# autonomousvision/unimatch

Hardware: NVIDIA H100
Metric: image-pairs/sec @480x832 gmflow-scale2-refine6; EPE vs reference (higher is better)
Workload: dtype fp32

## Files before the change

### include/unimatch_sm100.h

```cpp
#ifndef UNIMATCH_SM100_H_
#define UNIMATCH_SM100_H_

#include <stdint.h>

#ifdef __cplusplus
extern "C" {
#endif

#define UM_OK 0
#define UM_EINVAL (-22)
#define UM_ECUDA (-5)

#define UM_FEATURE_DIM 128

#define UM_ABI_VERSION 4
int um_abi_version(void);
const char* um_build_info(void);
const char* um_last_error(void);
int64_t um_launch_count(void);

#define UM_MASK_NONE 0
#define UM_MASK_SWIN 1
#define UM_MASK_CAUSAL 2

typedef struct um_attn_geom {
  int32_t h, w;
  int32_t kh, kw;
  int32_t sh, sw;
  int32_t mask_mode;
} um_attn_geom;

int um_window_attention(const float* q, const float* k, const float* v, float* out,
                        int32_t n_streams, int32_t kv_shift,
                        int64_t ldq, int64_t ldk, int64_t ldv, int64_t ldo,
                        const um_attn_geom* geom, void* workspace, int64_t workspace_bytes, int32_t flags,
                        void* stream);
#define UM_ATTN_FORCE_CUDA_CORES 1
int64_t um_window_attention_workspace(const um_attn_geom* geom, int32_t n_streams);

int32_t um_attention_planes_lp(const um_attn_geom* geom);
int um_window_attention_planes(const void* q_planes, const void* k_planes, const void* v_planes, float* out, int64_t ldo,
                               void* out_split, int64_t split_plane_stride, int32_t n_streams, int32_t kv_shift,
                               const um_attn_geom* geom, void* stream);

#define UM_VALUE_TENSOR 0
#define UM_VALUE_COORDS 1
#define UM_VALUE_XCOORD 2
#define UM_POST_NONE 0
#define UM_POST_MINUS_OWN 1
#define UM_POST_OWN_MINUS 2

int um_softmax_expectation(const float* q, const float* k, const float* values, float* out,
                           int32_t n_streams, int32_t n_total, int32_t kv_shift,
                           int64_t ldq, int64_t ldk, int32_t vdim, int32_t value_mode, int32_t post_op,
                           const um_attn_geom* geom, void* workspace, int64_t workspace_bytes, int32_t flags,
                           void* stream);
int64_t um_softmax_expectation_workspace(const um_attn_geom* geom, int32_t n_total, int32_t value_mode);

int um_local_corr_softmax(const float* f0, const float* f1, float* flow,
                          int32_t batch, int32_t h, int32_t w, int32_t ry, int32_t rx, int32_t stereo,
                          void* stream);

int um_local_corr_volume(const float* f0, const float* f1, const float* flow, float* corr,
                         int32_t batch, int32_t h, int32_t w, int32_t radius, int32_t flow_dim, void* stream);

int um_flow_warp(const float* f, const float* flow, float* out,
                 int32_t batch, int32_t h, int32_t w, int32_t flow_dim, void* stream);

int um_fb_consistency(const float* fwd_flow, const float* bwd_flow, float alpha, float beta, float* fwd_occ,
                      float* bwd_occ, int32_t batch, int32_t h, int32_t w, void* stream);

int um_fb_consistency_error(const float* fwd_flow, const float* bwd_flow, float alpha, float beta, float* fwd_occ,
                            float* bwd_occ, float* fwd_err, int32_t batch, int32_t h, int32_t w, void* stream);

int um_propagate_local(const float* q, const float* k, const float* flow, float* out,
                       int32_t batch, int32_t h, int32_t w, int32_t radius, int32_t flow_dim,
                       int64_t ldq, int64_t ldk, void* stream);

int um_depth_corr_softmax(const float* f0, const float* f1, const float* Kmat, const float* Kinv,
                          const float* pose, const float* cand, float* out,
                          int32_t batch, int32_t h, int32_t w, int32_t num_cand, int32_t from_argmax,
                          void* stream);

int um_add_position(const float* x, const float* table, float* out,
                    int32_t n_streams, int32_t h, int32_t w, int32_t wh, int32_t ww, void* stream);

int um_convex_upsample(const float* flow, const float* mask, float* up,
                       int32_t batch, int32_t h, int32_t w, int32_t flow_dim, int32_t factor, float mult,
                       void* stream);

int um_upsample2x(const float* flow, float* out, int32_t batch, int32_t h, int32_t w, int32_t flow_dim,
                  float mult, void* stream);

int um_resize_bilinear(const float* in, float* out, int32_t batch, int32_t channels, int32_t h_in, int32_t w_in,
                       int32_t h_out, int32_t w_out, const float* scale, int32_t flip_x, void* stream);

int um_frames_to_planar(const uint8_t* frames, float* out, int32_t n, int32_t h, int32_t w, int32_t transpose,
                        int32_t h_out, int32_t w_out, void* stream);

int um_frames_to_planar_normalized(const uint8_t* frames, float* out, int32_t n, int32_t h, int32_t w, int32_t h_out,
                                   int32_t w_out, const float* mean, const float* std, void* stream);

typedef struct um_ragged_item {
  int64_t offset;
  int32_t h, w;
  float scale;
  int32_t flags;
} um_ragged_item;
#define UM_RAGGED_FLIP_X 1
#define UM_RAGGED_TRANSPOSE 2

int um_frames_to_planar_normalized_ragged(const uint8_t* frames, int64_t frames_bytes, const um_ragged_item* items, float* out,
                                          int32_t n, int32_t h_max, int32_t w_max, int32_t h_out, int32_t w_out,
                                          const float* mean, const float* std, void* stream);

int um_frames_to_planar_ragged(const uint8_t* frames, int64_t frames_bytes, const um_ragged_item* items, float* out, int32_t n,
                               int32_t h_max, int32_t w_max, int32_t h_out, int32_t w_out, void* stream);

int um_resize_bilinear_ragged(const float* in, float* out, int64_t out_numel, const um_ragged_item* items, int32_t n,
                              int32_t h_in, int32_t w_in, int32_t h_max, int32_t w_max, void* stream);

int um_disparity_to_image_ragged(const float* disp, int64_t numel, const um_ragged_item* items, uint8_t* out,
                                 float* minmax_scratch, int32_t n, int32_t h_max, int32_t w_max, void* stream);

int um_flow_to_image_ragged(const float* flow, int64_t flow_numel, const um_ragged_item* flow_items, uint8_t* out,
                            int64_t out_bytes, const um_ragged_item* picture_items, float* max_scratch, int32_t n,
                            int32_t h_max, int32_t w_max, void* stream);

int um_fb_consistency_ragged(const float* flow, int64_t flow_numel, const um_ragged_item* flow_items, float alpha, float beta,
                             float* occ, int64_t occ_numel, const um_ragged_item* occ_items, int32_t n, int32_t h_max,
                             int32_t w_max, void* stream);

int um_chain_tracks(const float* flow, const float* occ, int32_t n, int32_t h, int32_t w, float* pos, uint8_t* vis,
                    float* pos_out, uint8_t* vis_out, void* stream);

int um_track_points_forward(const float* flow, const float* occ, int32_t n, int32_t h, int32_t w, int32_t t0,
                            const float* queries, int32_t nq, int32_t nt, float* pos, uint8_t* vis, float* tracks,
                            uint8_t* visible, void* stream);
int um_track_points_backward(const float* flow, const float* occ, int32_t n, int32_t h, int32_t w, const float* queries,
                             int32_t nq, int32_t nt, float* tracks, uint8_t* visible, void* stream);

int um_multi_flow_tracks(const float* flow, const float* occ, const float* err, const int32_t* src, const int32_t* dst,
                         int32_t n, int32_t k, int32_t h, int32_t w, int32_t r, float* pos, float* sig, uint8_t* vis,
                         float* tracks, uint8_t* visible, float* sigma, void* stream);

int um_flow_to_image(const float* flow, uint8_t* out, int64_t row_stride, int64_t image_stride, float* max_scratch,
                     int32_t n, int32_t h, int32_t w, void* stream);

int um_disparity_to_image(const float* disp, uint8_t* out, int64_t row_stride, int64_t image_stride, float* minmax_scratch,
                          int32_t n, int32_t h, int32_t w, void* stream);

int um_depth_to_image(const float* depth, uint8_t* out, int64_t row_stride, int64_t image_stride, void* scratch, int32_t n,
                      int32_t h, int32_t w, void* stream);

int um_depth_to_image_ragged(const float* depth, int64_t numel, const um_ragged_item* items, uint8_t* out, void* scratch,
                             int32_t n, int32_t h_max, int32_t w_max, void* stream);

#define UM_SUBMIT_CROP 0
#define UM_SUBMIT_RESIZE 1
#define UM_SUBMIT_FLO 0
#define UM_SUBMIT_KITTI_FLOW_PNG 1
#define UM_SUBMIT_KITTI_DISP_PNG 2
#define UM_SUBMIT_PFM 3
int um_encode_submission(const float* pred, int32_t batch, int32_t channels, int32_t h, int32_t w, int32_t geometry,
                         int32_t top, int32_t left, int32_t out_h, int32_t out_w, int32_t format, uint8_t* out,
                         int64_t sample_stride, void* stream);

#define UM_EVAL_FLOW 0
#define UM_EVAL_STEREO 1
#define UM_EVAL_DEPTH 2
#define UM_EVAL_PARTS 128
#define UM_EVAL_MASK_ALL 0
#define UM_EVAL_MASK_VALID 1
#define UM_EVAL_MASK_VALID_MAX 2
enum um_eval_flow_cols {
  UM_EVF_N = 0,
  UM_EVF_EPE,
  UM_EVF_1PX, UM_EVF_3PX, UM_EVF_5PX,
  UM_EVF_OUTLIER,
  UM_EVF_S0_10_N, UM_EVF_S0_10_EPE,
  UM_EVF_S10_40_N, UM_EVF_S10_40_EPE,
  UM_EVF_S40_N, UM_EVF_S40_EPE,
  UM_EVF_MATCHED_N, UM_EVF_MATCHED_EPE,
  UM_EVF_UNMATCHED_N, UM_EVF_UNMATCHED_EPE,
  UM_EVAL_FLOW_COLS
};
enum um_eval_stereo_cols {
  UM_EVS_N = 0, UM_EVS_ABS,
  UM_EVS_D1,
  UM_EVS_1PX, UM_EVS_2PX, UM_EVS_3PX,
  UM_EVAL_STEREO_COLS
};
enum um_eval_depth_cols {
  UM_EVD_N = 0,
  UM_EVD_ABS_REL,
  UM_EVD_SQ_REL,
  UM_EVD_SQ,
  UM_EVD_LOG_SQ,
  UM_EVD_A1, UM_EVD_A2, UM_EVD_A3,
  UM_EVAL_DEPTH_COLS
};
int um_eval_stats(const float* pred, int64_t pred_sb, int64_t pred_sc, int64_t pred_sy, int64_t pred_sx, const float* gt,
                  const float* valid, const float* noc_valid, int32_t task, int32_t mask_mode, float max_val, float eval_min,
                  float eval_max, int32_t batch, int32_t h, int32_t w, double* scratch, double* out, void* stream);

#define UM_ACT_NONE 0
#define UM_ACT_RELU 1
#define UM_ACT_TANH 2
#define UM_ACT_SIGMOID 3
#define UM_ACT_GELU 4
#define UM_CONV_LINEAR 0
#define UM_CONV_GRU_ZR 1
#define UM_CONV_GRU_Q 2
#define UM_CONV_LN 3
typedef struct um_conv_desc {
  const void* src[2];
  int32_t cin_p[2];
  int32_t nsrc;
  int32_t batch, h, w;
  const void* weights;
  const float* bias;
  int32_t kh, kw, pad_h, pad_w;
  int32_t cout, cout_p, bn;
  int32_t mode, act;
  float* out_f32;
  int64_t ld_f32;
  int32_t off_f32;
  int32_t cp_split;
  void* out_split;
  int32_t off_split;
  int32_t stride;
  const float* aux0;
  int64_t ld_aux0;
  const float* aux1;
  int64_t ld_aux1;
  const float* gamma;
  const float* beta;
  int64_t src_plane_stride, split_plane_stride;
  void* win_dst;
  int32_t win_c0, win_c1, win_lp, win_streams;
  um_attn_geom win_geom;
  const float* pre;
  int64_t ld_pre;
} um_conv_desc;
int um_conv2d_tc(const um_conv_desc* desc, void* stream);

typedef struct um_ffn_desc {
  const void* src[2];
  int64_t src_plane_stride;
  int64_t rows;
  const void* w1;
  const void* w2;
  int32_t hidden;
  const float* residual;
  int64_t ld_res;
  const float* gamma;
  const float* beta;
  float* out_f32;
  int64_t ld_f32;
  void* out_split;
  int64_t split_plane_stride;
} um_ffn_desc;
int um_ffn_tc(const um_ffn_desc* desc, void* stream);

int um_conv7x7_small(const float* in0, const float* in1, int32_t nchw, int32_t n_half, int32_t n, int32_t h, int32_t w,
                     int32_t cin, int32_t stride, const float* weight, const float* bias, int32_t cout, int32_t relu,
                     const float* scale, const float* shift, float* out_f32, int64_t ld_out, void* out_split, int32_t cp,
                     void* stream);

int64_t um_instance_norm_scratch_floats(int32_t n, int32_t c);
int um_instance_norm_stats(const float* x, int64_t ld, int32_t n, int32_t hw, int32_t c, float* scratch, float* stats,
                           void* stream);
int um_instance_norm_apply(const float* a, int64_t ld_a, const float* stats_a, int32_t relu_a, const float* res,
                           int64_t ld_res, const float* stats_res, int32_t relu_out, float* out_f32, int64_t ld_o,
                           void* out_split, int32_t cp, int32_t off, int32_t n, int32_t hw, int32_t c, void* stream);

int um_split_planes(const float* src, int64_t rows, int32_t channels, int64_t ld, void* dst, int32_t cp, int32_t off,
                    int64_t dst_plane_stride, void* stream);

#ifdef __cplusplus
}
#endif
#endif
```

### unimatch_b200/csrc/um_conv_tc.cu

```cuda
#include <stdlib.h>

#include "um_common.cuh"
#include "um_tc.cuh"

namespace um {

using namespace tc;

namespace {

constexpr int TW = 16, TH = 8;
__host__ __device__ constexpr int stages_for(int bn) { return bn >= 96 ? 2 : 3; }
constexpr int NTHREADS = 512;
constexpr int EPILOGUE = 8;
constexpr int PRODUCER = 12;
constexpr int REGS_PRODUCER = 32, REGS_MMA = 168, REGS_EPI = 144;
constexpr uint32_t A_BYTES = 2 * 16384;
constexpr uint32_t STAGING_UNIT = 16384;
constexpr uint32_t STAGING_BYTES = 2 * STAGING_UNIT;
constexpr uint32_t TAIL_BYTES = 256 + 2048;
__host__ __device__ constexpr uint32_t acc_bytes(int bn) { return (bn < 32 ? 32 : bn) * 128 * 4; }
__host__ __device__ constexpr uint32_t conv_smem_bytes(int bn) {
  return stages_for(bn) * (A_BYTES + 2 * bn * 128) + acc_bytes(bn) + STAGING_BYTES + TAIL_BYTES;
}

struct ConvParams {
  int B, H, W, tiles_x, tiles_y;
  int nsrc, cin_p[2];
  int KH, KW, PH, PW, stride;
  int cout, cout_p;
  const float* bias;
  int mode, act;
  float* out_f32; long long ld_f32; int off_f32;
  __half* out_split; int cp_split, off_split; long long plane_split;
  const float* aux0; long long ld_aux0;
  const float* aux1; long long ld_aux1;
  const float* gamma; const float* beta;
  const float* pre; long long ld_pre;
  int ntiles, tiles_n;
  __half* win_dst; long long win_plane;
  int win_c0, win_c1, win_lp;
  long long win_tokens, win_L;
  Geom win_g;
};

__device__ __forceinline__ float sigmoid_fast(float y) { return __fdividef(1.0f, 1.0f + __expf(-y)); }
__device__ __forceinline__ float tanh_fast(float y) { return 1.0f - __fdividef(2.0f, 1.0f + __expf(2.0f * y)); }
__device__ __forceinline__ uint32_t pack_h2(__half a, __half b) {
  return (uint32_t)__half_as_ushort(a) | ((uint32_t)__half_as_ushort(b) << 16);
}

__device__ __forceinline__ void load_acc32(const float* accs, int r, int c0, float* v) {
  const float* row = accs + (c0 >> 5) * 4096 + r * 32;
#pragma unroll
  for (int i = 0; i < 8; ++i) {
    const float4 x = *reinterpret_cast<const float4*>(row + ((i ^ (r & 7)) << 2));
    v[4 * i] = x.x; v[4 * i + 1] = x.y; v[4 * i + 2] = x.z; v[4 * i + 3] = x.w;
  }
}

template <int BN, int G, int MODE, int ACT, bool WIN = false>
__global__ void __launch_bounds__(NTHREADS, 1)
conv_tc_kernel(const __grid_constant__ CUtensorMap map_a0, const __grid_constant__ CUtensorMap map_a1,
               const __grid_constant__ CUtensorMap map_w, const __grid_constant__ CUtensorMap map_of,
               const __grid_constant__ CUtensorMap map_os, ConvParams p) {
  static_assert(BN == 16 || BN == 64 || BN == 96 || BN == 128, "tile widths 16, 64, 96, 128");
  constexpr int NSB = 2;
  constexpr uint32_t B_BYTES = 2 * BN * 128;
  constexpr uint32_t STAGE_BYTES = A_BYTES + B_BYTES;
  constexpr int STAGES = stages_for(BN);
  constexpr uint32_t ACC_BYTES = acc_bytes(BN);
  extern __shared__ __align__(1024) uint8_t smem[];
  float* accs = reinterpret_cast<float*>(smem + STAGES * STAGE_BYTES);
  float* stage_buf = reinterpret_cast<float*>(smem + STAGES * STAGE_BYTES + ACC_BYTES);
  uint64_t* bars = reinterpret_cast<uint64_t*>(smem + STAGES * STAGE_BYTES + ACC_BYTES + STAGING_BYTES);
  uint64_t* full = bars;
  uint64_t* empty = bars + STAGES;
  uint64_t* acc_full = bars + 2 * STAGES;
  uint64_t* acc_empty = acc_full + 1;
  float* coef = reinterpret_cast<float*>(reinterpret_cast<uint8_t*>(bars) + 256);
  const int mode = MODE >= 0 ? MODE : p.mode;
  const int act = ACT >= 0 ? ACT : p.act;

  const int warp = threadIdx.x >> 5, lane = threadIdx.x & 31;
  auto k_stages = [&]() {
    int n = 0;
    for (int s = 0; s < p.nsrc; ++s) n += p.KH * p.KW * (p.cin_p[s] >> 6);
    return n;
  };

  if (threadIdx.x == 0) {
    for (int i = 0; i < STAGES; ++i) { mbar_init(full + i, 1); mbar_init(empty + i, 8); }
    mbar_init(acc_full, 256);
    mbar_init(acc_empty, 128);
    fence_barrier_init();
  }
  if (warp == PRODUCER && lane == 0) {
    tma_prefetch_desc(&map_a0); tma_prefetch_desc(&map_w);
    if (p.nsrc > 1) tma_prefetch_desc(&map_a1);
  }
  __syncthreads();

  if (warp >= PRODUCER) {
    setmaxnreg_dec<REGS_PRODUCER>();
    if (warp != PRODUCER) return;
    const int cid = (int)blockIdx.x, ncid = (int)gridDim.x;
    const int taps = p.KH * p.KW;
    const int nk = k_stages();
    int it = 0;
    for (int t = cid; t < p.ntiles; t += ncid) {
      const int n0 = (t % p.tiles_n) * BN;
      int tile = t / p.tiles_n;
      const int x0 = (tile % p.tiles_x) * TW; tile /= p.tiles_x;
      const int y0 = (tile % p.tiles_y) * TH;
      const int b = tile / p.tiles_y;
      const int chunks0 = p.cin_p[0] >> 6;
      const int nk0 = taps * chunks0;
      const int rot = (int)((unsigned)cid % (unsigned)nk);
      for (int kk = 0; kk < nk; ++kk, ++it) {
        int k = kk + rot; if (k >= nk) k -= nk;
        const int sidx = (k >= nk0) ? 1 : 0;
        const int kl = sidx ? k - nk0 : k;
        const int chunks = sidx ? (p.cin_p[1] >> 6) : chunks0;
        const int tap = kl / chunks, kc = kl - tap * chunks;
        const int ky = tap / p.KW, kx = tap - ky * p.KW;
        const CUtensorMap* ma = sidx ? &map_a1 : &map_a0;
        const int st = it % STAGES;
        mbar_wait_inline(empty + st, ((it / STAGES) & 1) ^ 1);
        uint8_t* sa = smem + st * STAGE_BYTES;
        uint8_t* sb = sa + A_BYTES;
        const int kcol = (sidx ? taps * p.cin_p[0] : 0) + tap * p.cin_p[sidx] + kc * 64;
        if (elect_one()) {
          mbar_arrive_expect_tx(full + st, STAGE_BYTES);
#pragma unroll
          for (int part = 0; part < 2; ++part) {
            tma_load_4d(sa + part * 16384, ma, full + st, kc * 64, x0 * p.stride + kx - p.PW, y0 * p.stride + ky - p.PH, part * p.B + b);
            tma_load_2d(sb + part * (BN * 128), &map_w, full + st, kcol, part * p.cout_p + n0);
          }
        }
        __syncwarp();
      }
    }
  } else if (warp < EPILOGUE) {
    setmaxnreg_inc<REGS_MMA>();
    const int cid = (int)blockIdx.x, ncid = (int)gridDim.x;
    const int nk = k_stages();
    const int quarter = warp & 3;
    const int grp = warp >> 2;
    const int frow = grp * 64 + quarter * 16 + (lane >> 2);
    const int fcol = 2 * (lane & 3);
    int lt = 0, it = 0;
    for (int t = cid; t < p.ntiles; t += ncid, ++lt) {
      float acc[BN / 2], part[BN / 2];
      for (int k = 0; k < nk; ++k, ++it) {
        const int st = it % STAGES;
        mbar_wait_inline(full + st, (it / STAGES) & 1);
        const uint32_t a_base = smem_u32(smem + st * STAGE_BYTES) + grp * 8192;
        const uint32_t b_base = smem_u32(smem + st * STAGE_BYTES) + A_BYTES;
        const int pa[3] = {1, 0, 0}, pb[3] = {0, 1, 0};
        if (G > 1) fence_acc(part); else fence_acc(acc);
        wgmma_fence();
#pragma unroll
        for (int c = 0; c < 3; ++c)
#pragma unroll
          for (int ks = 0; ks < 4; ++ks) {
            const uint64_t da = desc_kmajor(a_base + pa[c] * 16384 + ks * 32);
            const uint64_t db = desc_kmajor(b_base + pb[c] * (BN * 128) + ks * 32);
            if (G > 1) wgmma_ss<BN>(part, da, db, (c | ks) != 0);
            else wgmma_ss<BN>(acc, da, db, k > 0 || (c | ks) != 0);
          }
        wgmma_commit();
        wgmma_wait<0>();
        if (G > 1) fence_acc(part); else fence_acc(acc);
        __syncwarp();
        if (lane == 0) mbar_arrive(empty + st);
        if (G > 1) {
#pragma unroll
          for (int i = 0; i < BN / 2; ++i) acc[i] = k ? acc[i] + part[i] : part[i];
        }
      }
      mbar_wait_inline(acc_empty, (lt & 1) ^ 1);
#pragma unroll
      for (int j = 0; j < BN / 8; ++j) {
        const int col = 8 * j + fcol;
        float* chunk = accs + (col >> 5) * 4096;
#pragma unroll
        for (int h = 0; h < 2; ++h) {
          const int row = frow + 8 * h;
          *reinterpret_cast<float2*>(chunk + row * 32 + ((((col & 31) >> 2) ^ (row & 7)) << 2) + (col & 3)) =
              make_float2(acc[4 * j + 2 * h], acc[4 * j + 2 * h + 1]);
        }
      }
      mbar_arrive(acc_full);
    }
  } else {
    setmaxnreg_inc<REGS_EPI>();
    const int cid = (int)blockIdx.x, ncid = (int)gridDim.x;
    const int r = threadIdx.x - EPILOGUE * 32;
    const bool leader = r == 0;
    int sctr = 0;
    auto epi_sync = [&]() { asm volatile("bar.sync 1, 128;" ::: "memory"); };
    if (mode == UM_CONV_LN) { coef[256 + r] = __ldg(p.gamma + r); coef[384 + r] = __ldg(p.beta + r); }
    epi_sync();
    int lt = 0;
    for (int t = cid; t < p.ntiles; t += ncid, ++lt) {
      const int n0 = (t % p.tiles_n) * BN;
      int tile = t / p.tiles_n;
      const int x0 = (tile % p.tiles_x) * TW; tile /= p.tiles_x;
      const int y0 = (tile % p.tiles_y) * TH;
      const int b = tile / p.tiles_y;
      const long long pix_r = ((long long)b * p.H + (y0 + (r >> 4))) * p.W + x0 + (r & 15);
      const bool valid_r = (y0 + (r >> 4) < p.H) && (x0 + (r & 15) < p.W);

      auto emit = [&](const float (&v)[32], int co_out, bool to_f32, bool to_split, bool to_win = false) {
        if (WIN && to_win) {
          uint8_t* sbs = reinterpret_cast<uint8_t*>(stage_buf + (sctr % NSB) * 4096);
          ++sctr;
          if (leader) bulk_wait_read<0>();
          epi_sync();
#pragma unroll
          for (int i = 0; i < 4; ++i) {
            uint32_t hw[4], lw[4];
#pragma unroll
            for (int e = 0; e < 4; ++e) split_f16x2(v[8 * i + 2 * e], v[8 * i + 2 * e + 1], &hw[e], &lw[e]);
            const int off = r * 64 + ((i ^ ((r >> 1) & 3)) << 4);
            *reinterpret_cast<uint4*>(sbs + off) = make_uint4(hw[0], hw[1], hw[2], hw[3]);
            *reinterpret_cast<uint4*>(sbs + 8192 + off) = make_uint4(lw[0], lw[1], lw[2], lw[3]);
          }
          epi_sync();
          const int wc = co_out - p.win_c0;
          __half* obase = p.win_dst + (long long)(wc >> 7) * 2 * p.win_plane + (wc & 127);
          const int* rowdst = reinterpret_cast<const int*>(coef + 256) + (lt & 1) * 128;
          const int piece = r & 3;
#pragma unroll
          for (int itr = 0; itr < 4; ++itr) {
            const int row = itr * 32 + (r >> 2);
            const int drow = rowdst[row];
            if (drow < 0) continue;
            const int soff = row * 64 + ((piece ^ ((row >> 1) & 3)) << 4);
            const uint4 hv = *reinterpret_cast<const uint4*>(sbs + soff);
            const uint4 lv = *reinterpret_cast<const uint4*>(sbs + 8192 + soff);
            __half* d = obase + (long long)drow * 128 + piece * 8;
            *reinterpret_cast<uint4*>(d) = hv;
            *reinterpret_cast<uint4*>(d + p.win_plane) = lv;
          }
          return;
        }
        if (to_f32) {
          float* my_stage = stage_buf + (sctr % NSB) * 4096;
          ++sctr;
          if (leader) bulk_wait_read<NSB - 1>();
          epi_sync();
#pragma unroll
          for (int i = 0; i < 8; ++i)
            *reinterpret_cast<float4*>(my_stage + r * 32 + ((i ^ (r & 7)) << 2)) = make_float4(v[4 * i], v[4 * i + 1], v[4 * i + 2], v[4 * i + 3]);
          fence_proxy_async();
          epi_sync();
          if (leader) { tma_store_4d(&map_of, my_stage, co_out, x0, y0, b); bulk_commit(); }
        }
        if (to_split) {
          uint8_t* sbs = reinterpret_cast<uint8_t*>(stage_buf + (sctr % NSB) * 4096);
          ++sctr;
          if (leader) bulk_wait_read<NSB - 1>();
          epi_sync();
#pragma unroll
          for (int i = 0; i < 4; ++i) {
            uint32_t hw[4], lw[4];
#pragma unroll
            for (int e = 0; e < 4; ++e) split_f16x2(v[8 * i + 2 * e], v[8 * i + 2 * e + 1], &hw[e], &lw[e]);
            const int off = r * 64 + ((i ^ ((r >> 1) & 3)) << 4);
            *reinterpret_cast<uint4*>(sbs + off) = make_uint4(hw[0], hw[1], hw[2], hw[3]);
            *reinterpret_cast<uint4*>(sbs + 8192 + off) = make_uint4(lw[0], lw[1], lw[2], lw[3]);
          }
          fence_proxy_async();
          epi_sync();
          if (leader) {
            tma_store_4d(&map_os, sbs, co_out, x0, y0, b);
            tma_store_4d(&map_os, sbs + 8192, co_out, x0, y0, p.B + b);
            bulk_commit();
          }
        }
      };

      if constexpr (BN == 128) {
        if (mode == UM_CONV_LN) {
          mbar_wait_inline(acc_full, lt & 1);
          float sum0 = 0.f, sum1 = 0.f, sq0 = 0.f, sq1 = 0.f;
#pragma unroll 1
          for (int h = 0; h < 2; ++h) {
            float v0[32], v1[32];
            load_acc32(accs, r, 32 * h, v0);
            load_acc32(accs, r, 64 + 32 * h, v1);
            float sum = 0.f;
#pragma unroll
            for (int i = 0; i < 32; ++i) sum += v0[i];
#pragma unroll
            for (int i = 0; i < 32; ++i) sum += v1[i];
            if (h == 0) sum0 = sum; else sum1 = sum;
          }
          const float mean = (sum0 + sum1) * (1.0f / 128.0f);
#pragma unroll 1
          for (int h = 0; h < 2; ++h) {
            float v0[32], v1[32];
            load_acc32(accs, r, 32 * h, v0);
            load_acc32(accs, r, 64 + 32 * h, v1);
            float sq = 0.f;
#pragma unroll
            for (int i = 0; i < 32; ++i) { const float dd = v0[i] - mean; sq = fmaf(dd, dd, sq); }
#pragma unroll
            for (int i = 0; i < 32; ++i) { const float dd = v1[i] - mean; sq = fmaf(dd, dd, sq); }
            if (h == 0) sq0 = sq; else sq1 = sq;
          }
          const float rstd = rsqrtf((sq0 + sq1) * (1.0f / 128.0f) + 1e-5f);
          const bool need_a = valid_r && p.aux0;
#pragma unroll 1
          for (int c0 = 0; c0 < 128; c0 += 32) {
            float a[32];
            if (need_a) {
              const float4* pa = reinterpret_cast<const float4*>(p.aux0 + pix_r * p.ld_aux0 + c0);
#pragma unroll
              for (int i = 0; i < 8; ++i) { const float4 t4 = __ldg(pa + i); a[4 * i] = t4.x; a[4 * i + 1] = t4.y; a[4 * i + 2] = t4.z; a[4 * i + 3] = t4.w; }
            }
            float v[32];
            load_acc32(accs, r, c0, v);
            if (c0 == 96) mbar_arrive(acc_empty);
            const float4* g4 = reinterpret_cast<const float4*>(coef + 256 + c0);
            const float4* b4 = reinterpret_cast<const float4*>(coef + 384 + c0);
#pragma unroll
            for (int i = 0; i < 8; ++i) {
              const float4 g = g4[i], bb = b4[i];
              v[4 * i] = (v[4 * i] - mean) * rstd * g.x + bb.x;
              v[4 * i + 1] = (v[4 * i + 1] - mean) * rstd * g.y + bb.y;
              v[4 * i + 2] = (v[4 * i + 2] - mean) * rstd * g.z + bb.z;
              v[4 * i + 3] = (v[4 * i + 3] - mean) * rstd * g.w + bb.w;
            }
            if (need_a) {
#pragma unroll
              for (int i = 0; i < 32; ++i) v[i] += a[i];
            }
            emit(v, c0, p.out_f32 != nullptr, p.out_split != nullptr);
          }
          continue;
        }
      }

      float* sbias = coef + (lt & 1) * 128;
      if (r < BN) sbias[r] = (p.bias && n0 + r < p.cout) ? __ldg(p.bias + n0 + r) : 0.f;
      if (WIN) {
        const int yy = y0 + (r >> 4), xx = x0 + (r & 15);
        const long long token = ((long long)b * p.H + yy) * p.W + xx;
        int drow = -1;
        if (yy < p.H && xx < p.W && token < p.win_tokens) {
          const Geom& g = p.win_g;
          const int n = (int)(token / p.win_L);
          const int t = (int)(token - (long long)n * p.win_L);
          const int ty = t / g.w, tx = t - ty * g.w;
          int yr = ty - g.sh; if (yr < 0) yr += g.h;
          int xr = tx - g.sw; if (xr < 0) xr += g.w;
          const int wy = yr / g.wh, wx = xr / g.ww;
          drow = (n * g.nwin + wy * g.kw + wx) * p.win_lp + (yr - wy * g.wh) * g.ww + (xr - wx * g.ww);
        }
        reinterpret_cast<int*>(coef + 256)[(lt & 1) * 128 + r] = drow;
      }
      epi_sync();

      constexpr int CH = BN < 32 ? BN : 32;
#pragma unroll 1
      for (int c0 = 0; c0 < BN; c0 += 32) {
        const int co0 = n0 + c0;
        const bool live = co0 < p.cout;
        bool to_f32 = p.out_f32 != nullptr, to_split = p.out_split != nullptr;
        int co_out = co0;
        if (mode == UM_CONV_GRU_ZR) {
          to_f32 = co0 < 128; to_split = co0 >= 128;
          if (co0 >= 128) co_out = co0 - 128;
        }
        bool to_win = false;
        if (WIN && co0 >= p.win_c0 && co0 < p.win_c1) { to_win = true; to_f32 = to_split = false; }
        float px[32];
        const bool need_p = live && valid_r && p.pre;
        if (need_p) {
          const float4* pp = reinterpret_cast<const float4*>(p.pre + pix_r * p.ld_pre + co0);
#pragma unroll
          for (int i = 0; i < 8; ++i) { const float4 t4 = __ldg(pp + i); px[4 * i] = t4.x; px[4 * i + 1] = t4.y; px[4 * i + 2] = t4.z; px[4 * i + 3] = t4.w; }
        }
        float v[32];
        mbar_wait_inline(acc_full, lt & 1);
        load_acc32(accs, r, c0, v);
        if (c0 + 32 >= BN) mbar_arrive(acc_empty);
        if (!live) continue;
        if (p.bias) {
          const float4* s4 = reinterpret_cast<const float4*>(sbias + c0);
#pragma unroll
          for (int i = 0; i < CH / 4; ++i) {
            const float4 bb = s4[i];
            v[4 * i] += bb.x; v[4 * i + 1] += bb.y; v[4 * i + 2] += bb.z; v[4 * i + 3] += bb.w;
          }
        }
        if (need_p) {
#pragma unroll
          for (int i = 0; i < CH; ++i) v[i] += px[i];
        }
        float ax[32], bx[32];
        const bool need_a = valid_r && p.aux0 && (mode == UM_CONV_GRU_Q || (mode == UM_CONV_GRU_ZR && co0 >= 128));
        const bool need_b = valid_r && mode == UM_CONV_GRU_Q;
        if (need_a) {
          const float4* ap = reinterpret_cast<const float4*>(p.aux0 + pix_r * p.ld_aux0 + (mode == UM_CONV_GRU_ZR ? co0 - 128 : co0));
#pragma unroll
          for (int i = 0; i < 8; ++i) { const float4 t4 = __ldg(ap + i); ax[4 * i] = t4.x; ax[4 * i + 1] = t4.y; ax[4 * i + 2] = t4.z; ax[4 * i + 3] = t4.w; }
        }
        if (need_b) {
          const float4* bp = reinterpret_cast<const float4*>(p.aux1 + pix_r * p.ld_aux1 + co0);
#pragma unroll
          for (int i = 0; i < 8; ++i) { const float4 t4 = __ldg(bp + i); bx[4 * i] = t4.x; bx[4 * i + 1] = t4.y; bx[4 * i + 2] = t4.z; bx[4 * i + 3] = t4.w; }
        }
        if (mode == UM_CONV_GRU_ZR) {
#pragma unroll
          for (int i = 0; i < CH; ++i) v[i] = sigmoid_fast(v[i]);
          if (need_a) {
#pragma unroll
            for (int i = 0; i < CH; ++i) v[i] *= ax[i];
          }
        } else if (mode == UM_CONV_GRU_Q) {
          if (need_b) {
#pragma unroll
            for (int i = 0; i < CH; ++i) v[i] = (1.0f - bx[i]) * ax[i] + bx[i] * tanh_fast(v[i]);
          }
        } else if (act == UM_ACT_RELU) {
#pragma unroll
          for (int i = 0; i < CH; ++i) v[i] = fmaxf(v[i], 0.f);
        } else if (act == UM_ACT_TANH) {
#pragma unroll
          for (int i = 0; i < CH; ++i) v[i] = tanh_fast(v[i]);
        } else if (act == UM_ACT_SIGMOID) {
#pragma unroll
          for (int i = 0; i < CH; ++i) v[i] = sigmoid_fast(v[i]);
        } else if (act == UM_ACT_GELU) {
#pragma unroll
          for (int i = 0; i < CH; ++i) v[i] = act_gelu(v[i]);
        }
        if constexpr (BN >= 32) {
          emit(v, co_out, to_f32, to_split, to_win);
        } else {
          const int nvalid = min(CH, p.cout - co0);
          float* sb = stage_buf;
          epi_sync();
#pragma unroll
          for (int i = 0; i < CH / 4; ++i)
            *reinterpret_cast<float4*>(sb + r * 32 + ((i ^ (r & 7)) << 2)) = make_float4(v[4 * i], v[4 * i + 1], v[4 * i + 2], v[4 * i + 3]);
          epi_sync();
          if (to_f32) {
#pragma unroll 1
            for (int itr = 0; itr < 8; ++itr) {
              const int row = itr * 16 + (r >> 3), piece = r & 7;
              const int yy = y0 + (row >> 4), xx = x0 + (row & 15);
              if (yy >= p.H || xx >= p.W || piece * 4 >= nvalid) continue;
              const float4 val = *reinterpret_cast<const float4*>(sb + row * 32 + ((piece ^ (row & 7)) << 2));
              float* dst = p.out_f32 + (((long long)b * p.H + yy) * p.W + xx) * p.ld_f32 + p.off_f32 + co_out + piece * 4;
              const float e[4] = {val.x, val.y, val.z, val.w};
              for (int k = 0; k < 4; ++k) if (piece * 4 + k < nvalid) dst[k] = e[k];
            }
          }
          if (to_split) {
#pragma unroll 1
            for (int itr = 0; itr < 4; ++itr) {
              const int row = itr * 32 + (r >> 2), piece = r & 3;
              const int yy = y0 + (row >> 4), xx = x0 + (row & 15);
              if (yy >= p.H || xx >= p.W || piece * 8 >= nvalid) continue;
              const float4 a4 = *reinterpret_cast<const float4*>(sb + row * 32 + (((2 * piece) ^ (row & 7)) << 2));
              const float4 c4 = *reinterpret_cast<const float4*>(sb + row * 32 + (((2 * piece + 1) ^ (row & 7)) << 2));
              const float e[8] = {a4.x, a4.y, a4.z, a4.w, c4.x, c4.y, c4.z, c4.w};
              __half* dh = p.out_split + (((long long)b * p.H + yy) * p.W + xx) * p.cp_split + p.off_split + co_out + piece * 8;
              __half* dl = dh + p.plane_split;
              for (int k = 0; k < 8; ++k)
                if (piece * 8 + k < nvalid) { __half h0, l0; split_f16(e[k], &h0, &l0); dh[k] = h0; dl[k] = l0; }
            }
          }
        }
      }
    }
    if (leader) bulk_wait_all();
  }
}

template <int VEC>
__global__ void __launch_bounds__(256) split_planes_kernel(const float* __restrict__ src, long long ld, int C,
                                                           __half* __restrict__ dst, int cp, int off, long long plane,
                                                           long long rows) {
  const int per_row = C / VEC;
  const long long i = (long long)blockIdx.x * blockDim.x + threadIdx.x;
  if (i >= rows * per_row) return;
  const long long row = i / per_row;
  const int c = (int)(i - row * per_row) * VEC;
  if (VEC == 4) {
    const float4 x = __ldg(reinterpret_cast<const float4*>(src + row * ld + c));
    __half h[4], l[4];
    split_f16(x.x, &h[0], &l[0]); split_f16(x.y, &h[1], &l[1]); split_f16(x.z, &h[2], &l[2]); split_f16(x.w, &h[3], &l[3]);
    *reinterpret_cast<uint2*>(dst + row * cp + off + c) = make_uint2(pack_h2(h[0], h[1]), pack_h2(h[2], h[3]));
    *reinterpret_cast<uint2*>(dst + plane + row * cp + off + c) = make_uint2(pack_h2(l[0], l[1]), pack_h2(l[2], l[3]));
  } else {
    __half h, l;
    split_f16(__ldg(src + row * ld + c), &h, &l);
    dst[row * cp + off + c] = h;
    dst[plane + row * cp + off + c] = l;
  }
}

}

int make_map_4d_f16(CUtensorMap* map, const void* base, uint64_t cp, uint64_t W, uint64_t H, uint64_t NB, uint32_t stride,
                    uint64_t plane_elems) {
  PFN_encodeTiled enc = get_encode_tiled();
  if (!enc) { set_error("cuTensorMapEncodeTiled unavailable"); return UM_ECUDA; }
  cuuint64_t dims[4] = {cp, W, H, NB};
  cuuint64_t strides[3] = {cp * 2, cp * W * 2, (plane_elems ? plane_elems : cp * W * H) * 2};
  cuuint32_t box[4] = {64, 16 * stride, 8 * stride, 1};
  cuuint32_t estr[4] = {1, stride, stride, 1};
  CUresult r = enc(map, CU_TENSOR_MAP_DATA_TYPE_FLOAT16, 4, const_cast<void*>(base), dims, strides, box, estr,
                   CU_TENSOR_MAP_INTERLEAVE_NONE, CU_TENSOR_MAP_SWIZZLE_128B, CU_TENSOR_MAP_L2_PROMOTION_L2_128B,
                   CU_TENSOR_MAP_FLOAT_OOB_FILL_NONE);
  if (r != CUDA_SUCCESS) { set_error("cuTensorMapEncodeTiled(4d) failed (%d)", (int)r); return UM_ECUDA; }
  return UM_OK;
}

int make_map_out(CUtensorMap* map, void* base, int elem_bytes, uint64_t cout, uint64_t ld, uint64_t W, uint64_t H, uint64_t N,
                 uint64_t plane_elems) {
  PFN_encodeTiled enc = get_encode_tiled();
  if (!enc) { set_error("cuTensorMapEncodeTiled unavailable"); return UM_ECUDA; }
  cuuint64_t dims[4] = {cout, W, H, N};
  cuuint64_t strides[3] = {ld * elem_bytes, ld * W * elem_bytes, (plane_elems ? plane_elems : ld * W * H) * elem_bytes};
  cuuint32_t box[4] = {32, 16, 8, 1};
  cuuint32_t estr[4] = {1, 1, 1, 1};
  CUresult r = enc(map, elem_bytes == 4 ? CU_TENSOR_MAP_DATA_TYPE_FLOAT32 : CU_TENSOR_MAP_DATA_TYPE_FLOAT16, 4, base, dims,
                   strides, box, estr, CU_TENSOR_MAP_INTERLEAVE_NONE,
                   elem_bytes == 4 ? CU_TENSOR_MAP_SWIZZLE_128B : CU_TENSOR_MAP_SWIZZLE_64B,
                   CU_TENSOR_MAP_L2_PROMOTION_NONE, CU_TENSOR_MAP_FLOAT_OOB_FILL_NONE);
  if (r != CUDA_SUCCESS) { set_error("cuTensorMapEncodeTiled(out) failed (%d)", (int)r); return UM_ECUDA; }
  return UM_OK;
}

namespace {

template <int BN, int G, int MODE, int ACT, bool WIN = false>
int launch_conv(const CUtensorMap& m0, const CUtensorMap& m1, const CUtensorMap& mw, const CUtensorMap& mof,
                const CUtensorMap& mos, const ConvParams& p, cudaStream_t st) {
  constexpr uint32_t smem = conv_smem_bytes(BN);
  static_assert(smem <= 232448, "shared memory budget");
  static PerDeviceBytes configured;
  if (int rc = ensure_smem(configured, conv_tc_kernel<BN, G, MODE, ACT, WIN>, smem, "conv_tc")) return rc;
  const int num_sms = device_sm_count();
  const int grid = p.ntiles < num_sms ? p.ntiles : num_sms;
  conv_tc_kernel<BN, G, MODE, ACT, WIN><<<grid, NTHREADS, smem, st>>>(m0, m1, mw, mof, mos, p);
  return check_launch("um_conv2d_tc");
}

}
}

extern "C" {

int um_conv2d_tc(const um_conv_desc* d, void* stream) {
  using namespace um;
  UM_REQUIRE(d && d->src[0] && d->weights, "um_conv2d_tc: null descriptor / source / weights");
  UM_REQUIRE(d->batch > 0 && d->h > 0 && d->w > 0, "um_conv2d_tc: bad shape");
  UM_REQUIRE(d->nsrc == 1 || (d->nsrc == 2 && d->src[1]), "um_conv2d_tc: nsrc must be 1 or 2");
  for (int s = 0; s < d->nsrc; ++s)
    UM_REQUIRE(d->cin_p[s] > 0 && d->cin_p[s] % 64 == 0, "um_conv2d_tc: padded input channels must be multiples of 64");
  UM_REQUIRE(d->bn == 16 || d->bn == 64 || d->bn == 96 || d->bn == 128 || d->bn == 192 || d->bn == 256,
             "um_conv2d_tc: bn must be 16, 64, 96, 128, 192 or 256");
  UM_REQUIRE(d->cout > 0 && d->cout_p >= d->cout && d->cout_p % d->bn == 0, "um_conv2d_tc: bad output channel padding");
  UM_REQUIRE(d->kh > 0 && d->kw > 0 && d->kh * d->kw <= 49, "um_conv2d_tc: bad filter size");
  UM_REQUIRE(d->mode >= UM_CONV_LINEAR && d->mode <= UM_CONV_LN, "um_conv2d_tc: bad mode");
  if (d->mode == UM_CONV_LN)
    UM_REQUIRE(d->cout == 128 && d->cout_p == 128 && d->bn == 128 && d->gamma && d->beta && d->ld_f32 % 4 == 0 &&
                   d->off_f32 % 4 == 0 && d->cp_split % 8 == 0 && d->off_split % 8 == 0 && d->ld_aux0 % 4 == 0,
               "um_conv2d_tc: LN needs cout = cout_p = bn = 128, gamma/beta and 16-byte aligned rows");
  const bool win = d->win_dst != nullptr;
  UM_REQUIRE(d->out_f32 || d->out_split || win, "um_conv2d_tc: no output");
  Geom wg{};
  if (win) {
    UM_REQUIRE(d->mode == UM_CONV_LINEAR && d->act == UM_ACT_NONE && d->bn == 128 && d->batch == 1 && d->stride == 1 &&
                   d->kh == 1 && d->kw == 1 && d->nsrc == 1 && d->cin_p[0] == 128,
               "um_conv2d_tc: window-plane output needs a plain 128 -> cout Linear layer (bn 128, batch 1)");
    UM_REQUIRE(make_geom(&d->win_geom, &wg), "um_conv2d_tc: bad window geometry");
    UM_REQUIRE(d->win_c0 >= 0 && d->win_c0 % 128 == 0 && d->win_c1 % 128 == 0 && d->win_c1 > d->win_c0 && d->win_c1 <= d->cout_p,
               "um_conv2d_tc: window-plane channel range must be 128-aligned and inside cout_p");
    UM_REQUIRE(d->win_streams > 0 && d->win_lp >= wg.lw && d->win_lp % 128 == 0 &&
                   (long long)d->win_streams * wg.h * wg.w <= (long long)d->h * d->w,
               "um_conv2d_tc: window-plane rows (streams * h * w) exceed the GEMM rows / bad lp");
    UM_REQUIRE((reinterpret_cast<uintptr_t>(d->win_dst) & 15) == 0, "um_conv2d_tc: window planes must be 16-byte aligned");
    UM_REQUIRE(d->out_f32 || d->out_split || (d->win_c0 == 0 && d->win_c1 >= d->cout),
               "um_conv2d_tc: channels outside the window-plane range have no destination");
  }
  if (d->src_plane_stride || d->split_plane_stride)
    UM_REQUIRE(d->batch == 1 && d->src_plane_stride >= 0 && d->split_plane_stride >= 0 && d->src_plane_stride % 8 == 0 &&
                   d->split_plane_stride % 8 == 0,
               "um_conv2d_tc: explicit (hi, lo) plane strides need batch 1 and multiples of 8 halves");
  if (d->mode == UM_CONV_GRU_ZR)
    UM_REQUIRE(d->cout == 256 && (d->bn == 128 || d->bn == 256) && d->aux0 && d->out_f32 && d->out_split,
               "um_conv2d_tc: GRU_ZR needs cout 256, bn 128 or 256, h, z-out and rh-out");
  if (d->mode == UM_CONV_GRU_Q)
    UM_REQUIRE(d->cout == 128 && d->aux0 && d->aux1, "um_conv2d_tc: GRU_Q needs cout 128, h and z");

  if (d->pre)
    UM_REQUIRE(d->mode != UM_CONV_LN && d->bn >= 32 && d->ld_pre % 4 == 0 && d->ld_pre >= d->cout && d->cout % 32 == 0 &&
                   (reinterpret_cast<uintptr_t>(d->pre) & 15) == 0,
               "um_conv2d_tc: pre-accumulated input needs a non-LN mode, bn >= 32, cout %% 32 == 0 and 16-byte aligned rows");
  UM_REQUIRE(d->stride == 1 || d->stride == 2 || d->stride == 4 || d->stride == 8, "um_conv2d_tc: stride must be 1, 2, 4 or 8");
  const int ho = (d->h + 2 * d->pad_h - d->kh) / d->stride + 1, wo = (d->w + 2 * d->pad_w - d->kw) / d->stride + 1;
  UM_REQUIRE(ho > 0 && wo > 0, "um_conv2d_tc: empty output");
  ConvParams p{};
  p.B = d->batch; p.H = ho; p.W = wo; p.stride = d->stride;
  p.tiles_x = (wo + TW - 1) / TW; p.tiles_y = (ho + TH - 1) / TH;
  p.nsrc = d->nsrc; p.cin_p[0] = d->cin_p[0]; p.cin_p[1] = d->nsrc > 1 ? d->cin_p[1] : 0;
  p.KH = d->kh; p.KW = d->kw; p.PH = d->pad_h; p.PW = d->pad_w;
  p.cout = d->cout; p.cout_p = d->cout_p; p.bias = d->bias; p.mode = d->mode; p.act = d->act;
  p.out_f32 = d->out_f32; p.ld_f32 = d->ld_f32; p.off_f32 = d->off_f32;
  p.out_split = reinterpret_cast<__half*>(d->out_split); p.cp_split = d->cp_split; p.off_split = d->off_split;
  p.plane_split = (long long)d->batch * ho * wo * d->cp_split;
  p.aux0 = d->aux0; p.ld_aux0 = d->ld_aux0; p.aux1 = d->aux1; p.ld_aux1 = d->ld_aux1;
  p.gamma = d->gamma; p.beta = d->beta;
  p.pre = d->pre; p.ld_pre = d->ld_pre;
  if (d->split_plane_stride) p.plane_split = d->split_plane_stride;
  if (win) {
    p.win_dst = reinterpret_cast<__half*>(d->win_dst);
    p.win_g = wg; p.win_lp = d->win_lp; p.win_c0 = d->win_c0; p.win_c1 = d->win_c1;
    p.win_L = (long long)wg.h * wg.w;
    p.win_tokens = (long long)d->win_streams * p.win_L;
    p.win_plane = (long long)d->win_streams * wg.nwin * d->win_lp * 128;
  }

  long long ktot = 0;
  for (int s = 0; s < d->nsrc; ++s) ktot += (long long)d->kh * d->kw * d->cin_p[s];
  const long long nk = ktot / 64;
  const bool multi = nk >= 8;
  const int bn = d->bn == 256 ? 128 : d->bn == 192 ? 96 : d->bn;
  p.tiles_n = d->cout_p / bn;
  p.ntiles = p.tiles_x * p.tiles_y * p.B * p.tiles_n;
  CUtensorMap m0, m1, mw;
  int rc;
  const uint64_t sps = (uint64_t)d->src_plane_stride;
  if ((rc = make_map_4d_f16(&m0, d->src[0], d->cin_p[0], d->w, d->h, 2ull * d->batch, d->stride, sps))) return rc;
  if (d->nsrc > 1) { if ((rc = make_map_4d_f16(&m1, d->src[1], d->cin_p[1], d->w, d->h, 2ull * d->batch, d->stride, sps))) return rc; }
  else m1 = m0;
  if ((rc = make_map_2d_f16(&mw, d->weights, 2ull * d->cout_p, (uint64_t)ktot, (uint32_t)bn))) return rc;
  cudaStream_t st = (cudaStream_t)stream;
  CUtensorMap mof = m0, mos = m0;
  if (d->bn >= 32) {
    const int c_f32 = (d->mode == UM_CONV_GRU_ZR) ? 128 : d->cout, c_split = (d->mode == UM_CONV_GRU_ZR) ? 128 : d->cout;
    if (d->out_f32) {
      UM_REQUIRE(d->ld_f32 % 4 == 0 && d->off_f32 % 4 == 0 && (reinterpret_cast<uintptr_t>(d->out_f32) & 15) == 0,
                 "um_conv2d_tc: fp32 output must be 16-byte aligned (ld, channel offset multiples of 4)");
      if ((rc = make_map_out(&mof, d->out_f32 + d->off_f32, 4, c_f32, d->ld_f32, wo, ho, d->batch))) return rc;
    }
    if (d->out_split) {
      UM_REQUIRE(d->cp_split % 8 == 0 && d->off_split % 8 == 0 && (reinterpret_cast<uintptr_t>(d->out_split) & 15) == 0,
                 "um_conv2d_tc: split output must be 16-byte aligned (cp, channel offset multiples of 8)");
      if ((rc = make_map_out(&mos, reinterpret_cast<__half*>(d->out_split) + d->off_split, 2, c_split, d->cp_split, wo, ho,
                             2ull * d->batch, (uint64_t)d->split_plane_stride))) return rc;
    }
  }
#define UM_CONV_CASE(BN_, G_, MODE_, ACT_)                                                   \
  if (bn == BN_ && multi == (G_ > 1) && d->mode == MODE_ && ((MODE_) != UM_CONV_LINEAR || d->act == (ACT_))) \
    return launch_conv<BN_, G_, MODE_, (MODE_) == UM_CONV_LINEAR ? (ACT_) : 0>(m0, m1, mw, mof, mos, p, st);
  if (win) {
    UM_REQUIRE(nk <= 2, "um_conv2d_tc: window-plane output is built for K <= 128");
    return launch_conv<128, 1, UM_CONV_LINEAR, UM_ACT_NONE, true>(m0, m1, mw, mof, mos, p, st);
  }
  UM_CONV_CASE(128, 1, UM_CONV_LINEAR, UM_ACT_NONE)
  UM_CONV_CASE(128, 1, UM_CONV_LINEAR, UM_ACT_RELU)
  UM_CONV_CASE(128, 1, UM_CONV_LINEAR, UM_ACT_GELU)
  UM_CONV_CASE(128, 1, UM_CONV_LN, 0)
  UM_CONV_CASE(128, 2, UM_CONV_LN, 0)
  UM_CONV_CASE(128, 2, UM_CONV_LINEAR, UM_ACT_NONE)
  UM_CONV_CASE(128, 2, UM_CONV_LINEAR, UM_ACT_RELU)
  UM_CONV_CASE(128, 2, UM_CONV_GRU_ZR, 0)
  UM_CONV_CASE(128, 2, UM_CONV_GRU_Q, 0)
  UM_CONV_CASE(96, 2, UM_CONV_LINEAR, UM_ACT_RELU)
  UM_CONV_CASE(64, 4, UM_CONV_LINEAR, UM_ACT_NONE)
  UM_CONV_CASE(64, 4, UM_CONV_LINEAR, UM_ACT_RELU)
#undef UM_CONV_CASE
  if (bn == 128) return multi ? launch_conv<128, 2, -1, -1>(m0, m1, mw, mof, mos, p, st) : launch_conv<128, 1, -1, -1>(m0, m1, mw, mof, mos, p, st);
  if (bn == 96) return multi ? launch_conv<96, 2, -1, -1>(m0, m1, mw, mof, mos, p, st) : launch_conv<96, 1, -1, -1>(m0, m1, mw, mof, mos, p, st);
  if (bn == 64) return multi ? launch_conv<64, 4, -1, -1>(m0, m1, mw, mof, mos, p, st) : launch_conv<64, 1, -1, -1>(m0, m1, mw, mof, mos, p, st);
  return multi ? launch_conv<16, 4, -1, -1>(m0, m1, mw, mof, mos, p, st) : launch_conv<16, 1, -1, -1>(m0, m1, mw, mof, mos, p, st);
}

int um_split_planes(const float* src, int64_t rows, int32_t channels, int64_t ld, void* dst, int32_t cp, int32_t off,
                    int64_t dst_plane_stride, void* stream) {
  UM_REQUIRE(src && dst && rows > 0 && channels > 0 && off >= 0 && off + channels <= cp && ld >= channels,
             "um_split_planes: bad arguments");
  UM_REQUIRE(dst_plane_stride == 0 || (dst_plane_stride >= rows * cp && dst_plane_stride % 4 == 0),
             "um_split_planes: dst_plane_stride must cover rows * cp halves (multiple of 4)");
  const long long plane = dst_plane_stride ? (long long)dst_plane_stride : (long long)rows * cp;
  const bool vec = (channels % 4 == 0) && (ld % 4 == 0) && (off % 4 == 0) && (cp % 4 == 0) &&
                   ((reinterpret_cast<uintptr_t>(src) & 15) == 0);
  if (vec) {
    const long long total = (long long)rows * (channels / 4);
    um::split_planes_kernel<4><<<(unsigned)((total + 255) / 256), 256, 0, (cudaStream_t)stream>>>(
        src, ld, channels, reinterpret_cast<__half*>(dst), cp, off, plane, rows);
  } else {
    const long long total = (long long)rows * channels;
    um::split_planes_kernel<1><<<(unsigned)((total + 255) / 256), 256, 0, (cudaStream_t)stream>>>(
        src, ld, channels, reinterpret_cast<__half*>(dst), cp, off, plane, rows);
  }
  return um::check_launch("um_split_planes");
}

}
```

### unimatch_b200/csrc/um_norm.cu

```cuda
#include "um_common.cuh"
#include "um_tc.cuh"

namespace {

constexpr int CHUNKS = 64;

__device__ __forceinline__ float4 in_pivot(const float* __restrict__ x, long long ld, int hw, int n, int c4) {
  const int np = hw < 16 ? hw : 16;
  float4 p = make_float4(0.f, 0.f, 0.f, 0.f);
  for (int r = 0; r < np; ++r) {
    const float4 v = __ldg(reinterpret_cast<const float4*>(x + ((long long)n * hw + r) * ld) + c4);
    p.x += v.x; p.y += v.y; p.z += v.z; p.w += v.w;
  }
  const float inv = 1.0f / (float)np;
  return make_float4(p.x * inv, p.y * inv, p.z * inv, p.w * inv);
}

__global__ void __launch_bounds__(256) in_partial_kernel(const float* __restrict__ x, long long ld, int hw, int C,
                                                         float* __restrict__ partial) {
  extern __shared__ float sm[];
  const int n = blockIdx.y, chunk = blockIdx.x;
  const int c4n = C >> 2;
  const int rlanes = 256 / c4n;
  const int c4 = threadIdx.x % c4n, rl = threadIdx.x / c4n;
  const int rows_per_chunk = (hw + CHUNKS - 1) / CHUNKS;
  const int r0 = chunk * rows_per_chunk, r1 = min(hw, r0 + rows_per_chunk);
  float4 s = make_float4(0.f, 0.f, 0.f, 0.f), q = make_float4(0.f, 0.f, 0.f, 0.f);
  if (rl < rlanes) {
    const float4 pv = in_pivot(x, ld, hw, n, c4);
    for (int r = r0 + rl; r < r1; r += rlanes) {
      float4 v = __ldg(reinterpret_cast<const float4*>(x + ((long long)n * hw + r) * ld) + c4);
      v.x -= pv.x; v.y -= pv.y; v.z -= pv.z; v.w -= pv.w;
      s.x += v.x; s.y += v.y; s.z += v.z; s.w += v.w;
      q.x = fmaf(v.x, v.x, q.x); q.y = fmaf(v.y, v.y, q.y); q.z = fmaf(v.z, v.z, q.z); q.w = fmaf(v.w, v.w, q.w);
    }
  }
  float* ss = sm;
  float* qs = sm + rlanes * C;
  if (rl < rlanes) {
    reinterpret_cast<float4*>(ss + rl * C)[c4] = s;
    reinterpret_cast<float4*>(qs + rl * C)[c4] = q;
  }
  __syncthreads();
  if (threadIdx.x < C) {
    float a = 0.f, b = 0.f;
    for (int i = 0; i < rlanes; ++i) { a += ss[i * C + threadIdx.x]; b += qs[i * C + threadIdx.x]; }
    float* dst = partial + (((long long)n * CHUNKS + chunk) * 2) * C;
    dst[threadIdx.x] = a;
    dst[C + threadIdx.x] = b;
  }
}

__global__ void in_finalize_kernel(const float* __restrict__ x, long long ld, const float* __restrict__ partial,
                                   float* __restrict__ stats, int hw, int C, int total) {
  const int i = blockIdx.x * blockDim.x + threadIdx.x;
  if (i >= total) return;
  const int n = i / C, c = i - n * C;
  const float4 pv = in_pivot(x, ld, hw, n, c >> 2);
  const float piv = (c & 3) == 0 ? pv.x : (c & 3) == 1 ? pv.y : (c & 3) == 2 ? pv.z : pv.w;
  double s = 0.0, q = 0.0;
  for (int k = 0; k < CHUNKS; ++k) {
    const float* p = partial + (((long long)n * CHUNKS + k) * 2) * C;
    s += (double)p[c]; q += (double)p[C + c];
  }
  const double dm = s / hw;
  double var = q / hw - dm * dm;
  if (var < 0.0) var = 0.0;
  stats[((long long)n * 2) * C + c] = (float)((double)piv + dm);
  stats[((long long)n * 2 + 1) * C + c] = (float)(1.0 / sqrt(var + 1e-5));
}

struct ApplyParams {
  const float* a; long long ld_a; const float* st_a; int relu_a;
  const float* res; long long ld_res; const float* st_res; int relu_out;
  float* out; long long ld_o;
  __half* split; int cp, off; long long plane;
  int hw, C; long long total4;
};

__device__ __forceinline__ uint32_t pk(__half a, __half b) {
  return (uint32_t)__half_as_ushort(a) | ((uint32_t)__half_as_ushort(b) << 16);
}

__global__ void __launch_bounds__(256) in_apply_kernel(ApplyParams p) {
  long long i = (long long)blockIdx.x * blockDim.x + threadIdx.x;
  const long long stride = (long long)gridDim.x * blockDim.x;
  const int c4n = p.C >> 2;
  for (; i < p.total4; i += stride) {
    const int c4 = (int)(i % c4n);
    const long long row = i / c4n;
    const int n = (int)(row / p.hw);
    float4 v = __ldg(reinterpret_cast<const float4*>(p.a + row * p.ld_a) + c4);
    if (p.st_a) {
      const float4 m = __ldg(reinterpret_cast<const float4*>(p.st_a + ((long long)n * 2) * p.C) + c4);
      const float4 r = __ldg(reinterpret_cast<const float4*>(p.st_a + ((long long)n * 2 + 1) * p.C) + c4);
      v.x = (v.x - m.x) * r.x; v.y = (v.y - m.y) * r.y; v.z = (v.z - m.z) * r.z; v.w = (v.w - m.w) * r.w;
    }
    if (p.relu_a) { v.x = fmaxf(v.x, 0.f); v.y = fmaxf(v.y, 0.f); v.z = fmaxf(v.z, 0.f); v.w = fmaxf(v.w, 0.f); }
    if (p.res) {
      float4 u = __ldg(reinterpret_cast<const float4*>(p.res + row * p.ld_res) + c4);
      if (p.st_res) {
        const float4 m = __ldg(reinterpret_cast<const float4*>(p.st_res + ((long long)n * 2) * p.C) + c4);
        const float4 r = __ldg(reinterpret_cast<const float4*>(p.st_res + ((long long)n * 2 + 1) * p.C) + c4);
        u.x = (u.x - m.x) * r.x; u.y = (u.y - m.y) * r.y; u.z = (u.z - m.z) * r.z; u.w = (u.w - m.w) * r.w;
      }
      v.x += u.x; v.y += u.y; v.z += u.z; v.w += u.w;
    }
    if (p.relu_out) { v.x = fmaxf(v.x, 0.f); v.y = fmaxf(v.y, 0.f); v.z = fmaxf(v.z, 0.f); v.w = fmaxf(v.w, 0.f); }
    if (p.out) reinterpret_cast<float4*>(p.out + row * p.ld_o)[c4] = v;
    if (p.split) {
      __half h[4], l[4];
      um::tc::split_f16(v.x, &h[0], &l[0]); um::tc::split_f16(v.y, &h[1], &l[1]);
      um::tc::split_f16(v.z, &h[2], &l[2]); um::tc::split_f16(v.w, &h[3], &l[3]);
      __half* d = p.split + row * p.cp + p.off + c4 * 4;
      *reinterpret_cast<uint2*>(d) = make_uint2(pk(h[0], h[1]), pk(h[2], h[3]));
      *reinterpret_cast<uint2*>(d + p.plane) = make_uint2(pk(l[0], l[1]), pk(l[2], l[3]));
    }
  }
}

}

extern "C" {

int64_t um_instance_norm_scratch_floats(int32_t n, int32_t c) { return (int64_t)n * CHUNKS * 2 * c; }

int um_instance_norm_stats(const float* x, int64_t ld, int32_t n, int32_t hw, int32_t c, float* scratch, float* stats,
                           void* stream) {
  UM_REQUIRE(x && scratch && stats && n > 0 && hw > 0 && c > 0 && c % 4 == 0 && c <= 256 && ld % 4 == 0 && ld >= c,
             "um_instance_norm_stats: bad arguments (channels must be a multiple of 4, <= 256)");
  const int rlanes = 256 / (c / 4);
  UM_REQUIRE(rlanes >= 1, "um_instance_norm_stats: too many channels");
  cudaStream_t st = (cudaStream_t)stream;
  in_partial_kernel<<<dim3(CHUNKS, n), 256, 2 * rlanes * c * sizeof(float), st>>>(x, ld, hw, c, scratch);
  int rc = um::check_launch("um_instance_norm_stats(partial)");
  if (rc) return rc;
  const int total = n * c;
  in_finalize_kernel<<<(total + 127) / 128, 128, 0, st>>>(x, ld, scratch, stats, hw, c, total);
  return um::check_launch("um_instance_norm_stats(finalize)");
}

int um_instance_norm_apply(const float* a, int64_t ld_a, const float* stats_a, int32_t relu_a, const float* res,
                           int64_t ld_res, const float* stats_res, int32_t relu_out, float* out_f32, int64_t ld_o,
                           void* out_split, int32_t cp, int32_t off, int32_t n, int32_t hw, int32_t c, void* stream) {
  UM_REQUIRE(a && n > 0 && hw > 0 && c > 0 && c % 4 == 0 && ld_a % 4 == 0, "um_instance_norm_apply: bad arguments");
  UM_REQUIRE(out_f32 || out_split, "um_instance_norm_apply: no output");
  UM_REQUIRE(!res || ld_res % 4 == 0, "um_instance_norm_apply: bad residual stride");
  UM_REQUIRE(!out_f32 || ld_o % 4 == 0, "um_instance_norm_apply: bad output stride");
  UM_REQUIRE(!out_split || (cp % 4 == 0 && off % 4 == 0 && off + c <= cp), "um_instance_norm_apply: bad split layout");
  ApplyParams p{};
  p.a = a; p.ld_a = ld_a; p.st_a = stats_a; p.relu_a = relu_a;
  p.res = res; p.ld_res = ld_res; p.st_res = stats_res; p.relu_out = relu_out;
  p.out = out_f32; p.ld_o = ld_o;
  p.split = reinterpret_cast<__half*>(out_split); p.cp = cp; p.off = off; p.plane = (long long)n * hw * cp;
  p.hw = hw; p.C = c; p.total4 = (long long)n * hw * (c / 4);
  long long blocks = (p.total4 + 255) / 256;
  if (blocks > 132LL * 32) blocks = 132LL * 32;
  in_apply_kernel<<<(unsigned)blocks, 256, 0, (cudaStream_t)stream>>>(p);
  return um::check_launch("um_instance_norm_apply");
}

}
```

### unimatch_b200/csrc/um_stem.cu

```cuda
#include "um_common.cuh"
#include "um_tc.cuh"

namespace {

constexpr int TX = 32, TY = 8;
constexpr int PX = 4;
constexpr int CB = 16;
constexpr int NT = 256;

struct StemParams {
  const float* in0; const float* in1;
  int nchw, n_half;
  int N, H, W, cin, stride;
  int HO, WO, cout;
  const float* weight;
  const float* bias;
  int relu;
  float scale[3], shift[3];
  float* out; long long ld_out;
  __half* split; int cp; long long plane;
  int tiles_x, tiles_y, ntiles;
};

template <int CIN, int S>
__global__ void __launch_bounds__(NT) stem7x7_kernel(StemParams p) {
  extern __shared__ __align__(16) float sm[];
  constexpr int IWR = (TX - 1) * S + 7, IW = (IWR + 3) & ~3, IH = (TY - 1) * S + 7;
  constexpr int NIN = (PX - 1) * S + 7;
  float* s_w = sm;
  float* s_in = sm + p.cout * CIN * 49;
  const int tid = threadIdx.x;
  for (int i = tid; i < p.cout * CIN * 49; i += NT) {
    const int co = i / (CIN * 49), k = i - co * (CIN * 49);
    s_w[k * p.cout + co] = __ldg(p.weight + i);
  }
  const int pg = tid & 63, cg = tid >> 6;
  const int lx = (pg & 7) * PX, ly = pg >> 3;

  for (int t = blockIdx.x; t < p.ntiles; t += gridDim.x) {
    int tt = t;
    const int tx0 = (tt % p.tiles_x) * TX; tt /= p.tiles_x;
    const int ty0 = (tt % p.tiles_y) * TY;
    const int n = tt / p.tiles_y;
    const int x_in0 = tx0 * S - 3, y_in0 = ty0 * S - 3;
    __syncthreads();
    for (int i = tid; i < CIN * IH * IW; i += NT) {
      const int c = i / (IH * IW), r = i - c * IH * IW;
      const int yy = y_in0 + r / IW, xx = x_in0 + r % IW;
      float v = 0.f;
      if (yy >= 0 && yy < p.H && xx >= 0 && xx < p.W) {
        if (p.nchw) {
          const float* src = (n < p.n_half) ? p.in0 + (long long)n * CIN * p.H * p.W : p.in1 + (long long)(n - p.n_half) * CIN * p.H * p.W;
          v = __ldg(src + ((long long)c * p.H + yy) * p.W + xx) * p.scale[c] + p.shift[c];
        } else {
          v = __ldg(p.in0 + (((long long)n * p.H + yy) * p.W + xx) * CIN + c);
        }
      }
      s_in[i] = v;
    }
    __syncthreads();
    const int oy = ty0 + ly;
    for (int cbase = cg * CB; cbase < p.cout; cbase += 4 * CB) {
      float acc[PX][CB];
#pragma unroll
      for (int c = 0; c < CB; ++c) {
        const float bv = p.bias ? __ldg(p.bias + cbase + c) : 0.f;
#pragma unroll
        for (int j = 0; j < PX; ++j) acc[j][c] = bv;
      }
#pragma unroll 1
      for (int c = 0; c < CIN; ++c) {
#pragma unroll 1
        for (int ky = 0; ky < 7; ++ky) {
          const float* row = s_in + (c * IH + ly * S + ky) * IW + lx * S;
          float in[16];
#pragma unroll
          for (int q = 0; q < (NIN + 3) / 4; ++q) {
            const float4 v4 = *reinterpret_cast<const float4*>(row + 4 * q);
            in[4 * q] = v4.x; in[4 * q + 1] = v4.y; in[4 * q + 2] = v4.z; in[4 * q + 3] = v4.w;
          }
          const float* wrow = s_w + ((c * 7 + ky) * 7) * p.cout + cbase;
#pragma unroll
          for (int kx = 0; kx < 7; ++kx) {
            float w[CB];
#pragma unroll
            for (int q = 0; q < CB / 4; ++q) {
              const float4 w4 = *reinterpret_cast<const float4*>(wrow + kx * p.cout + 4 * q);
              w[4 * q] = w4.x; w[4 * q + 1] = w4.y; w[4 * q + 2] = w4.z; w[4 * q + 3] = w4.w;
            }
#pragma unroll
            for (int j = 0; j < PX; ++j) {
              const float xv = in[j * S + kx];
#pragma unroll
              for (int cc = 0; cc < CB; ++cc) acc[j][cc] = fmaf(xv, w[cc], acc[j][cc]);
            }
          }
        }
      }
      if (oy < p.HO) {
#pragma unroll
        for (int j = 0; j < PX; ++j) {
          const int ox = tx0 + lx + j;
          if (ox >= p.WO) continue;
          const long long pix = ((long long)n * p.HO + oy) * p.WO + ox;
          if (p.relu) {
#pragma unroll
            for (int cc = 0; cc < CB; ++cc) acc[j][cc] = fmaxf(acc[j][cc], 0.f);
          }
          if (p.out) {
#pragma unroll
            for (int q = 0; q < CB / 4; ++q)
              *reinterpret_cast<float4*>(p.out + pix * p.ld_out + cbase + 4 * q) =
                  make_float4(acc[j][4 * q], acc[j][4 * q + 1], acc[j][4 * q + 2], acc[j][4 * q + 3]);
          }
          if (p.split) {
            __half* d = p.split + pix * p.cp + cbase;
#pragma unroll
            for (int q = 0; q < CB / 8; ++q) {
              uint32_t hw[4], lw[4];
#pragma unroll
              for (int e = 0; e < 4; ++e) um::tc::split_f16x2(acc[j][8 * q + 2 * e], acc[j][8 * q + 2 * e + 1], &hw[e], &lw[e]);
              *reinterpret_cast<uint4*>(d + 8 * q) = make_uint4(hw[0], hw[1], hw[2], hw[3]);
              *reinterpret_cast<uint4*>(d + p.plane + 8 * q) = make_uint4(lw[0], lw[1], lw[2], lw[3]);
            }
          }
        }
      }
    }
  }
}

template <int CIN, int S>
int launch(StemParams p, cudaStream_t st) {
  constexpr int IWR = (TX - 1) * S + 7, IW = (IWR + 3) & ~3, IH = (TY - 1) * S + 7;
  const size_t smem = (size_t)(p.cout * CIN * 49 + CIN * IH * IW + 8) * sizeof(float);
  static um::PerDeviceBytes configured;
  if (int rc = um::ensure_smem(configured, stem7x7_kernel<CIN, S>, smem, "stem7x7")) return rc;
  const int num_sms = um::device_sm_count();
  p.tiles_x = (p.WO + TX - 1) / TX; p.tiles_y = (p.HO + TY - 1) / TY;
  p.ntiles = p.tiles_x * p.tiles_y * p.N;
  const int grid = p.ntiles < 2 * num_sms ? p.ntiles : 2 * num_sms;
  stem7x7_kernel<CIN, S><<<grid, NT, smem, st>>>(p);
  return um::check_launch("um_conv7x7_small");
}

}

extern "C" int um_conv7x7_small(const float* in0, const float* in1, int32_t nchw, int32_t n_half, int32_t n, int32_t h,
                                int32_t w, int32_t cin, int32_t stride, const float* weight, const float* bias, int32_t cout,
                                int32_t relu, const float* scale, const float* shift, float* out_f32, int64_t ld_out,
                                void* out_split, int32_t cp, void* stream) {
  UM_REQUIRE(in0 && weight && n > 0 && h > 0 && w > 0 && cin >= 1 && cin <= 3 && (stride == 1 || stride == 2),
             "um_conv7x7_small: bad arguments (1 <= cin <= 3, stride 1 or 2)");
  UM_REQUIRE(cout > 0 && cout % 16 == 0 && cout <= 128 && (out_f32 || out_split),
             "um_conv7x7_small: cout must be a multiple of 16 (<= 128) and an output given");
  UM_REQUIRE(!out_f32 || ld_out % 4 == 0, "um_conv7x7_small: bad output stride");
  UM_REQUIRE(!out_split || cp % 8 == 0, "um_conv7x7_small: bad plane width");
  UM_REQUIRE(!nchw || in1 || n_half >= n, "um_conv7x7_small: second source missing");
  StemParams p{};
  p.in0 = in0; p.in1 = in1; p.nchw = nchw; p.n_half = n_half;
  p.N = n; p.H = h; p.W = w; p.cin = cin; p.stride = stride;
  p.HO = (h + 6 - 7) / stride + 1; p.WO = (w + 6 - 7) / stride + 1; p.cout = cout;
  p.weight = weight; p.bias = bias; p.relu = relu;
  for (int c = 0; c < 3; ++c) { p.scale[c] = scale ? scale[c] : 1.f; p.shift[c] = shift ? shift[c] : 0.f; }
  p.out = out_f32; p.ld_out = ld_out;
  p.split = reinterpret_cast<__half*>(out_split); p.cp = cp; p.plane = (long long)n * p.HO * p.WO * cp;
  cudaStream_t st = (cudaStream_t)stream;
  if (stride == 1) {
    if (cin == 1) return launch<1, 1>(p, st);
    if (cin == 2) return launch<2, 1>(p, st);
    return launch<3, 1>(p, st);
  }
  if (cin == 1) return launch<1, 2>(p, st);
  if (cin == 2) return launch<2, 2>(p, st);
  return launch<3, 2>(p, st);
}
```

### unimatch_b200/ops.py

```python
import ctypes
import os

import torch

_HERE = os.path.dirname(os.path.abspath(__file__))
LIB_PATH = os.path.join(_HERE, "libunimatch_sm100.so")

MASK_NONE, MASK_SWIN, MASK_CAUSAL = 0, 1, 2
VALUE_TENSOR, VALUE_COORDS, VALUE_XCOORD = 0, 1, 2
POST_NONE, POST_MINUS_OWN, POST_OWN_MINUS = 0, 1, 2


FORCE_CUDA_CORES = 1
_force_cuda_cores = False


def set_force_cuda_cores(flag):
    global _force_cuda_cores
    _force_cuda_cores = bool(flag)


EVAL_FLOW, EVAL_STEREO, EVAL_DEPTH = 0, 1, 2
EVAL_MASK_ALL, EVAL_MASK_VALID, EVAL_MASK_VALID_MAX = 0, 1, 2
EVAL_PARTS = 128
EVAL_FLOW_COLS = ("n", "epe", "1px", "3px", "5px", "outlier", "s0_10_n", "s0_10_epe", "s10_40_n", "s10_40_epe", "s40_n",
                  "s40_epe", "matched_n", "matched_epe", "unmatched_n", "unmatched_epe")
EVAL_STEREO_COLS = ("n", "abs", "d1", "1px", "2px", "3px")
EVAL_DEPTH_COLS = ("n", "abs_rel", "sq_rel", "sq", "log_sq", "a1", "a2", "a3")
EVAL_COLS = {EVAL_FLOW: EVAL_FLOW_COLS, EVAL_STEREO: EVAL_STEREO_COLS, EVAL_DEPTH: EVAL_DEPTH_COLS}


ACT_NONE, ACT_RELU, ACT_TANH, ACT_SIGMOID, ACT_GELU = 0, 1, 2, 3, 4
CONV_LINEAR, CONV_GRU_ZR, CONV_GRU_Q, CONV_LN = 0, 1, 2, 3


class AttnGeom(ctypes.Structure):
    _fields_ = [(n, ctypes.c_int32) for n in ("h", "w", "kh", "kw", "sh", "sw", "mask_mode")]


class ConvDesc(ctypes.Structure):
    _fields_ = [("src", ctypes.c_void_p * 2), ("cin_p", ctypes.c_int32 * 2), ("nsrc", ctypes.c_int32),
                ("batch", ctypes.c_int32), ("h", ctypes.c_int32), ("w", ctypes.c_int32),
                ("weights", ctypes.c_void_p), ("bias", ctypes.c_void_p),
                ("kh", ctypes.c_int32), ("kw", ctypes.c_int32), ("pad_h", ctypes.c_int32), ("pad_w", ctypes.c_int32),
                ("cout", ctypes.c_int32), ("cout_p", ctypes.c_int32), ("bn", ctypes.c_int32),
                ("mode", ctypes.c_int32), ("act", ctypes.c_int32),
                ("out_f32", ctypes.c_void_p), ("ld_f32", ctypes.c_int64), ("off_f32", ctypes.c_int32),
                ("cp_split", ctypes.c_int32), ("out_split", ctypes.c_void_p), ("off_split", ctypes.c_int32),
                ("stride", ctypes.c_int32),
                ("aux0", ctypes.c_void_p), ("ld_aux0", ctypes.c_int64), ("aux1", ctypes.c_void_p), ("ld_aux1", ctypes.c_int64),
                ("gamma", ctypes.c_void_p), ("beta", ctypes.c_void_p),
                ("src_plane_stride", ctypes.c_int64), ("split_plane_stride", ctypes.c_int64),
                ("win_dst", ctypes.c_void_p), ("win_c0", ctypes.c_int32), ("win_c1", ctypes.c_int32),
                ("win_lp", ctypes.c_int32), ("win_streams", ctypes.c_int32), ("win_geom", AttnGeom),
                ("pre", ctypes.c_void_p), ("ld_pre", ctypes.c_int64)]


class RaggedItem(ctypes.Structure):
    _fields_ = [("offset", ctypes.c_int64), ("h", ctypes.c_int32), ("w", ctypes.c_int32), ("scale", ctypes.c_float),
                ("flags", ctypes.c_int32)]


RAGGED_FLIP_X, RAGGED_TRANSPOSE = 1, 2
RAGGED_ITEM_BYTES = ctypes.sizeof(RaggedItem)


class FfnDesc(ctypes.Structure):
    _fields_ = [("src", ctypes.c_void_p * 2), ("src_plane_stride", ctypes.c_int64), ("rows", ctypes.c_int64),
                ("w1", ctypes.c_void_p), ("w2", ctypes.c_void_p), ("hidden", ctypes.c_int32),
                ("residual", ctypes.c_void_p), ("ld_res", ctypes.c_int64), ("gamma", ctypes.c_void_p), ("beta", ctypes.c_void_p),
                ("out_f32", ctypes.c_void_p), ("ld_f32", ctypes.c_int64), ("out_split", ctypes.c_void_p),
                ("split_plane_stride", ctypes.c_int64)]


_P, _I, _L, _F = ctypes.c_void_p, ctypes.c_int32, ctypes.c_int64, ctypes.c_float
_G, _FP, _RC = ctypes.POINTER(AttnGeom), ctypes.POINTER(ctypes.c_float), ctypes.c_int

_SIGNATURES = {
    "um_abi_version": (_RC, []),
    "um_build_info": (ctypes.c_char_p, []),
    "um_last_error": (ctypes.c_char_p, []),
    "um_launch_count": (_L, []),
    "um_window_attention": (_RC, [_P, _P, _P, _P, _I, _I, _L, _L, _L, _L, _G, _P, _L, _I, _P]),
    "um_window_attention_workspace": (_L, [_G, _I]),
    "um_attention_planes_lp": (_I, [_G]),
    "um_window_attention_planes": (_RC, [_P, _P, _P, _P, _L, _P, _L, _I, _I, _G, _P]),
    "um_softmax_expectation": (_RC, [_P, _P, _P, _P, _I, _I, _I, _L, _L, _I, _I, _I, _G, _P, _L, _I, _P]),
    "um_softmax_expectation_workspace": (_L, [_G, _I, _I]),
    "um_local_corr_softmax": (_RC, [_P, _P, _P, _I, _I, _I, _I, _I, _I, _P]),
    "um_local_corr_volume": (_RC, [_P, _P, _P, _P, _I, _I, _I, _I, _I, _P]),
    "um_flow_warp": (_RC, [_P, _P, _P, _I, _I, _I, _I, _P]),
    "um_fb_consistency": (_RC, [_P, _P, _F, _F, _P, _P, _I, _I, _I, _P]),
    "um_fb_consistency_ragged": (_RC, [_P, _L, _P, _F, _F, _P, _L, _P, _I, _I, _I, _P]),
    "um_fb_consistency_error": (_RC, [_P, _P, _F, _F, _P, _P, _P, _I, _I, _I, _P]),
    "um_chain_tracks": (_RC, [_P, _P, _I, _I, _I, _P, _P, _P, _P, _P]),
    "um_track_points_forward": (_RC, [_P, _P, _I, _I, _I, _I, _P, _I, _I, _P, _P, _P, _P, _P]),
    "um_track_points_backward": (_RC, [_P, _P, _I, _I, _I, _P, _I, _I, _P, _P, _P]),
    "um_multi_flow_tracks": (_RC, [_P, _P, _P, _P, _P, _I, _I, _I, _I, _I, _P, _P, _P, _P, _P, _P, _P]),
    "um_propagate_local": (_RC, [_P, _P, _P, _P, _I, _I, _I, _I, _I, _L, _L, _P]),
    "um_depth_corr_softmax": (_RC, [_P, _P, _P, _P, _P, _P, _P, _I, _I, _I, _I, _I, _P]),
    "um_add_position": (_RC, [_P, _P, _P, _I, _I, _I, _I, _I, _P]),
    "um_convex_upsample": (_RC, [_P, _P, _P, _I, _I, _I, _I, _I, _F, _P]),
    "um_upsample2x": (_RC, [_P, _P, _I, _I, _I, _I, _F, _P]),
    "um_resize_bilinear": (_RC, [_P, _P, _I, _I, _I, _I, _I, _I, _FP, _I, _P]),
    "um_frames_to_planar": (_RC, [_P, _P, _I, _I, _I, _I, _I, _I, _P]),
    "um_frames_to_planar_ragged": (_RC, [_P, _L, _P, _P, _I, _I, _I, _I, _I, _P]),
    "um_frames_to_planar_normalized": (_RC, [_P, _P, _I, _I, _I, _I, _I, _FP, _FP, _P]),
    "um_frames_to_planar_normalized_ragged": (_RC, [_P, _L, _P, _P, _I, _I, _I, _I, _I, _FP, _FP, _P]),
    "um_resize_bilinear_ragged": (_RC, [_P, _P, _L, _P, _I, _I, _I, _I, _I, _P]),
    "um_disparity_to_image_ragged": (_RC, [_P, _L, _P, _P, _P, _I, _I, _I, _P]),
    "um_flow_to_image": (_RC, [_P, _P, _L, _L, _P, _I, _I, _I, _P]),
    "um_flow_to_image_ragged": (_RC, [_P, _L, _P, _P, _L, _P, _P, _I, _I, _I, _P]),
    "um_disparity_to_image": (_RC, [_P, _P, _L, _L, _P, _I, _I, _I, _P]),
    "um_depth_to_image": (_RC, [_P, _P, _L, _L, _P, _I, _I, _I, _P]),
    "um_depth_to_image_ragged": (_RC, [_P, _L, _P, _P, _P, _I, _I, _I, _P]),
    "um_encode_submission": (_RC, [_P, _I, _I, _I, _I, _I, _I, _I, _I, _I, _I, _P, _L, _P]),
    "um_eval_stats": (_RC, [_P, _L, _L, _L, _L, _P, _P, _P, _I, _I, _F, _F, _F, _I, _I, _I, _P, _P, _P]),
    "um_conv2d_tc": (_RC, [ctypes.POINTER(ConvDesc), _P]),
    "um_ffn_tc": (_RC, [ctypes.POINTER(FfnDesc), _P]),
    "um_conv7x7_small": (_RC, [_P, _P, _I, _I, _I, _I, _I, _I, _I, _P, _P, _I, _I, _FP, _FP, _P, _L, _P, _I, _P]),
    "um_instance_norm_scratch_floats": (_L, [_I, _I]),
    "um_instance_norm_stats": (_RC, [_P, _L, _I, _I, _I, _P, _P, _P]),
    "um_instance_norm_apply": (_RC, [_P, _L, _P, _I, _P, _L, _P, _I, _P, _L, _P, _I, _I, _I, _I, _I, _P]),
    "um_split_planes": (_RC, [_P, _L, _I, _L, _P, _I, _I, _L, _P]),
}
SYMBOLS = list(_SIGNATURES)


def _load():
    from .csrc.build import build, have_nvcc
    if have_nvcc():
        build()
    elif not os.path.exists(LIB_PATH):
        raise ImportError("libunimatch_sm100.so is missing and nvcc is not available to build it")
    lib = ctypes.CDLL(LIB_PATH)
    missing = [s for s in SYMBOLS if not hasattr(lib, s)]
    if missing:
        raise ImportError("libunimatch_sm100.so lacks symbols %s (stale build? run python unimatch_b200/csrc/build.py --force)" % missing)
    for name, (restype, argtypes) in _SIGNATURES.items():
        fn = getattr(lib, name)
        fn.restype, fn.argtypes = restype, argtypes
    return lib


LIB = _load()


def build_info():
    return LIB.um_build_info().decode()


def launch_count():
    return int(LIB.um_launch_count())


def _check(rc, name):
    if rc != 0:
        raise RuntimeError("%s failed (%d): %s" % (name, rc, LIB.um_last_error().decode()))


def _p(t):
    return ctypes.c_void_p(t.data_ptr()) if t is not None else None


def _stream():
    return ctypes.c_void_p(torch.cuda.current_stream().cuda_stream)


def _f32c(t, name, rows_ok=False):
    if not t.is_cuda:
        raise RuntimeError("%s: expected a CUDA tensor (libunimatch_sm100 has no CPU path)" % name)
    if t.dtype != torch.float32:
        raise RuntimeError("%s: expected float32" % name)
    if rows_ok:
        if t.stride(-1) != 1:
            raise RuntimeError("%s: last dim must be contiguous" % name)
    elif not t.is_contiguous():
        raise RuntimeError("%s: expected a contiguous tensor" % name)
    return t


def _rows(t, name):
    _f32c(t, name, rows_ok=True)
    if t.dim() != 3 or t.shape[-1] != 128:
        raise RuntimeError("%s: expected [N, L, 128]" % name)
    ld = t.stride(1)
    if t.shape[0] > 1 and t.stride(0) != ld * t.shape[1]:
        raise RuntimeError("%s: batch stride must equal L * row stride" % name)
    return ld


_lib = torch.library.Library("unimatch_sm100", "DEF")


def _define(schema, impl):
    _lib.define(schema)
    name = schema.split("(")[0]
    _lib.impl(name, impl, "CUDA")
    return getattr(torch.ops.unimatch_sm100, name)


def _window_attention(q, k, v, kv_shift, h, w, kh, kw, sh, sw, mask_mode):
    ldq, ldk, ldv = _rows(q, "q"), _rows(k, "k"), _rows(v, "v")
    n, l, _ = q.shape
    out = torch.empty((n, l, 128), device=q.device, dtype=torch.float32)
    g = AttnGeom(h, w, kh, kw, sh, sw, mask_mode)
    flags = FORCE_CUDA_CORES if _force_cuda_cores else 0
    ws_bytes = 0 if flags else int(LIB.um_window_attention_workspace(ctypes.byref(g), n))
    ws = torch.empty((ws_bytes,), device=q.device, dtype=torch.uint8) if ws_bytes else None
    _check(LIB.um_window_attention(_p(q), _p(k), _p(v), _p(out), n, kv_shift, ldq, ldk, ldv, 128, ctypes.byref(g),
                                   _p(ws), ws_bytes, flags, _stream()), "um_window_attention")
    return out


window_attention = _define(
    "window_attention(Tensor q, Tensor k, Tensor v, int kv_shift, int h, int w, int kh, int kw, int sh, int sw, "
    "int mask_mode) -> Tensor", _window_attention)


def attention_planes_lp(h, w, kh, kw, sh, sw, mask_mode):
    g = AttnGeom(h, w, kh, kw, sh, sw, mask_mode)
    return int(LIB.um_attention_planes_lp(ctypes.byref(g)))


def _planes_ok(t, name, n, nwin, lp):
    if t.dtype != torch.float16 or not t.is_contiguous() or t.numel() != 2 * n * nwin * lp * 128:
        raise RuntimeError("%s: expected contiguous fp16 planes [2, %d, %d, %d, 128]" % (name, n, nwin, lp))


def _window_attention_planes(qp, kp, vp, n, kv_shift, h, w, kh, kw, sh, sw, mask_mode, out_f32, out_split):
    g = AttnGeom(h, w, kh, kw, sh, sw, mask_mode)
    lp = int(LIB.um_attention_planes_lp(ctypes.byref(g)))
    if lp == 0:
        raise RuntimeError("window_attention_planes: geometry is not built for the tensor-core kernel")
    for t, nm in ((qp, "q_planes"), (kp, "k_planes"), (vp, "v_planes")):
        _planes_ok(t, nm, n, kh * kw, lp)
    ldo, plane = 0, 0
    if out_f32 is not None:
        ldo = _rows(out_f32, "out_f32")
    if out_split is not None:
        if out_split.dtype != torch.float16 or not out_split.is_contiguous() or out_split.shape[0] != 2 or out_split.shape[-1] != 128:
            raise RuntimeError("window_attention_planes: out_split must be contiguous fp16 planes [2, rows, 128]")
        plane = out_split[0].numel()
    _check(LIB.um_window_attention_planes(_p(qp), _p(kp), _p(vp), _p(out_f32), ldo, _p(out_split), plane, n, kv_shift,
                                          ctypes.byref(g), _stream()), "um_window_attention_planes")


window_attention_planes = _define(
    "window_attention_planes(Tensor q_planes, Tensor k_planes, Tensor v_planes, int n_streams, int kv_shift, int h, int w, "
    "int kh, int kw, int sh, int sw, int mask_mode, Tensor(a!)? out_f32, Tensor(b!)? out_split) -> ()",
    _window_attention_planes)


def _softmax_expectation(q, k, values, n_streams, kv_shift, vdim, value_mode, post_op, h, w, kh, kw, mask_mode):
    ldq, ldk = _rows(q, "q"), _rows(k, "k")
    n_total, l, _ = q.shape
    if values is not None:
        _f32c(values, "values")
    out = torch.empty((n_streams, l, vdim), device=q.device, dtype=torch.float32)
    g = AttnGeom(h, w, kh, kw, 0, 0, mask_mode)
    flags = FORCE_CUDA_CORES if _force_cuda_cores else 0
    ws_bytes = 0 if flags else int(LIB.um_softmax_expectation_workspace(ctypes.byref(g), n_total, value_mode))
    ws = torch.empty((ws_bytes,), device=q.device, dtype=torch.uint8) if ws_bytes else None
    _check(LIB.um_softmax_expectation(_p(q), _p(k), _p(values), _p(out), n_streams, n_total, kv_shift, ldq, ldk, vdim,
                                      value_mode, post_op, ctypes.byref(g), _p(ws), ws_bytes, flags, _stream()),
           "um_softmax_expectation")
    return out


softmax_expectation = _define(
    "softmax_expectation(Tensor q, Tensor k, Tensor? values, int n_streams, int kv_shift, int vdim, int value_mode, "
    "int post_op, int h, int w, int kh, int kw, int mask_mode) -> Tensor", _softmax_expectation)


def _local_corr_softmax(f0, f1, h, w, ry, rx, stereo):
    _f32c(f0, "f0"), _f32c(f1, "f1")
    b = f0.shape[0]
    out = torch.empty((b, h, w, 1 if stereo else 2), device=f0.device, dtype=torch.float32)
    _check(LIB.um_local_corr_softmax(_p(f0), _p(f1), _p(out), b, h, w, ry, rx, int(stereo), _stream()),
           "um_local_corr_softmax")
    return out


local_corr_softmax = _define("local_corr_softmax(Tensor f0, Tensor f1, int h, int w, int ry, int rx, bool stereo) -> Tensor",
                             _local_corr_softmax)


def _local_corr_volume(f0, f1, flow, h, w, radius):
    _f32c(f0, "f0"), _f32c(f1, "f1"), _f32c(flow, "flow")
    b = f0.shape[0]
    k = (2 * radius + 1) ** 2
    out = torch.empty((b, h, w, k), device=f0.device, dtype=torch.float32)
    _check(LIB.um_local_corr_volume(_p(f0), _p(f1), _p(flow), _p(out), b, h, w, radius, flow.shape[-1], _stream()),
           "um_local_corr_volume")
    return out


local_corr_volume = _define("local_corr_volume(Tensor f0, Tensor f1, Tensor flow, int h, int w, int radius) -> Tensor",
                            _local_corr_volume)


def _flow_warp(f, flow, h, w):
    _f32c(f, "f"), _f32c(flow, "flow")
    out = torch.empty_like(f)
    _check(LIB.um_flow_warp(_p(f), _p(flow), _p(out), f.shape[0], h, w, flow.shape[-1], _stream()), "um_flow_warp")
    return out


flow_warp = _define("flow_warp(Tensor f, Tensor flow, int h, int w) -> Tensor", _flow_warp)


def _fb_consistency(fwd_flow, bwd_flow, alpha, beta):
    _f32c(fwd_flow, "fwd_flow"), _f32c(bwd_flow, "bwd_flow")
    if fwd_flow.dim() != 4 or fwd_flow.shape[1] != 2 or fwd_flow.shape != bwd_flow.shape:
        raise ValueError("fb_consistency: flows must be planar [B,2,H,W] of equal shape")
    b, _, h, w = fwd_flow.shape
    fwd_occ = torch.empty((b, h, w), device=fwd_flow.device, dtype=torch.float32)
    bwd_occ = torch.empty_like(fwd_occ)
    _check(LIB.um_fb_consistency(_p(fwd_flow), _p(bwd_flow), float(alpha), float(beta), _p(fwd_occ), _p(bwd_occ), b, h, w,
                                 _stream()), "um_fb_consistency")
    return fwd_occ, bwd_occ


fb_consistency = _define("fb_consistency(Tensor fwd_flow, Tensor bwd_flow, float alpha, float beta) -> (Tensor, Tensor)",
                         _fb_consistency)


def _fb_consistency_error(fwd_flow, bwd_flow, alpha, beta):
    _f32c(fwd_flow, "fwd_flow"), _f32c(bwd_flow, "bwd_flow")
    if fwd_flow.dim() != 4 or fwd_flow.shape[1] != 2 or fwd_flow.shape != bwd_flow.shape:
        raise ValueError("fb_consistency_error: flows must be planar [B,2,H,W] of equal shape")
    b, _, h, w = fwd_flow.shape
    fwd_occ = torch.empty((b, h, w), device=fwd_flow.device, dtype=torch.float32)
    bwd_occ, fwd_err = torch.empty_like(fwd_occ), torch.empty_like(fwd_occ)
    _check(LIB.um_fb_consistency_error(_p(fwd_flow), _p(bwd_flow), float(alpha), float(beta), _p(fwd_occ), _p(bwd_occ),
                                       _p(fwd_err), b, h, w, _stream()), "um_fb_consistency_error")
    return fwd_occ, bwd_occ, fwd_err


fb_consistency_error = _define("fb_consistency_error(Tensor fwd_flow, Tensor bwd_flow, float alpha, float beta) -> "
                               "(Tensor, Tensor, Tensor)", _fb_consistency_error)


def _chain_tracks(flow, occ, pos, vis):
    _f32c(flow, "flow"), _f32c(pos, "pos")
    if flow.dim() != 4 or flow.shape[1] != 2:
        raise RuntimeError("chain_tracks: expected planar flows [n, 2, h, w]")
    n, _, h, w = flow.shape
    if occ is not None:
        _f32c(occ, "occ")
        if tuple(occ.shape) != (n, h, w) or occ.device != flow.device:
            raise RuntimeError("chain_tracks: occ must be [n, h, w] on the flows' device")
    if tuple(pos.shape) != (h, w, 2) or pos.device != flow.device:
        raise RuntimeError("chain_tracks: pos must be [h, w, 2] on the flows' device")
    if vis.dtype != torch.uint8 or tuple(vis.shape) != (h, w) or not vis.is_contiguous() or vis.device != flow.device:
        raise RuntimeError("chain_tracks: vis must be contiguous uint8 [h, w] on the flows' device")
    pos_out = torch.empty((n, h, w, 2), device=flow.device, dtype=torch.float32)
    vis_out = torch.empty((n, h, w), device=flow.device, dtype=torch.uint8)
    _check(LIB.um_chain_tracks(_p(flow), _p(occ), n, h, w, _p(pos), _p(vis), _p(pos_out), _p(vis_out), _stream()),
           "um_chain_tracks")
    return pos_out, vis_out


chain_tracks = _define("chain_tracks(Tensor flow, Tensor? occ, Tensor(a!) pos, Tensor(b!) vis) -> (Tensor, Tensor)",
                       _chain_tracks)


def _point_tables(queries, tracks, visible, device):
    _f32c(queries, "queries"), _f32c(tracks, "tracks")
    if queries.dim() != 2 or queries.shape[1] != 3 or queries.device != device:
        raise RuntimeError("track_points: queries must be [nq, 3] on the flows' device")
    nq = queries.shape[0]
    if tracks.dim() != 3 or tracks.shape[0] != nq or tracks.shape[2] != 2 or tracks.device != device:
        raise RuntimeError("track_points: tracks must be [nq, nt, 2] on the flows' device")
    if (visible.dtype != torch.uint8 or tuple(visible.shape) != tuple(tracks.shape[:2]) or not visible.is_contiguous()
            or visible.device != device):
        raise RuntimeError("track_points: visible must be contiguous uint8 [nq, nt] on the flows' device")
    return nq, tracks.shape[1]


def _flows_and_masks(flow, occ, name):
    _f32c(flow, name)
    if flow.dim() != 4 or flow.shape[1] != 2:
        raise RuntimeError("%s: expected planar flows [n, 2, h, w]" % name)
    if occ is not None:
        _f32c(occ, "occ")
        if tuple(occ.shape) != (flow.shape[0],) + tuple(flow.shape[2:]) or occ.device != flow.device:
            raise RuntimeError("%s: occ must be [n, h, w] on the flows' device" % name)
    return flow.shape[0], flow.shape[2], flow.shape[3]


def _track_points_forward(flow, occ, t0, queries, pos, vis, tracks, visible):
    n, h, w = _flows_and_masks(flow, occ, "track_points_forward")
    nq, nt = _point_tables(queries, tracks, visible, flow.device)
    _f32c(pos, "pos")
    if tuple(pos.shape) != (nq, 2) or pos.device != flow.device:
        raise RuntimeError("track_points_forward: pos must be [nq, 2] on the flows' device")
    if vis.dtype != torch.uint8 or tuple(vis.shape) != (nq,) or vis.device != flow.device:
        raise RuntimeError("track_points_forward: vis must be uint8 [nq] on the flows' device")
    _check(LIB.um_track_points_forward(_p(flow), _p(occ), n, h, w, int(t0), _p(queries), nq, nt, _p(pos), _p(vis),
                                       _p(tracks), _p(visible), _stream()), "um_track_points_forward")


track_points_forward = _define("track_points_forward(Tensor flow, Tensor? occ, int t0, Tensor queries, Tensor(a!) pos, "
                               "Tensor(b!) vis, Tensor(c!) tracks, Tensor(d!) visible) -> ()", _track_points_forward)


def _track_points_backward(flow, occ, queries, tracks, visible):
    n, h, w = _flows_and_masks(flow, occ, "track_points_backward")
    nq, nt = _point_tables(queries, tracks, visible, flow.device)
    _check(LIB.um_track_points_backward(_p(flow) if n else None, _p(occ) if n else None, n, h, w, _p(queries), nq, nt,
                                        _p(tracks), _p(visible), _stream()), "um_track_points_backward")


track_points_backward = _define("track_points_backward(Tensor flow, Tensor? occ, Tensor queries, Tensor(a!) tracks, "
                                "Tensor(b!) visible) -> ()", _track_points_backward)


def _multi_flow_tracks(flow, occ, err, src, dst, pos, sig, vis):
    _f32c(flow, "flow"), _f32c(occ, "occ"), _f32c(err, "err"), _f32c(pos, "pos"), _f32c(sig, "sig")
    if flow.dim() != 5 or flow.shape[2] != 2:
        raise RuntimeError("multi_flow_tracks: expected planar flows [n, k, 2, h, w]")
    n, k, _, h, w = flow.shape
    dev = flow.device
    for name, t in (("occ", occ), ("err", err)):
        if tuple(t.shape) != (n, k, h, w) or t.device != dev:
            raise RuntimeError("multi_flow_tracks: %s must be [n, k, h, w] on the flows' device" % name)
    for name, t, shape in (("src", src, (n, k)), ("dst", dst, (n,))):
        if t.dtype != torch.int32 or tuple(t.shape) != shape or not t.is_contiguous() or t.device != dev:
            raise RuntimeError("multi_flow_tracks: %s must be contiguous int32 %s on the flows' device" % (name, list(shape)))
    r = pos.shape[0] if pos.dim() == 4 else -1
    if tuple(pos.shape) != (r, h, w, 2) or pos.device != dev:
        raise RuntimeError("multi_flow_tracks: pos must be [r, h, w, 2] on the flows' device")
    if tuple(sig.shape) != (r, h, w) or sig.device != dev:
        raise RuntimeError("multi_flow_tracks: sig must be [r, h, w] like pos")
    if vis.dtype != torch.uint8 or tuple(vis.shape) != (r, h, w) or not vis.is_contiguous() or vis.device != dev:
        raise RuntimeError("multi_flow_tracks: vis must be contiguous uint8 [r, h, w] like pos")
    tracks = torch.empty((n, h, w, 2), device=dev, dtype=torch.float32)
    visible = torch.empty((n, h, w), device=dev, dtype=torch.uint8)
    sigma = torch.empty((n, h, w), device=dev, dtype=torch.float32)
    _check(LIB.um_multi_flow_tracks(_p(flow), _p(occ), _p(err), _p(src), _p(dst), n, k, h, w, r, _p(pos), _p(sig), _p(vis),
                                    _p(tracks), _p(visible), _p(sigma), _stream()), "um_multi_flow_tracks")
    return tracks, visible, sigma


multi_flow_tracks = _define("multi_flow_tracks(Tensor flow, Tensor occ, Tensor err, Tensor src, Tensor dst, Tensor(a!) pos, "
                            "Tensor(b!) sig, Tensor(c!) vis) -> (Tensor, Tensor, Tensor)", _multi_flow_tracks)


def _propagate_local(q, k, flow, h, w, radius):
    ldq, ldk = _rows(q, "q"), _rows(k, "k")
    _f32c(flow, "flow")
    b = q.shape[0]
    out = torch.empty_like(flow)
    _check(LIB.um_propagate_local(_p(q), _p(k), _p(flow), _p(out), b, h, w, radius, flow.shape[-1], ldq, ldk, _stream()),
           "um_propagate_local")
    return out


propagate_local = _define("propagate_local(Tensor q, Tensor k, Tensor flow, int h, int w, int radius) -> Tensor",
                          _propagate_local)


def _depth_corr_softmax(f0, f1, K, Kinv, pose, cand, h, w, from_argmax):
    for t, n in ((f0, "f0"), (f1, "f1"), (K, "K"), (Kinv, "Kinv"), (pose, "pose"), (cand, "cand")):
        _f32c(t, n)
    b = f0.shape[0]
    out = torch.empty((b, h, w, 1), device=f0.device, dtype=torch.float32)
    _check(LIB.um_depth_corr_softmax(_p(f0), _p(f1), _p(K), _p(Kinv), _p(pose), _p(cand), _p(out), b, h, w,
                                     cand.numel(), int(from_argmax), _stream()), "um_depth_corr_softmax")
    return out


depth_corr_softmax = _define(
    "depth_corr_softmax(Tensor f0, Tensor f1, Tensor K, Tensor Kinv, Tensor pose, Tensor cand, int h, int w, "
    "bool from_argmax) -> Tensor", _depth_corr_softmax)


def _add_position(x, table, h, w):
    _f32c(x, "x"), _f32c(table, "table")
    out = torch.empty_like(x)
    _check(LIB.um_add_position(_p(x), _p(table), _p(out), x.shape[0], h, w, table.shape[0], table.shape[1], _stream()),
           "um_add_position")
    return out


add_position = _define("add_position(Tensor x, Tensor table, int h, int w) -> Tensor", _add_position)


def _convex_upsample(flow, mask, factor, mult):
    _f32c(flow, "flow"), _f32c(mask, "mask")
    b, h, w, fd = flow.shape
    out = torch.empty((b, fd, h * factor, w * factor), device=flow.device, dtype=torch.float32)
    _check(LIB.um_convex_upsample(_p(flow), _p(mask), _p(out), b, h, w, fd, factor, float(mult), _stream()),
           "um_convex_upsample")
    return out


convex_upsample = _define("convex_upsample(Tensor flow, Tensor mask, int factor, float mult) -> Tensor", _convex_upsample)


def _upsample2x(flow, mult):
    _f32c(flow, "flow")
    b, h, w, fd = flow.shape
    out = torch.empty((b, 2 * h, 2 * w, fd), device=flow.device, dtype=torch.float32)
    _check(LIB.um_upsample2x(_p(flow), _p(out), b, h, w, fd, float(mult), _stream()), "um_upsample2x")
    return out


upsample2x = _define("upsample2x(Tensor flow, float mult) -> Tensor", _upsample2x)


def _resize_bilinear(x, h_out, w_out, scale, flip_x):
    _f32c(x, "x")
    if x.dim() != 4 or x.shape[1] > 3:
        raise RuntimeError("resize_bilinear: expected planar [B, C <= 3, H, W]")
    b, c, h, w = x.shape
    out = torch.empty((b, c, h_out, w_out), device=x.device, dtype=torch.float32)
    sc = (ctypes.c_float * c)(*scale) if scale is not None else None
    _check(LIB.um_resize_bilinear(_p(x), _p(out), b, c, h, w, h_out, w_out, sc, int(flip_x), _stream()), "um_resize_bilinear")
    return out


resize_bilinear = _define("resize_bilinear(Tensor x, int h_out, int w_out, float[]? scale, bool flip_x) -> Tensor", _resize_bilinear)


def _frames_to_planar(frames, h_out, w_out, transpose):
    if not frames.is_cuda or frames.dtype != torch.uint8 or frames.dim() != 4 or frames.shape[-1] != 3 or not frames.is_contiguous():
        raise RuntimeError("frames_to_planar: expected contiguous CUDA uint8 frames [T, H, W, 3]")
    t, h, w, _ = frames.shape
    out = torch.empty((t, 3, h_out, w_out), device=frames.device, dtype=torch.float32)
    _check(LIB.um_frames_to_planar(_p(frames), _p(out), t, h, w, int(transpose), h_out, w_out, _stream()), "um_frames_to_planar")
    return out


frames_to_planar = _define("frames_to_planar(Tensor frames, int h_out, int w_out, bool transpose) -> Tensor", _frames_to_planar)


def _frames_to_planar_normalized(frames, h_out, w_out, mean, std):
    if not frames.is_cuda or frames.dtype != torch.uint8 or frames.dim() != 4 or frames.shape[-1] != 3 or not frames.is_contiguous():
        raise RuntimeError("frames_to_planar_normalized: expected contiguous CUDA uint8 frames [T, H, W, 3]")
    if len(mean) != 3 or len(std) != 3:
        raise RuntimeError("frames_to_planar_normalized: expected 3 means and 3 stds")
    t, h, w, _ = frames.shape
    out = torch.empty((t, 3, h_out, w_out), device=frames.device, dtype=torch.float32)
    m, s = (ctypes.c_float * 3)(*mean), (ctypes.c_float * 3)(*std)
    _check(LIB.um_frames_to_planar_normalized(_p(frames), _p(out), t, h, w, h_out, w_out, m, s, _stream()),
           "um_frames_to_planar_normalized")
    return out


frames_to_planar_normalized = _define(
    "frames_to_planar_normalized(Tensor frames, int h_out, int w_out, float[] mean, float[] std) -> Tensor",
    _frames_to_planar_normalized)


def _flow_to_image(flow, out):
    _f32c(flow, "flow")
    if flow.dim() != 4 or flow.shape[1] != 2:
        raise RuntimeError("flow_to_image: expected planar flow [N, 2, H, W]")
    n, _, h, w = flow.shape
    if out.dtype != torch.uint8 or tuple(out.shape) != (n, h, w, 3) or out.stride(-1) != 1 or (w > 1 and out.stride(2) != 3) \
            or out.device != flow.device:
        raise RuntimeError("flow_to_image: out must be uint8 [N, H, W, 3] on the flow's device with 3-byte pixels")
    scratch = torch.empty((n,), device=flow.device, dtype=torch.float32)
    _check(LIB.um_flow_to_image(_p(flow), _p(out), out.stride(1), out.stride(0), _p(scratch), n, h, w, _stream()),
           "um_flow_to_image")


flow_to_image = _define("flow_to_image(Tensor flow, Tensor(a!) out) -> ()", _flow_to_image)


def _disparity_to_image(disp, out):
    _f32c(disp, "disp")
    if disp.dim() != 3:
        raise RuntimeError("disparity_to_image: expected disparities [N, H, W]")
    n, h, w = disp.shape
    if out.dtype != torch.uint8 or tuple(out.shape) != (n, h, w, 3) or out.stride(-1) != 1 or (w > 1 and out.stride(2) != 3) \
            or out.device != disp.device:
        raise RuntimeError("disparity_to_image: out must be uint8 [N, H, W, 3] on the disparity's device with 3-byte pixels")
    scratch = torch.empty((2 * n,), device=disp.device, dtype=torch.float32)
    _check(LIB.um_disparity_to_image(_p(disp), _p(out), out.stride(1), out.stride(0), _p(scratch), n, h, w, _stream()),
           "um_disparity_to_image")


disparity_to_image = _define("disparity_to_image(Tensor disp, Tensor(a!) out) -> ()", _disparity_to_image)


def _ragged_items(items, name):
    if not items.is_cuda or items.dtype != torch.uint8 or items.dim() != 2 or items.shape[1] != RAGGED_ITEM_BYTES \
            or not items.is_contiguous() or not 1 <= items.shape[0] <= 65535:
        raise RuntimeError("%s: items must be a contiguous CUDA uint8 table [1..65535, %d]" % (name, RAGGED_ITEM_BYTES))
    return items.shape[0]


def _frames_to_planar_normalized_ragged(frames, items, h_max, w_max, h_out, w_out, mean, std):
    if not frames.is_cuda or frames.dtype != torch.uint8 or not frames.is_contiguous() or frames.numel() == 0:
        raise RuntimeError("frames_to_planar_normalized_ragged: expected contiguous CUDA uint8 packed frames")
    if len(mean) != 3 or len(std) != 3:
        raise RuntimeError("frames_to_planar_normalized_ragged: expected 3 means and 3 stds")
    n = _ragged_items(items, "frames_to_planar_normalized_ragged")
    out = torch.empty((n, 3, h_out, w_out), device=frames.device, dtype=torch.float32)
    m, s = (ctypes.c_float * 3)(*mean), (ctypes.c_float * 3)(*std)
    _check(LIB.um_frames_to_planar_normalized_ragged(_p(frames), frames.numel(), _p(items), _p(out), n, h_max, w_max, h_out,
                                                     w_out, m, s, _stream()), "um_frames_to_planar_normalized_ragged")
    return out


frames_to_planar_normalized_ragged = _define(
    "frames_to_planar_normalized_ragged(Tensor frames, Tensor items, int h_max, int w_max, int h_out, int w_out, float[] mean, "
    "float[] std) -> Tensor", _frames_to_planar_normalized_ragged)


def _resize_bilinear_ragged(x, items, h_max, w_max, out_numel):
    _f32c(x, "x")
    if x.dim() != 4 or x.shape[1] != 1:
        raise RuntimeError("resize_bilinear_ragged: expected planar [n, 1, H, W]")
    n = _ragged_items(items, "resize_bilinear_ragged")
    if x.shape[0] != n or out_numel < 1:
        raise RuntimeError("resize_bilinear_ragged: one item per image and a positive output size")
    out = torch.empty((out_numel,), device=x.device, dtype=torch.float32)
    _check(LIB.um_resize_bilinear_ragged(_p(x), _p(out), out_numel, _p(items), n, x.shape[2], x.shape[3], h_max, w_max,
                                         _stream()), "um_resize_bilinear_ragged")
    return out


resize_bilinear_ragged = _define("resize_bilinear_ragged(Tensor x, Tensor items, int h_max, int w_max, int out_numel) -> Tensor",
                                 _resize_bilinear_ragged)


def _disparity_to_image_ragged(disp, items, out, h_max, w_max):
    _f32c(disp, "disp")
    if out.dtype != torch.uint8 or not out.is_contiguous() or out.device != disp.device or out.numel() < 3 * disp.numel():
        raise RuntimeError("disparity_to_image_ragged: out must be contiguous uint8 of 3 bytes per disparity on its device")
    n = _ragged_items(items, "disparity_to_image_ragged")
    scratch = torch.empty((2 * n,), device=disp.device, dtype=torch.float32)
    _check(LIB.um_disparity_to_image_ragged(_p(disp), disp.numel(), _p(items), _p(out), _p(scratch), n, h_max, w_max, _stream()),
           "um_disparity_to_image_ragged")


disparity_to_image_ragged = _define("disparity_to_image_ragged(Tensor disp, Tensor items, Tensor(a!) out, int h_max, int w_max) -> ()",
                                    _disparity_to_image_ragged)


def _frames_to_planar_ragged(frames, items, h_max, w_max, h_out, w_out):
    if not frames.is_cuda or frames.dtype != torch.uint8 or not frames.is_contiguous() or frames.numel() == 0:
        raise RuntimeError("frames_to_planar_ragged: expected contiguous CUDA uint8 packed frames")
    n = _ragged_items(items, "frames_to_planar_ragged")
    out = torch.empty((n, 3, h_out, w_out), device=frames.device, dtype=torch.float32)
    _check(LIB.um_frames_to_planar_ragged(_p(frames), frames.numel(), _p(items), _p(out), n, h_max, w_max, h_out, w_out,
                                          _stream()), "um_frames_to_planar_ragged")
    return out


frames_to_planar_ragged = _define(
    "frames_to_planar_ragged(Tensor frames, Tensor items, int h_max, int w_max, int h_out, int w_out) -> Tensor",
    _frames_to_planar_ragged)


def _flow_to_image_ragged(flow, flow_items, out, picture_items, h_max, w_max):
    _f32c(flow, "flow")
    if out.dtype != torch.uint8 or not out.is_contiguous() or out.device != flow.device or out.numel() == 0:
        raise RuntimeError("flow_to_image_ragged: out must be contiguous uint8 on the flow's device")
    n = _ragged_items(flow_items, "flow_to_image_ragged")
    if _ragged_items(picture_items, "flow_to_image_ragged") != n:
        raise RuntimeError("flow_to_image_ragged: one picture item per flow item")
    scratch = torch.empty((n,), device=flow.device, dtype=torch.float32)
    _check(LIB.um_flow_to_image_ragged(_p(flow), flow.numel(), _p(flow_items), _p(out), out.numel(), _p(picture_items),
                                       _p(scratch), n, h_max, w_max, _stream()), "um_flow_to_image_ragged")


flow_to_image_ragged = _define(
    "flow_to_image_ragged(Tensor flow, Tensor flow_items, Tensor(a!) out, Tensor picture_items, int h_max, int w_max) -> ()",
    _flow_to_image_ragged)


def _fb_consistency_ragged(flow, flow_items, occ, occ_items, h_max, w_max, alpha, beta):
    _f32c(flow, "flow"), _f32c(occ, "occ")
    n2 = _ragged_items(flow_items, "fb_consistency_ragged")
    if _ragged_items(occ_items, "fb_consistency_ragged") != n2 or n2 % 2 or occ.device != flow.device:
        raise RuntimeError("fb_consistency_ragged: two flow items and two mask items per pair, on one device")
    _check(LIB.um_fb_consistency_ragged(_p(flow), flow.numel(), _p(flow_items), float(alpha), float(beta), _p(occ), occ.numel(),
                                        _p(occ_items), n2 // 2, h_max, w_max, _stream()), "um_fb_consistency_ragged")


fb_consistency_ragged = _define(
    "fb_consistency_ragged(Tensor flow, Tensor flow_items, Tensor(a!) occ, Tensor occ_items, int h_max, int w_max, float alpha, "
    "float beta) -> ()", _fb_consistency_ragged)

DEPTH_TO_IMAGE_SCRATCH_WORDS = 2056


def _depth_to_image(depth, out):
    _f32c(depth, "depth")
    if depth.dim() != 3:
        raise RuntimeError("depth_to_image: expected depths [N, H, W]")
    n, h, w = depth.shape
    if out.dtype != torch.uint8 or tuple(out.shape) != (n, h, w, 3) or out.stride(-1) != 1 or (w > 1 and out.stride(2) != 3) \
            or out.device != depth.device:
        raise RuntimeError("depth_to_image: out must be uint8 [N, H, W, 3] on the depth's device with 3-byte pixels")
    scratch = torch.empty((DEPTH_TO_IMAGE_SCRATCH_WORDS * n,), device=depth.device, dtype=torch.int32)
    _check(LIB.um_depth_to_image(_p(depth), _p(out), out.stride(1), out.stride(0), _p(scratch), n, h, w, _stream()),
           "um_depth_to_image")


depth_to_image = _define("depth_to_image(Tensor depth, Tensor(a!) out) -> ()", _depth_to_image)


def _depth_to_image_ragged(depth, items, out, h_max, w_max):
    _f32c(depth, "depth")
    if out.dtype != torch.uint8 or not out.is_contiguous() or out.device != depth.device or out.numel() < 3 * depth.numel():
        raise RuntimeError("depth_to_image_ragged: out must be contiguous uint8 of 3 bytes per depth on its device")
    n = _ragged_items(items, "depth_to_image_ragged")
    scratch = torch.empty((DEPTH_TO_IMAGE_SCRATCH_WORDS * n,), device=depth.device, dtype=torch.int32)
    _check(LIB.um_depth_to_image_ragged(_p(depth), depth.numel(), _p(items), _p(out), _p(scratch), n, h_max, w_max, _stream()),
           "um_depth_to_image_ragged")


depth_to_image_ragged = _define("depth_to_image_ragged(Tensor depth, Tensor items, Tensor(a!) out, int h_max, int w_max) -> ()",
                                _depth_to_image_ragged)

SUBMIT_CROP, SUBMIT_RESIZE = 0, 1
SUBMIT_FLO, SUBMIT_KITTI_FLOW_PNG, SUBMIT_KITTI_DISP_PNG, SUBMIT_PFM = 0, 1, 2, 3
SUBMIT_CHANNELS = {SUBMIT_FLO: 2, SUBMIT_KITTI_FLOW_PNG: 2, SUBMIT_KITTI_DISP_PNG: 1, SUBMIT_PFM: 1}


def submission_payload_bytes(fmt, h, w):
    if fmt == SUBMIT_FLO:
        return 8 * h * w
    if fmt == SUBMIT_PFM:
        return 4 * h * w
    if fmt == SUBMIT_KITTI_FLOW_PNG:
        return h * (1 + 6 * w)
    if fmt == SUBMIT_KITTI_DISP_PNG:
        return h * (1 + 2 * w)
    raise RuntimeError("encode_submission: unknown format %r" % (fmt,))


def _encode_submission(pred, fmt, out_h, out_w, resize, top, left):
    _f32c(pred, "pred")
    if pred.dim() != 4:
        raise RuntimeError("encode_submission: expected planar predictions [B, C, h, w]")
    if fmt not in SUBMIT_CHANNELS or pred.shape[1] != SUBMIT_CHANNELS[fmt]:
        raise RuntimeError("encode_submission: format %r needs [B, %s, h, w]" % (fmt, SUBMIT_CHANNELS.get(fmt, "?")))
    b, c, h, w = pred.shape
    nbytes = submission_payload_bytes(fmt, out_h, out_w)
    out = torch.empty((b, nbytes), device=pred.device, dtype=torch.uint8)
    _check(LIB.um_encode_submission(_p(pred), b, c, h, w, SUBMIT_RESIZE if resize else SUBMIT_CROP, top, left, out_h, out_w,
                                    fmt, _p(out), nbytes, _stream()), "um_encode_submission")
    return out


encode_submission = _define(
    "encode_submission(Tensor pred, int fmt, int out_h, int out_w, bool resize, int top, int left) -> Tensor",
    _encode_submission)


def _eval_stats(pred, gt, valid, noc_valid, task, mask_mode, max_val, eval_min, eval_max):
    if task not in EVAL_COLS:
        raise RuntimeError("eval_stats: unknown task %d" % task)
    nd = 4 if task == EVAL_FLOW else 3
    if pred.dim() != nd or (nd == 4 and pred.shape[1] != 2):
        raise RuntimeError("eval_stats: expected pred [B, 2, h, w] for flow and [B, h, w] otherwise")
    if not pred.is_cuda or pred.dtype != torch.float32:
        raise RuntimeError("eval_stats: pred must be a float32 CUDA tensor")
    _f32c(gt, "gt")
    if gt.shape != pred.shape or gt.device != pred.device:
        raise RuntimeError("eval_stats: gt must have the prediction's shape and device")
    b, h, w = pred.shape[0], pred.shape[-2], pred.shape[-1]
    for t, name in ((valid, "valid"), (noc_valid, "noc_valid")):
        if t is not None:
            _f32c(t, name)
            if tuple(t.shape) != (b, h, w) or t.device != pred.device:
                raise RuntimeError("eval_stats: %s must be [B, h, w] on the prediction's device" % name)
    sb, sy, sx = pred.stride(0), pred.stride(-2), pred.stride(-1)
    sc = pred.stride(1) if nd == 4 else 0
    cols = len(EVAL_COLS[task])
    scratch = torch.empty((b * EVAL_PARTS * cols,), device=pred.device, dtype=torch.float64)
    out = torch.empty((b, cols), device=pred.device, dtype=torch.float64)
    _check(LIB.um_eval_stats(_p(pred), sb, sc, sy, sx, _p(gt), _p(valid), _p(noc_valid), task, mask_mode, float(max_val),
                             float(eval_min), float(eval_max), b, h, w, _p(scratch), _p(out), _stream()), "um_eval_stats")
    return out


eval_stats = _define(
    "eval_stats(Tensor pred, Tensor gt, Tensor? valid, Tensor? noc_valid, int task, int mask_mode, float max_val, "
    "float eval_min, float eval_max) -> Tensor", _eval_stats)


def prep_conv_weight(w, cin_splits, cout_p):
    cout, _, kh, kw = w.shape
    cols, off = [], 0
    for c in cin_splits:
        cp = (c + 63) // 64 * 64
        ws = w[:, off:off + c].permute(0, 2, 3, 1)
        ws = torch.nn.functional.pad(ws, (0, cp - c)).reshape(cout, kh * kw * cp)
        cols.append(ws)
        off += c
    m = torch.cat(cols, dim=1)
    m = torch.nn.functional.pad(m, (0, 0, 0, cout_p - cout)).float()
    hi = m.half()
    lo = (m - hi.float()).half()
    return torch.stack((hi, lo), dim=0).contiguous()


def split_buffer(batch, h, w, cp, device):
    return torch.zeros((2, batch, h, w, cp), device=device, dtype=torch.float16)


def _split_planes(src, dst, off):
    _f32c(src, "src", rows_ok=True)
    s2 = src.flatten(0, -2)
    rows, c = s2.shape
    cp = dst.shape[-1]
    if dst.dtype != torch.float16 or not dst.is_contiguous() or dst.shape[0] != 2 or dst[0].numel() < rows * cp:
        raise RuntimeError("split_planes: dst must be contiguous fp16 planes [2, >= rows, cp]")
    _check(LIB.um_split_planes(_p(s2), rows, c, s2.stride(0), _p(dst), cp, off, dst[0].numel(), _stream()), "um_split_planes")


split_planes = _define("split_planes(Tensor src, Tensor(a!) dst, int off) -> ()", _split_planes)


def _conv2d_tc(src0, src1, weights, bias, kh, kw, pad_h, pad_w, cout, bn, mode, act, out_f32, off_f32, out_split,
               off_split, aux0, aux1, gamma=None, beta=None, stride=1, rows=0, win_dst=None, win_geom=None, win_c0=0,
               win_c1=0, win_streams=0, pre=None):
    d = ConvDesc()
    if rows:
        if rows % 16 or src0.dim() != 3 or rows > src0.shape[1]:
            raise RuntimeError("conv2d_tc: rows must be a multiple of 16 within the [2, R, cp] source planes")
        b, h, w, cp0 = 1, rows // 16, 16, src0.shape[-1]
        d.src_plane_stride = src0.stride(0)
        if src1 is not None and (src1.shape[1] != src0.shape[1] or src1.stride(0) != src0.stride(0)):
            raise RuntimeError("conv2d_tc: both sources must have the same number of rows and the same plane stride")
        if out_split is not None:
            d.split_plane_stride = out_split.stride(0)
    else:
        _, b, h, w, cp0 = src0.shape
    d.src[0] = src0.data_ptr(); d.cin_p[0] = cp0
    d.nsrc = 1
    if src1 is not None:
        d.src[1] = src1.data_ptr(); d.cin_p[1] = src1.shape[-1]; d.nsrc = 2
    d.batch, d.h, d.w = b, h, w
    d.weights = weights.data_ptr()
    d.bias = bias.data_ptr() if bias is not None else None
    d.kh, d.kw, d.pad_h, d.pad_w = kh, kw, pad_h, pad_w
    d.stride = stride
    d.cout, d.cout_p, d.bn = cout, weights.shape[1], bn
    d.mode, d.act = mode, act
    if out_f32 is not None:
        _f32c(out_f32, "out_f32", rows_ok=True)
        d.out_f32 = out_f32.data_ptr(); d.ld_f32 = out_f32.stride(-2); d.off_f32 = off_f32
    if out_split is not None:
        d.out_split = out_split.data_ptr(); d.cp_split = out_split.shape[-1]; d.off_split = off_split
    if aux0 is not None:
        d.aux0 = aux0.data_ptr(); d.ld_aux0 = aux0.stride(-2)
    if aux1 is not None:
        d.aux1 = aux1.data_ptr(); d.ld_aux1 = aux1.stride(-2)
    if gamma is not None:
        d.gamma = gamma.data_ptr(); d.beta = beta.data_ptr()
    if pre is not None:
        _f32c(pre, "pre", rows_ok=True)
        d.pre = pre.data_ptr(); d.ld_pre = pre.stride(-2)
    if win_dst is not None:
        g = AttnGeom(*win_geom)
        lp = int(LIB.um_attention_planes_lp(ctypes.byref(g)))
        nops = (win_c1 - win_c0) // 128
        if win_dst.dtype != torch.float16 or not win_dst.is_contiguous() or lp == 0 or \
                win_dst.numel() != nops * 2 * win_streams * g.kh * g.kw * lp * 128:
            raise RuntimeError("conv2d_tc: win_dst must be contiguous fp16 planes [ops, 2, streams, windows, lp, 128]")
        d.win_dst = win_dst.data_ptr(); d.win_geom = g; d.win_lp = lp
        d.win_c0, d.win_c1, d.win_streams = win_c0, win_c1, win_streams
    _check(LIB.um_conv2d_tc(ctypes.byref(d), _stream()), "um_conv2d_tc")


conv2d_tc = _define(
    "conv2d_tc(Tensor src0, Tensor? src1, Tensor weights, Tensor? bias, int kh, int kw, int pad_h, int pad_w, int cout, "
    "int bn, int mode, int act, Tensor(a!)? out_f32, int off_f32, Tensor(b!)? out_split, int off_split, Tensor? aux0, "
    "Tensor? aux1, Tensor? gamma=None, Tensor? beta=None, int stride=1, int rows=0, Tensor(c!)? win_dst=None, "
    "int[]? win_geom=None, int win_c0=0, int win_c1=0, int win_streams=0, Tensor? pre=None) -> ()", _conv2d_tc)


def ffn_tc_supported(rows):
    return rows > 0 and rows % 256 == 0


def _ffn_tc(src0, src1, w1, w2, residual, gamma, beta, out_f32, out_split, rows):
    for t, name in ((src0, "src0"), (src1, "src1")):
        if t.dtype != torch.float16 or t.dim() != 3 or t.shape[0] != 2 or t.shape[-1] != 128 or t.stride(-1) != 1 or \
                t.stride(1) != 128 or rows > t.shape[1]:
            raise RuntimeError("ffn_tc: %s must be fp16 planes [2, R >= rows, 128]" % name)
    if src1.stride(0) != src0.stride(0):
        raise RuntimeError("ffn_tc: both sources must have the same plane stride")
    hidden = w1.shape[1]
    if w1.shape[0] != 2 or w1.shape[2] != 256 or tuple(w2.shape) != (2, 128, hidden) or not w1.is_contiguous() or not w2.is_contiguous():
        raise RuntimeError("ffn_tc: w1 must be [2, hidden, 256] and w2 [2, 128, hidden] prepared planes")
    d = FfnDesc()
    d.src[0] = src0.data_ptr(); d.src[1] = src1.data_ptr(); d.src_plane_stride = src0.stride(0)
    d.rows = rows; d.w1 = w1.data_ptr(); d.w2 = w2.data_ptr(); d.hidden = hidden
    if residual is not None:
        _f32c(residual, "residual", rows_ok=True)
        d.residual = residual.data_ptr(); d.ld_res = residual.stride(-2)
    d.gamma = gamma.data_ptr(); d.beta = beta.data_ptr()
    if out_f32 is not None:
        _f32c(out_f32, "out_f32", rows_ok=True)
        d.out_f32 = out_f32.data_ptr(); d.ld_f32 = out_f32.stride(-2)
    if out_split is not None:
        if out_split.dtype != torch.float16 or out_split.shape[0] != 2 or out_split.shape[-1] != 128 or out_split.stride(1) != 128:
            raise RuntimeError("ffn_tc: out_split must be fp16 planes [2, R, 128]")
        d.out_split = out_split.data_ptr(); d.split_plane_stride = out_split.stride(0)
    _check(LIB.um_ffn_tc(ctypes.byref(d), _stream()), "um_ffn_tc")


ffn_tc = _define(
    "ffn_tc(Tensor src0, Tensor src1, Tensor w1, Tensor w2, Tensor? residual, Tensor gamma, Tensor beta, "
    "Tensor(a!)? out_f32, Tensor(b!)? out_split, int rows) -> ()", _ffn_tc)


def _instance_norm_stats(x):
    _f32c(x, "x", rows_ok=True)
    n, c = x.shape[0], x.shape[-1]
    hw = x[0].numel() // c
    scratch = torch.empty((int(LIB.um_instance_norm_scratch_floats(n, c)),), device=x.device, dtype=torch.float32)
    stats = torch.empty((n, 2, c), device=x.device, dtype=torch.float32)
    _check(LIB.um_instance_norm_stats(_p(x), x.stride(-2), n, hw, c, _p(scratch), _p(stats), _stream()),
           "um_instance_norm_stats")
    return stats


instance_norm_stats = _define("instance_norm_stats(Tensor x) -> Tensor", _instance_norm_stats)


def _instance_norm_apply(a, stats_a, relu_a, res, stats_res, relu_out, out_f32, out_split, off):
    _f32c(a, "a", rows_ok=True)
    n, c = a.shape[0], a.shape[-1]
    hw = a[0].numel() // c
    _check(LIB.um_instance_norm_apply(_p(a), a.stride(-2), _p(stats_a), int(relu_a), _p(res),
                                      res.stride(-2) if res is not None else 0, _p(stats_res), int(relu_out), _p(out_f32),
                                      out_f32.stride(-2) if out_f32 is not None else 0, _p(out_split),
                                      out_split.shape[-1] if out_split is not None else 0, off, n, hw, c, _stream()),
           "um_instance_norm_apply")


instance_norm_apply = _define(
    "instance_norm_apply(Tensor a, Tensor? stats_a, bool relu_a, Tensor? res, Tensor? stats_res, bool relu_out, "
    "Tensor(a!)? out_f32, Tensor(b!)? out_split, int off) -> ()", _instance_norm_apply)


def _conv7x7_small(in0, in1, nchw, weight, bias, stride, relu, scale, shift, out_f32, out_split):
    _f32c(in0, "in0"), _f32c(weight, "weight")
    if nchw:
        n0, cin, h, w = in0.shape
        n = n0 + (in1.shape[0] if in1 is not None else 0)
    else:
        n, h, w, cin = in0.shape
        n0 = n
    cout = weight.shape[0]
    sc = (ctypes.c_float * 3)(*scale) if scale is not None else None
    sh = (ctypes.c_float * 3)(*shift) if shift is not None else None
    _check(LIB.um_conv7x7_small(_p(in0), _p(in1), int(nchw), n0, n, h, w, cin, stride, _p(weight), _p(bias), cout, int(relu),
                                sc, sh, _p(out_f32), out_f32.stride(-2) if out_f32 is not None else 0, _p(out_split),
                                out_split.shape[-1] if out_split is not None else 0, _stream()), "um_conv7x7_small")


conv7x7_small = _define(
    "conv7x7_small(Tensor in0, Tensor? in1, bool nchw, Tensor weight, Tensor? bias, int stride, bool relu, float[]? scale, "
    "float[]? shift, Tensor(a!)? out_f32, Tensor(b!)? out_split) -> ()", _conv7x7_small)
```

### unimatch_b200/unimatch.py

```python
import math
from collections import namedtuple
from contextlib import contextmanager

import torch
import torch.nn as nn

from . import ops
from .spec import param_spec

_OPS = torch.ops.unimatch_sm100


class _Layer(namedtuple("_Layer", "weights bias kh kw pad_h pad_w stride cout bn mode act gamma beta k")):
    __slots__ = ()

    def out_hw(self, h, w, stride):
        return (h + 2 * self.pad_h - self.kh) // stride + 1, (w + 2 * self.pad_w - self.kw) // stride + 1


def _layer(w, cin_splits, bn, bias=None, act=ops.ACT_NONE, mode=ops.CONV_LINEAR, gamma=None, beta=None, stride=1):
    if w.dim() == 2:
        w = w[:, :, None, None]
    cout, cin, kh, kw = w.shape
    return _Layer(ops.prep_conv_weight(w, cin_splits, (cout + bn - 1) // bn * bn), bias, kh, kw, kh // 2, kw // 2, stride,
                  cout, bn, mode, act, gamma, beta, cin * kh * kw)


class _Node(nn.Module):
    """Parameter container; gives the flat spec table the reference's dotted state_dict names."""


def _attach(root, key, param):
    parts = key.split(".")
    node = root
    for name in parts[:-1]:
        if name not in node._modules:
            node.add_module(name, _Node())
        node = node._modules[name]
    node.register_parameter(parts[-1], param)


def _sine_table(wh, ww):
    y = torch.arange(1, wh + 1, dtype=torch.float32)
    x = torch.arange(1, ww + 1, dtype=torch.float32)
    y = y / (float(wh) + 1e-6) * (2 * math.pi)
    x = x / (float(ww) + 1e-6) * (2 * math.pi)
    n = torch.arange(64, dtype=torch.float32)
    dim_t = 10000 ** (2 * torch.div(n, 2, rounding_mode="floor") / 64)
    even = (torch.arange(64) % 2 == 0)

    def enc(v):
        a = v[:, None] / dim_t
        return torch.where(even, a.sin(), a.cos())

    ey, ex = enc(y), enc(x)
    return torch.cat((ey[:, None, :].expand(wh, ww, 64), ex[None, :, :].expand(wh, ww, 64)), dim=2).contiguous()


def _ceil16(n):
    return (n + 15) // 16 * 16


class UniMatch(nn.Module):
    def __init__(self, num_scales=1, feature_channels=128, upsample_factor=8, num_head=1, ffn_dim_expansion=4,
                 num_transformer_layers=6, reg_refine=False, task="flow"):
        super().__init__()
        if feature_channels != 128:
            raise ValueError("libunimatch_sm100 is built for feature_channels=128 (main_flow.py:73)")
        if num_head != 1:
            raise NotImplementedError("multi-head attention is not implemented (as in transformer.py:63-66)")
        self.feature_channels = feature_channels
        self.num_scales = num_scales
        self.upsample_factor = upsample_factor
        self.reg_refine = reg_refine
        self.num_transformer_layers = num_transformer_layers
        self.task_built = task
        self._spec = param_spec(num_scales, feature_channels, upsample_factor, num_head, ffn_dim_expansion,
                                num_transformer_layers, reg_refine, task)
        for key, shape in self._spec.items():
            _attach(self, key, nn.Parameter(self._init_tensor(key, shape)))
        self._prep_key = None
        self._prep = None
        self._tables = {}
        self._cands = {}
        self._attn_ws = {}
        self._pad_ws = {}
        self.training = False
        self.kernel_timer = None

    @staticmethod
    def _init_tensor(key, shape):
        t = torch.empty(shape)
        if len(shape) == 4:
            nn.init.kaiming_normal_(t, mode="fan_out", nonlinearity="relu")
        elif len(shape) == 2:
            nn.init.xavier_uniform_(t)
        elif ".norm" in key:
            t.fill_(1.0 if key.endswith("weight") else 0.0)
        else:
            t.uniform_(-0.05, 0.05)
        return t

    def train(self, mode=True):
        if mode:
            raise NotImplementedError("unimatch_b200.UniMatch is inference-only (use .eval(); training stays on the reference)")
        return super().train(False)

    def _prepared(self):
        params = dict(self.named_parameters())
        key = (tuple((p._version, p.data_ptr()) for p in params.values()),)
        if self._prep_key == key:
            return self._prep
        w = {k: v.detach() for k, v in params.items()}
        LN = ops.CONV_LN
        P = {"raw": w, "blocks": []}
        for i in range(self.num_transformer_layers):
            sk, ck = "transformer.layers.%d.self_attn." % i, "transformer.layers.%d.cross_attn_ffn." % i
            w_in = torch.cat([w[sk + "q_proj.weight"], w[sk + "k_proj.weight"], w[sk + "v_proj.weight"],
                              w[ck + "k_proj.weight"], w[ck + "v_proj.weight"]], dim=0)
            hid = w[ck + "mlp.0.weight"].shape[0]
            P["blocks"].append(dict(
                tc_in=_layer(w_in, [128], 128),
                tc_m_s=_layer(w[sk + "merge.weight"], [128], 128, mode=LN, gamma=w[sk + "norm1.weight"], beta=w[sk + "norm1.bias"]),
                tc_q_c=_layer(w[ck + "q_proj.weight"], [128], 128),
                tc_m_c=_layer(w[ck + "merge.weight"], [128], 128, mode=LN, gamma=w[ck + "norm1.weight"], beta=w[ck + "norm1.bias"]),
                tc_w1=_layer(w[ck + "mlp.0.weight"], [128, 128], 256, act=ops.ACT_GELU),
                tc_w2=_layer(w[ck + "mlp.2.weight"], [hid], 128, mode=LN, gamma=w[ck + "norm2.weight"], beta=w[ck + "norm2.bias"])))
        P["tcb"] = self._prepare_backbone(w, self.num_scales)
        qw, qb = w["feature_flow_attn.q_proj.weight"], w["feature_flow_attn.q_proj.bias"]
        kw, kb = w["feature_flow_attn.k_proj.weight"], w["feature_flow_attn.k_proj.bias"]
        P["prop_q"] = _layer(qw, [128], 128, qb.contiguous())
        P["prop_k"] = _layer(kw, [128], 128, kb.contiguous())
        P["prop_qk"] = _layer(torch.cat([qw, kw], 0), [128], 128, torch.cat([qb, kb]).contiguous())
        if self.reg_refine:
            P["tc"] = self._prepare_refine(w)
        if "upsampler.0.weight" in w:
            w0 = w["upsampler.0.weight"]
            w0 = torch.cat([w0[:, 2:], w0[:, :2]], dim=1)
            w2 = w["upsampler.2.weight"]
            P["up"] = dict(c0=_layer(w0, [130], 128, w["upsampler.0.bias"], act=ops.ACT_RELU),
                           c2=_layer(w2, [256], 192 if w2.shape[0] % 192 == 0 else 64, w["upsampler.2.bias"]))
        self._prep_key, self._prep = key, P
        return P

    @staticmethod
    def _prepare_backbone(w, num_scales):
        first_stride = {"layer2": 2, "layer3": 2 if num_scales == 1 else 1}
        T = {}
        for key, wt in w.items():
            if not key.startswith("backbone.") or not key.endswith(".weight") or key == "backbone.conv1.weight":
                continue
            name = key[:-7]
            part = name.split(".")
            stride = first_stride.get(part[1], 1) if part[2:3] == ["0"] and part[3] in ("conv1", "downsample") else 1
            bn = 128 if wt.shape[0] > 64 else 64
            T[name] = _layer(wt, [wt.shape[1]], bn, w.get(name + ".bias"), stride=stride)
        return T

    @staticmethod
    def _prepare_refine(w):
        R = ops.ACT_RELU
        T = {}
        pw, pb = w["refine_proj.weight"], w["refine_proj.bias"]
        T["proj_net"] = _layer(pw[:128], [128], 128, pb[:128].contiguous(), act=ops.ACT_TANH)
        T["proj_inp"] = _layer(pw[128:], [128], 128, pb[128:].contiguous(), act=R)
        e = "refine.encoder."
        T["convc1"] = _layer(w[e + "convc1.weight"], [81], 256, w[e + "convc1.bias"], act=R)
        T["convc2"] = _layer(w[e + "convc2.weight"], [256], 96, w[e + "convc2.bias"], act=R)
        T["convf2"] = _layer(w[e + "convf2.weight"], [128], 64, w[e + "convf2.bias"], act=R)
        T["conv"] = _layer(w[e + "conv.weight"], [256], 128, w[e + "conv.bias"], act=R)
        g = "refine.gru.conv"
        Z, Q = ops.CONV_GRU_ZR, ops.CONV_GRU_Q
        for sfx in ("1", "2"):
            wzr = torch.cat([w[g + "z%s.weight" % sfx], w[g + "r%s.weight" % sfx]], 0)
            bzr = torch.cat([w[g + "z%s.bias" % sfx], w[g + "r%s.bias" % sfx]])
            wq, bq = w[g + "q%s.weight" % sfx], w[g + "q%s.bias" % sfx]
            if sfx == "1":
                T["zr1_fix"] = _layer(wzr[:, :256], [128, 128], 128, bzr)
                T["zr1_var"] = _layer(wzr[:, 256:], [128], 128, mode=Z)
            else:
                T["zr2_fix"] = _layer(wzr[:, 128:256], [128], 128, bzr)
                T["zr2_var"] = _layer(torch.cat([wzr[:, :128], wzr[:, 256:]], 1), [128, 128], 128, mode=Z)
            T["q%s_fix" % sfx] = _layer(wq[:, 128:256], [128], 128, bq)
            T["q%s_var" % sfx] = _layer(torch.cat([wq[:, :128], wq[:, 256:]], 1), [128, 128], 128, mode=Q)
        T["fh1"] = _layer(w["refine.flow_head.conv1.weight"], [128], 128, w["refine.flow_head.conv1.bias"], act=R)
        T["fh2"] = _layer(w["refine.flow_head.conv2.weight"], [256], 16, w["refine.flow_head.conv2.bias"])
        if "refine.mask.0.weight" in w:
            T["mask0"] = _layer(w["refine.mask.0.weight"], [128], 128, w["refine.mask.0.bias"], act=R)
            T["mask2"] = _layer(w["refine.mask.2.weight"], [256], 64, w["refine.mask.2.bias"])
        return T

    def _pos_table(self, wh, ww, device):
        k = (wh, ww, str(device))
        if k not in self._tables:
            self._tables[k] = _sine_table(wh, ww).to(device)
        return self._tables[k]

    @contextmanager
    def _section(self, name):
        t = self.kernel_timer
        if t is None:
            yield
            return
        e0, e1 = torch.cuda.Event(enable_timing=True), torch.cuda.Event(enable_timing=True)
        e0.record()
        yield
        e1.record()
        t.setdefault("_events", []).append(("sec:" + name, e0, e1, 0.0))

    def _timed(self, tag, flops, fn, *a):
        t = self.kernel_timer
        if t is None:
            return fn(*a)
        e0, e1 = torch.cuda.Event(enable_timing=True), torch.cuda.Event(enable_timing=True)
        e0.record()
        out = fn(*a)
        e1.record()
        t.setdefault("_events", []).append((tag, e0, e1, flops))
        return out

    def _conv(self, layer, src0, src1=None, stride=None, rows=0, out_f32=None, off_f32=0, out_split=None, off_split=0,
              aux0=None, aux1=None, **kw):
        stride = layer.stride if stride is None else stride

        def launch():
            _OPS.conv2d_tc(src0=src0, src1=src1, weights=layer.weights, bias=layer.bias, kh=layer.kh, kw=layer.kw,
                           pad_h=layer.pad_h, pad_w=layer.pad_w, cout=layer.cout, bn=layer.bn, mode=layer.mode, act=layer.act,
                           out_f32=out_f32, off_f32=off_f32, out_split=out_split, off_split=off_split, aux0=aux0, aux1=aux1,
                           gamma=layer.gamma, beta=layer.beta, stride=stride, rows=rows, **kw)
        if self.kernel_timer is None:
            return launch()
        pix = rows or src0.shape[1] * math.prod(layer.out_hw(src0.shape[2], src0.shape[3], stride))
        return self._timed("conv", 2.0 * pix * layer.cout * layer.k, launch)

    def _stage_backbone(self, P, img0, img1, normalise):
        T = P["tcb"]
        dev = img0.device
        nb = img0.shape[0] + (img1.shape[0] if img1 is not None else 0)
        C, IS, IA = self._conv, _OPS.instance_norm_stats, _OPS.instance_norm_apply
        pad64 = lambda c: (c + 63) // 64 * 64

        nplanes = [0]

        def planes(h, w, c):
            cp = pad64(c)
            if cp == c:
                return torch.empty((2, nb, h, w, cp), device=dev, dtype=torch.float16)
            nplanes[0] += 1
            return self._zero_padded("backbone%d" % nplanes[0], (2, nb, h, w, cp), dev)

        def conv(src_s, name, h, w, stride=None):
            layer = T[name]
            out = torch.empty((nb, *layer.out_hw(h, w, layer.stride if stride is None else stride), layer.cout), device=dev)
            C(layer, src_s, out_f32=out, stride=stride)
            return out

        hh, ww = img0.shape[2], img0.shape[3]
        a = torch.empty((nb, (hh - 1) // 2 + 1, (ww - 1) // 2 + 1, 64), device=dev)
        if normalise:
            mean, std = (0.485, 0.456, 0.406), (0.229, 0.224, 0.225)
            scale = [1.0 / (255.0 * s_) for s_ in std]
            shift = [-m_ / s_ for m_, s_ in zip(mean, std)]
        else:
            scale = shift = None
        _OPS.conv7x7_small(img0, img1, True, P["raw"]["backbone.conv1.weight"], None, 2, False, scale, shift, a, None)
        h, w = a.shape[1], a.shape[2]
        cur_f = torch.empty((nb, h, w, 64), device=dev)
        cur_s = planes(h, w, 64)
        IA(a, IS(a), True, None, None, False, cur_f, cur_s, 0)
        for li in (1, 2, 3):
            for bi in range(2):
                pf = "backbone.layer%d.%d." % (li, bi)
                a1 = conv(cur_s, pf + "conv1", h, w)
                _, ho, wo, cout = a1.shape
                t_s = planes(ho, wo, cout)
                IA(a1, IS(a1), True, None, None, False, None, t_s, 0)
                a2 = conv(t_s, pf + "conv2", ho, wo)
                if (pf + "downsample.0") in T:
                    res = conv(cur_s, pf + "downsample.0", h, w)
                    st_res = IS(res)
                else:
                    res, st_res = cur_f, None
                out_f = torch.empty((nb, ho, wo, cout), device=dev)
                out_s = planes(ho, wo, cout)
                IA(a2, IS(a2), True, res, st_res, True, out_f, out_s, 0)
                cur_f, cur_s, h, w = out_f, out_s, ho, wo
        x6 = torch.empty((nb, h, w, 128), device=dev)
        x6_s = planes(h, w, 128) if self.num_scales > 1 else None
        C(T["backbone.conv2"], cur_s, out_f32=x6, out_split=x6_s)
        if self.num_scales == 1:
            return [x6]
        strides = (1, 2, 4, 8)[:self.num_scales]
        feats = [conv(x6_s, "backbone.trident_conv", h, w, stride=s) for s in strides]
        return feats[::-1]

    @staticmethod
    def _attn_plan(attn_type, splits, h, w, layer_idx):
        shift = ("swin" in attn_type) and splits > 1 and layer_idx % 2 == 1
        full2d = (1, 1, 0, 0, ops.MASK_NONE)
        if splits > 1:
            wh, ww = h // splits, w // splits
            swin2d = (splits, splits, wh // 2 if shift else 0, ww // 2 if shift else 0,
                      ops.MASK_SWIN if shift else ops.MASK_NONE)
            swin1d = (h, splits, 0, ww // 2 if shift else 0, ops.MASK_SWIN if shift else ops.MASK_NONE)
        full1d = (h, 1, 0, 0, ops.MASK_NONE)
        if attn_type == "swin" and splits > 1:
            return swin2d, swin2d
        if attn_type == "self_swin2d_cross_1d":
            return (swin2d if splits > 1 else full2d), full1d
        if attn_type == "self_swin2d_cross_swin1d":
            return (swin2d if splits > 1 else full2d), (swin1d if splits > 1 else full1d)
        return full2d, full2d

    def _zero_padded(self, tag, shape, dev):
        key = (tag, tuple(shape), str(dev))
        buf = self._pad_ws.get(key)
        if buf is None:
            if len(self._pad_ws) >= 24:
                self._pad_ws.clear()
            buf = torch.zeros(shape, device=dev, dtype=torch.float16)
            self._pad_ws[key] = buf
        return buf

    def _attn_planes(self, dev, n, h, w, kh, kw, lp):
        key = (str(dev), n, h, w, kh, kw, lp)
        buf = self._attn_ws.get(key)
        if buf is None:
            if len(self._attn_ws) >= 4:
                self._attn_ws.clear()
            buf = torch.zeros((6, 2, n, kh * kw, lp, 128), device=dev, dtype=torch.float16)
            self._attn_ws[key] = buf
        return buf

    def cached_buffers(self):
        return list(self._attn_ws.values()) + list(self._pad_ws.values())

    def _stage_transformer(self, P, x, h, w, attn_type, splits, tag="s0"):
        n, l, c = x.shape
        half = n // 2
        rows = n * l
        rp = _ceil16(rows)
        dev = x.device
        G = self._conv
        mk = torch.empty if rp == rows else torch.zeros
        planes = lambda cp: mk((2, rp, cp), device=dev, dtype=torch.float16)
        f32 = lambda cols: mk((rp, cols), device=dev)
        tok = lambda t, c0, c1: t[:rows].view(n, l, t.shape[-1])[:, :, c0:c1]
        hid = P["blocks"][0]["tc_w1"].cout
        x_f, xo_f, x1_f = f32(c), f32(c), f32(c)
        x_s, xo_s, x1_s, msg_s, m_s = planes(c), planes(c), planes(c), planes(c), planes(c)
        fused_ffn = ops.ffn_tc_supported(rp)
        hid_s = None if fused_ffn else planes(hid)
        x_f[:rows] = x.reshape(rows, c)
        _OPS.split_planes(x_f, x_s, 0)
        y = q_f = None
        for i, blk in enumerate(P["blocks"]):
            geo_s, geo_c = self._attn_plan(attn_type, splits, h, w, i)
            gs, gc = (h, w) + geo_s, (h, w) + geo_c
            lp_s = ops.attention_planes_lp(*gs)
            lp_c = ops.attention_planes_lp(*gc) if geo_c == geo_s else 0
            ws = self._attn_planes(dev, n, h, w, geo_s[0], geo_s[1], lp_s) if lp_s else None
            win_c1 = 640 if lp_c else (384 if lp_s else 0)
            if win_c1 < 640 and y is None:
                y = f32(5 * c)
            G(blk["tc_in"], x_s, rows=rp, out_f32=y if win_c1 < 640 else None, win_dst=ws[:win_c1 // 128] if win_c1 else None,
              win_geom=gs if win_c1 else None, win_c1=win_c1, win_streams=n)
            fl_s, fl_c = (4.0 * (l // (g[0] * g[1])) * l * 128 * n for g in (geo_s, geo_c))
            if lp_s:
                self._timed("attn:" + tag, fl_s, _OPS.window_attention_planes, ws[0], ws[1], ws[2], n, 0, *gs, None, msg_s)
            else:
                msg = self._timed("attn_simt:" + tag, fl_s, _OPS.window_attention, tok(y, 0, 128), tok(y, 128, 256), tok(y, 256, 384), 0, *gs)
                _OPS.split_planes(msg.view(rows, c), msg_s, 0)
            G(blk["tc_m_s"], msg_s, rows=rp, out_f32=x1_f, out_split=x1_s, aux0=x_f)
            if lp_c:
                G(blk["tc_q_c"], x1_s, rows=rp, win_dst=ws[5:6], win_geom=gc, win_c1=128, win_streams=n)
                self._timed("attn:" + tag, fl_c, _OPS.window_attention_planes, ws[5], ws[3], ws[4], n, half, *gc, None, msg_s)
            else:
                if q_f is None:
                    q_f = f32(c)
                G(blk["tc_q_c"], x1_s, rows=rp, out_f32=q_f)
                msg = self._timed("attn_simt:" + tag, fl_c, _OPS.window_attention, tok(q_f, 0, 128), tok(y, 384, 512), tok(y, 512, 640), half, *gc)
                _OPS.split_planes(msg.view(rows, c), msg_s, 0)
            G(blk["tc_m_c"], msg_s, rows=rp, out_split=m_s)
            w1, w2 = blk["tc_w1"], blk["tc_w2"]
            if fused_ffn:
                self._timed("conv", 2.0 * rp * hid * (2 * c + c), _OPS.ffn_tc, x1_s, m_s, w1.weights, w2.weights, x1_f,
                            w2.gamma, w2.beta, xo_f, xo_s, rp)
            else:
                G(w1, x1_s, m_s, rows=rp, out_split=hid_s)
                G(w2, hid_s, rows=rp, out_f32=xo_f, out_split=xo_s, aux0=x1_f)
            x_f, xo_f, x_s, xo_s = xo_f, x_f, xo_s, x_s
        return x_f[:rows].view(n, l, c), x_s

    def _stage_features(self, f0, f1, flow, h, wd, splits):
        Bp, c = f0.shape[0], f0.shape[-1]
        if flow is not None:
            f1 = _OPS.flow_warp(f1.contiguous(), flow.contiguous(), h, wd)
        table = self._pos_table(h // splits, wd // splits, f0.device)
        tok = torch.cat((f0, f1), dim=0).view(2 * Bp, h, wd, c)
        return _OPS.add_position(tok, table, h, wd).view(2 * Bp, h * wd, c)

    def _stage_correlation(self, tok, Bp, h, wd, task, radius, pred_bidir_flow=False, depth=None):
        t0, t1 = tok[:Bp], tok[Bp:]
        if task == "depth":
            cams, from_argmax, bidir = depth
            if bidir:
                q0, q1 = torch.cat((t0, t1), 0).contiguous(), torch.cat((t1, t0), 0).contiguous()
            else:
                q0, q1 = t0.contiguous(), t1.contiguous()
            return _OPS.depth_corr_softmax(q0, q1, cams["K"].contiguous(), cams["K_inv"].contiguous(),
                                           cams["pose"].contiguous(), cams["cand"], h, wd, bool(from_argmax))
        if radius == -1:
            if task == "flow":
                ns = 2 * Bp if pred_bidir_flow else Bp
                return _OPS.softmax_expectation(tok, tok, None, ns, Bp, 2, ops.VALUE_COORDS, ops.POST_MINUS_OWN,
                                                h, wd, 1, 1, ops.MASK_NONE).view(ns, h, wd, 2)
            if task == "stereo":
                return _OPS.softmax_expectation(tok, tok, None, Bp, Bp, 1, ops.VALUE_XCOORD, ops.POST_OWN_MINUS,
                                                h, wd, h, 1, ops.MASK_CAUSAL).view(Bp, h, wd, 1)
            raise NotImplementedError
        if task == "flow":
            return _OPS.local_corr_softmax(t0.contiguous(), t1.contiguous(), h, wd, radius, radius, False)
        if task == "stereo":
            return _OPS.local_corr_softmax(t0.contiguous(), t1.contiguous(), h, wd, 0, radius, True)
        raise NotImplementedError

    def _stage_propagation(self, P, x_s, flow, nb, h, wd, prop_r):
        dev = flow.device
        L = h * wd
        rows = nb * L
        rq = rows if rows % 16 == 0 else x_s.shape[1]
        G = self._conv
        fd = flow.shape[-1]
        flow = flow.contiguous()
        if prop_r > 0:
            qk = torch.empty((rq, 256), device=dev)
            G(P["prop_qk"], x_s, rows=rq, out_f32=qk)
            qk = qk[:rows].view(nb, L, 256)
            return _OPS.propagate_local(qk[:, :, :128], qk[:, :, 128:], flow, h, wd, prop_r)
        q = torch.empty((rq, 128), device=dev)
        q_s = torch.empty((2, rq, 128), device=dev, dtype=torch.float16)
        k = torch.empty((rq, 128), device=dev)
        G(P["prop_q"], x_s, rows=rq, out_f32=q, out_split=q_s)
        G(P["prop_k"], q_s, rows=rq, out_f32=k)
        return _OPS.softmax_expectation(q[:rows].view(nb, L, 128), k[:rows].view(nb, L, 128), flow.view(nb, L, fd), nb, 0, fd,
                                        ops.VALUE_TENSOR, ops.POST_NONE, h, wd, 1, 1, ops.MASK_NONE).view(nb, h, wd, fd)

    class _RefineState:
        pass

    def _stage_refine_setup(self, P, feat0, b, h, w):
        T = P["tc"]
        dev = feat0.device
        st = self._RefineState()
        z16 = lambda cp: torch.empty((2, b, h, w, cp), device=dev, dtype=torch.float16)
        st.corr_s = self._zero_padded("corr", (2, b, h, w, 128), dev)
        st.cor1_s, st.cf_s, st.flo1_s = z16(256), z16(256), z16(128)
        st.inp_s, st.mfx_s = z16(128), z16(128)
        st.h0_s, st.h1_s, st.h2_s, st.rh_s, st.fh_s = z16(128), z16(128), z16(128), z16(128), z16(256)
        f0_s = z16(128)
        _OPS.split_planes(feat0, f0_s, 0)
        f32 = lambda cc: torch.empty((b, h, w, cc), device=dev)
        st.net0, st.z, st.h1, st.h2 = f32(128), f32(128), f32(128), f32(128)
        C = self._conv
        C(T["proj_net"], f0_s, out_f32=st.net0, out_split=st.h0_s)
        C(T["proj_inp"], f0_s, out_split=st.inp_s)
        st.pre_zr1, st.pre_q1, st.pre_zr2, st.pre_q2 = f32(256), f32(128), f32(256), f32(128)
        C(T["zr1_fix"], st.h0_s, st.inp_s, out_f32=st.pre_zr1)
        C(T["q1_fix"], st.inp_s, out_f32=st.pre_q1)
        C(T["zr2_fix"], st.inp_s, out_f32=st.pre_zr2)
        C(T["q2_fix"], st.inp_s, out_f32=st.pre_q2)
        return st

    def _update_block(self, P, st, corr, flow, want_mask):
        T, w = P["tc"], P["raw"]
        fd = T["fh2"].cout
        C = self._conv
        b, h, wd, _ = corr.shape
        dev = corr.device
        _OPS.split_planes(corr, st.corr_s, 0)
        C(T["convc1"], st.corr_s, out_split=st.cor1_s)
        C(T["convc2"], st.cor1_s, out_split=st.cf_s)
        _OPS.conv7x7_small(flow, None, False, w["refine.encoder.convf1.weight"], w["refine.encoder.convf1.bias"], 1, True,
                           None, None, None, st.flo1_s)
        C(T["convf2"], st.flo1_s, out_split=st.cf_s, off_split=192)
        C(T["conv"], st.cf_s, out_split=st.mfx_s)
        _OPS.split_planes(flow, st.mfx_s, 128 - fd)
        C(T["zr1_var"], st.mfx_s, out_f32=st.z, out_split=st.rh_s, aux0=st.net0, pre=st.pre_zr1)
        C(T["q1_var"], st.rh_s, st.mfx_s, out_f32=st.h1, out_split=st.h1_s, aux0=st.net0, aux1=st.z, pre=st.pre_q1)
        C(T["zr2_var"], st.h1_s, st.mfx_s, out_f32=st.z, out_split=st.rh_s, aux0=st.h1, pre=st.pre_zr2)
        C(T["q2_var"], st.rh_s, st.mfx_s, out_f32=st.h2, out_split=st.h2_s, aux0=st.h1, aux1=st.z, pre=st.pre_q2)
        C(T["fh1"], st.h2_s, out_split=st.fh_s)
        delta = torch.empty((b, h, wd, fd), device=dev)
        C(T["fh2"], st.fh_s, out_f32=delta)
        mask = None
        if want_mask and "mask0" in T:
            C(T["mask0"], st.h2_s, out_split=st.fh_s)
            mask = torch.empty((b, h, wd, T["mask2"].cout), device=dev)
            C(T["mask2"], st.fh_s, out_f32=mask)
        return st.h2, mask, delta

    def _stage_refine_iter(self, P, rst, g0, g1, flow, task, want_mask, depth=None):
        h, wd = flow.shape[1], flow.shape[2]
        if task == "depth":
            cams, min_depth, max_depth = depth
            cflow = self._rigid_flow(flow, cams["K"].float(), cams["K_inv"].float(), cams["pose"].float(), h, wd)
        else:
            cflow = flow.contiguous()
        with self._section("refine_corr_volume"):
            corr = _OPS.local_corr_volume(g0, g1, cflow, h, wd, 4)
        with self._section("refine_update_block"):
            _, mask, delta = self._update_block(P, rst, corr, flow.contiguous(), want_mask)
        if task == "depth":
            flow = (flow - delta).clamp(min=min_depth, max=max_depth)
        else:
            flow = flow + delta
        if task == "stereo":
            flow = flow.clamp(min=0)
        return flow, mask

    def _stage_upsample_learned(self, P, flow2, feat, factor, mult):
        U = P["up"]
        b, h, w, _ = feat.shape
        dev = feat.device
        src = self._zero_padded("upsampler", (2, b, h, w, 192), dev)
        _OPS.split_planes(feat.contiguous(), src, 0)
        _OPS.split_planes(flow2.contiguous(), src, 128)
        mid = torch.empty((2, b, h, w, 256), device=dev, dtype=torch.float16)
        self._conv(U["c0"], src, out_split=mid)
        m = torch.empty((b, h, w, U["c2"].cout), device=dev)
        self._conv(U["c2"], mid, out_f32=m)
        return _OPS.convex_upsample(flow2.contiguous(), m, factor, float(mult))

    @staticmethod
    def _rigid_flow(inv_depth, K, K_inv, pose, h, w):
        b = inv_depth.shape[0]
        dev = inv_depth.device
        ys, xs = torch.meshgrid(torch.arange(h, device=dev, dtype=torch.float32),
                                torch.arange(w, device=dev, dtype=torch.float32), indexing="ij")
        grid = torch.stack([xs, ys, torch.ones_like(xs)], dim=0).view(1, 3, -1).expand(b, 3, h * w)
        depth = (1.0 / inv_depth.view(b, 1, h * w))
        pts = K_inv.bmm(grid) * depth
        pts = torch.bmm(pose[:, :3, :3], pts) + pose[:, :3, -1:]
        proj = torch.bmm(K, pts)
        z = proj[:, 2:3].clamp(min=1e-3)
        uv = proj[:, :2] / z - grid[:, :2]
        return uv.view(b, 2, h, w).permute(0, 2, 3, 1).contiguous()

    def forward(self, img0, img1, attn_type=None, attn_splits_list=None, corr_radius_list=None, prop_radius_list=None,
                num_reg_refine=1, pred_bidir_flow=False, task="flow", intrinsics=None, pose=None,
                min_depth=1. / 0.5, max_depth=1. / 10, num_depth_candidates=64, depth_from_argmax=False,
                pred_bidir_depth=False, **kwargs):
        if self.training:
            raise NotImplementedError("unimatch_b200.UniMatch is inference-only; call .eval()")
        with torch.no_grad():
            P = self._prepared()
            B = img0.shape[0]
            with self._section("backbone"):
                feats = self._stage_backbone(P, img0.float().contiguous(), img1.float().contiguous(), task == "flow")
            return self._forward_encoded(P, [f[:B] for f in feats], [f[B:] for f in feats], attn_type, attn_splits_list,
                                         corr_radius_list, prop_radius_list, num_reg_refine, pred_bidir_flow, task, None,
                                         intrinsics, pose, min_depth, max_depth, num_depth_candidates, depth_from_argmax,
                                         pred_bidir_depth)

    def depth_cameras(self, intrinsics, pose, up, min_depth, max_depth, num_depth_candidates, pred_bidir_depth):
        dev = intrinsics.device
        Ks = intrinsics.clone().float()
        Ks[:, :2] = Ks[:, :2] / up
        B = Ks.shape[0]
        if pred_bidir_depth:
            K = Ks.repeat(2, 1, 1)
            pc = pose.float() if pose.shape[0] == 2 * B else torch.cat((pose, torch.inverse(pose)), dim=0).float()
        else:
            K, pc = Ks, pose.float()
        key = (float(min_depth), float(max_depth), int(num_depth_candidates), str(dev))
        cand = self._cands.get(key)
        if cand is None:
            cand = self._cands[key] = torch.linspace(min_depth, max_depth, num_depth_candidates).float().to(dev)
        return {"Ks": Ks, "K": K, "K_inv": torch.inverse(K), "pose": pc, "cand": cand}

    def encode_frames(self, frames, task="flow"):
        if self.training:
            raise NotImplementedError("unimatch_b200.UniMatch is inference-only; call .eval()")
        if task not in ("flow", "stereo", "depth"):
            raise ValueError("encode_frames: unknown task %r" % (task,))
        with torch.no_grad():
            P = self._prepared()
            with self._section("backbone"):
                return self._stage_backbone(P, frames.float().contiguous(), None, task == "flow")

    def forward_encoded(self, feats0, feats1, attn_type=None, attn_splits_list=None, corr_radius_list=None,
                        prop_radius_list=None, num_reg_refine=1, pred_bidir_flow=False, task="flow", cameras=None,
                        intrinsics=None, pose=None, min_depth=1. / 0.5, max_depth=1. / 10, num_depth_candidates=64,
                        depth_from_argmax=False, pred_bidir_depth=False, **kwargs):
        if self.training:
            raise NotImplementedError("unimatch_b200.UniMatch is inference-only; call .eval()")
        if task not in ("flow", "depth"):
            raise ValueError("forward_encoded drives the flow and depth tasks only (each stereo pair encodes two distinct views)")
        if len(feats0) != self.num_scales or len(feats1) != self.num_scales:
            raise ValueError("forward_encoded needs one feature map per scale (%d)" % self.num_scales)
        with torch.no_grad():
            return self._forward_encoded(self._prepared(), list(feats0), list(feats1), attn_type, attn_splits_list,
                                         corr_radius_list, prop_radius_list, num_reg_refine, pred_bidir_flow, task, cameras,
                                         intrinsics, pose, min_depth, max_depth, num_depth_candidates, depth_from_argmax,
                                         pred_bidir_depth)

    def _forward_encoded(self, P, feats0, feats1, attn_type, attn_splits_list, corr_radius_list, prop_radius_list,
                         num_reg_refine, pred_bidir_flow, task, cams, intrinsics, pose, min_depth, max_depth,
                         num_depth_candidates, depth_from_argmax, pred_bidir_depth):
        assert task == "flow" or not pred_bidir_flow
        if task == "depth":
            assert self.num_scales == 1 and len(attn_splits_list) == len(prop_radius_list) == 1
            if cams is None:
                if intrinsics is None or pose is None:
                    raise ValueError("the depth task needs intrinsics= and pose= (or, in forward_encoded, cameras=)")
                cams = self.depth_cameras(intrinsics, pose, self.upsample_factor, min_depth, max_depth, num_depth_candidates,
                                          pred_bidir_depth)
            streams = (2 if pred_bidir_depth else 1) * feats0[0].shape[0]
            if cams["K"].shape[0] != streams or cams["pose"].shape[0] != streams:
                raise ValueError("the depth cameras were built for another batch or pred_bidir_depth setting")
        else:
            assert len(attn_splits_list) == len(corr_radius_list) == len(prop_radius_list) == self.num_scales
            cams, pred_bidir_depth, depth_from_argmax = None, False, False
        flow = None
        preds = []
        for s in range(self.num_scales):
            f0, f1 = feats0[s], feats1[s]
            _, h, wd, c = f0.shape
            if pred_bidir_flow and s > 0:
                f0, f1 = torch.cat((f0, f1), dim=0), torch.cat((f1, f0), dim=0)
            f0_ori, f1_ori = f0, f1
            Bp = f0.shape[0]
            if s > 0:
                flow = _OPS.upsample2x(flow.contiguous(), 2.0)
            splits = attn_splits_list[s]
            prop_r = prop_radius_list[s]
            tok = self._stage_features(f0, f1, flow, h, wd, splits)
            with self._section("transformer_s%d" % s):
                tok, tok_s = self._stage_transformer(P, tok, h, wd, attn_type, splits, "s%d" % s)

            with self._section("correlation_s%d" % s):
                dargs = (cams, depth_from_argmax, pred_bidir_depth) if task == "depth" else None
                pred = self._stage_correlation(tok, Bp, h, wd, task, None if task == "depth" else corr_radius_list[s],
                                               pred_bidir_flow, dargs)
            flow = flow + pred if flow is not None else pred
            if task == "stereo":
                flow = flow.clamp(min=0)

            bidir0 = (pred_bidir_flow or pred_bidir_depth) and s == 0
            nb = 2 * Bp if bidir0 else Bp
            with self._section("propagation_s%d" % s):
                flow = self._stage_propagation(P, tok_s, flow, nb, h, wd, prop_r)
            if s != self.num_scales - 1:
                continue

            feat0 = tok[:nb].reshape(nb, h, wd, c)
            if self.reg_refine:
                assert num_reg_refine > 0
                g0, g1 = f0_ori.contiguous(), f1_ori.contiguous()
                drefine = None
                if task == "depth":
                    if pred_bidir_depth:
                        g0, g1 = torch.cat((g0, g1), dim=0), torch.cat((g1, g0), dim=0)
                    drefine = (cams, min_depth, max_depth)
                rst = self._stage_refine_setup(P, feat0.contiguous(), nb, h, wd)
                for it in range(num_reg_refine):
                    flow, mask = self._stage_refine_iter(P, rst, g0, g1, flow, task, it == num_reg_refine - 1, drefine)

            up = self.upsample_factor
            if task == "depth":
                out = self._stage_upsample_learned(P, torch.cat((flow, torch.zeros_like(flow)), -1), feat0, up,
                                                   1).clamp(min=min_depth, max=max_depth)[:, :1]
            elif self.reg_refine:
                out = _OPS.convex_upsample(flow.contiguous(), mask, up, float(up))
            elif task == "stereo":
                out = -self._stage_upsample_learned(P, torch.cat((-flow, torch.zeros_like(flow)), -1), feat0, up, up)[:, :1]
            else:
                out = self._stage_upsample_learned(P, flow, feat0, up, up)
            preds.append(out)

        if task == "stereo":
            preds = [p.squeeze(1) for p in preds]
        if task == "depth":
            preds = [1.0 / p.squeeze(1) for p in preds]
        return {"flow_preds": preds}
```

Measured before the change: 85.27.

## Fuse InstanceNorm statistics into conv epilogues via per-tile partials

After: 86.41 (median of 6 runs). 1.3% higher.

```diff
diff --git a/include/unimatch_sm100.h b/include/unimatch_sm100.h
--- a/include/unimatch_sm100.h
+++ b/include/unimatch_sm100.h
@@ -242,7 +242,10 @@
   um_attn_geom win_geom;
   const float* pre;
   int64_t ld_pre;
+  float* in_partial;
 } um_conv_desc;
+#define UM_CONV_TILE_H 8
+#define UM_CONV_TILE_W 16
 int um_conv2d_tc(const um_conv_desc* desc, void* stream);
 
 typedef struct um_ffn_desc {
@@ -267,6 +270,12 @@
                      int32_t cin, int32_t stride, const float* weight, const float* bias, int32_t cout, int32_t relu,
                      const float* scale, const float* shift, float* out_f32, int64_t ld_out, void* out_split, int32_t cp,
                      void* stream);
+int um_conv7x7_small_partials(const float* in0, const float* in1, int32_t nchw, int32_t n_half, int32_t n, int32_t h,
+                              int32_t w, int32_t cin, int32_t stride, const float* weight, const float* bias, int32_t cout,
+                              int32_t relu, const float* scale, const float* shift, float* out_f32, int64_t ld_out,
+                              void* out_split, int32_t cp, float* in_partial, void* stream);
+#define UM_STEM_TILE_H 8
+#define UM_STEM_TILE_W 32
 
 int64_t um_instance_norm_scratch_floats(int32_t n, int32_t c);
 int um_instance_norm_stats(const float* x, int64_t ld, int32_t n, int32_t hw, int32_t c, float* scratch, float* stats,
@@ -274,6 +283,8 @@
 int um_instance_norm_apply(const float* a, int64_t ld_a, const float* stats_a, int32_t relu_a, const float* res,
                            int64_t ld_res, const float* stats_res, int32_t relu_out, float* out_f32, int64_t ld_o,
                            void* out_split, int32_t cp, int32_t off, int32_t n, int32_t hw, int32_t c, void* stream);
+int um_instance_norm_finalize(const float* partial, int32_t n, int32_t h, int32_t w, int32_t tile_h, int32_t tile_w,
+                              int32_t c, float* stats, void* stream);
 
 int um_split_planes(const float* src, int64_t rows, int32_t channels, int64_t ld, void* dst, int32_t cp, int32_t off,
                     int64_t dst_plane_stride, void* stream);
diff --git a/unimatch_b200/csrc/um_conv_tc.cu b/unimatch_b200/csrc/um_conv_tc.cu
--- a/unimatch_b200/csrc/um_conv_tc.cu
+++ b/unimatch_b200/csrc/um_conv_tc.cu
@@ -10,6 +10,7 @@
 namespace {
 
 constexpr int TW = 16, TH = 8;
+static_assert(TW == UM_CONV_TILE_W && TH == UM_CONV_TILE_H, "the InstanceNorm partials' tile grid is part of the ABI");
 __host__ __device__ constexpr int stages_for(int bn) { return bn >= 96 ? 2 : 3; }
 constexpr int NTHREADS = 512;
 constexpr int EPILOGUE = 8;
@@ -42,6 +43,7 @@
   int win_c0, win_c1, win_lp;
   long long win_tokens, win_L;
   Geom win_g;
+  float* in_partial;
 };
 
 __device__ __forceinline__ float sigmoid_fast(float y) { return __fdividef(1.0f, 1.0f + __expf(-y)); }
@@ -363,6 +365,48 @@
         reinterpret_cast<int*>(coef + 256)[(lt & 1) * 128 + r] = drow;
       }
       epi_sync();
+
+      if constexpr (!WIN && (BN == 64 || BN == 128) && MODE == UM_CONV_LINEAR && ACT == UM_ACT_NONE) {
+        if (p.in_partial) {
+          mbar_wait_inline(acc_full, lt & 1);
+          const int co = n0 + r;
+          if (r < BN && co < p.cout) {
+            const float* col = accs + (r >> 5) * 4096 + (r & 3);
+            const int piece = (r & 31) >> 2;
+            const float bb = sbias[r];
+            const int vh = min(TH, p.H - y0), vw = min(TW, p.W - x0);
+            const float shift = col[piece << 2] + bb;
+            float sr[TH], qr[TH];
+#pragma unroll
+            for (int yy = 0; yy < TH; ++yy) { sr[yy] = 0.f; qr[yy] = 0.f; }
+            auto add = [&](int yy, int xx) {
+              const float d = (col[(yy * TW + xx) * 32 + ((piece ^ (xx & 7)) << 2)] + bb) - shift;
+              sr[yy] += d;
+              qr[yy] = fmaf(d, d, qr[yy]);
+            };
+            if (vh == TH && vw == TW) {
+#pragma unroll
+              for (int xx = 0; xx < TW; ++xx)
+#pragma unroll
+                for (int yy = 0; yy < TH; ++yy) add(yy, xx);
+            } else {
+#pragma unroll 1
+              for (int xx = 0; xx < vw; ++xx)
+#pragma unroll
+                for (int yy = 0; yy < TH; ++yy)
+                  if (yy < vh) add(yy, xx);
+            }
+            float s = sr[0], q = qr[0];
+#pragma unroll
+            for (int yy = 1; yy < TH; ++yy) { s += sr[yy]; q += qr[yy]; }
+            const int per_img = p.tiles_x * p.tiles_y;
+            float* dst = p.in_partial + ((long long)b * per_img + (t / p.tiles_n) % per_img) * 3 * p.cout + co;
+            dst[0] = shift;
+            dst[p.cout] = s;
+            dst[2 * p.cout] = q;
+          }
+        }
+      }
 
       constexpr int CH = BN < 32 ? BN : 32;
 #pragma unroll 1
@@ -606,6 +650,11 @@
     UM_REQUIRE(d->mode != UM_CONV_LN && d->bn >= 32 && d->ld_pre % 4 == 0 && d->ld_pre >= d->cout && d->cout % 32 == 0 &&
                    (reinterpret_cast<uintptr_t>(d->pre) & 15) == 0,
                "um_conv2d_tc: pre-accumulated input needs a non-LN mode, bn >= 32, cout %% 32 == 0 and 16-byte aligned rows");
+  if (d->in_partial)
+    UM_REQUIRE(d->mode == UM_CONV_LINEAR && d->act == UM_ACT_NONE && !d->pre && !win &&
+                   (reinterpret_cast<uintptr_t>(d->in_partial) & 3) == 0,
+               "um_conv2d_tc: InstanceNorm partials need a LINEAR layer without activation, pre-accumulated input or "
+               "window-plane output");
   UM_REQUIRE(d->stride == 1 || d->stride == 2 || d->stride == 4 || d->stride == 8, "um_conv2d_tc: stride must be 1, 2, 4 or 8");
   const int ho = (d->h + 2 * d->pad_h - d->kh) / d->stride + 1, wo = (d->w + 2 * d->pad_w - d->kw) / d->stride + 1;
   UM_REQUIRE(ho > 0 && wo > 0, "um_conv2d_tc: empty output");
@@ -621,6 +670,7 @@
   p.aux0 = d->aux0; p.ld_aux0 = d->ld_aux0; p.aux1 = d->aux1; p.ld_aux1 = d->ld_aux1;
   p.gamma = d->gamma; p.beta = d->beta;
   p.pre = d->pre; p.ld_pre = d->ld_pre;
+  p.in_partial = d->in_partial;
   if (d->split_plane_stride) p.plane_split = d->split_plane_stride;
   if (win) {
     p.win_dst = reinterpret_cast<__half*>(d->win_dst);
@@ -635,6 +685,8 @@
   const long long nk = ktot / 64;
   const bool multi = nk >= 8;
   const int bn = d->bn == 256 ? 128 : d->bn == 192 ? 96 : d->bn;
+  UM_REQUIRE(!d->in_partial || bn == 128 || (bn == 64 && multi),
+             "um_conv2d_tc: InstanceNorm partials need bn 128 / 256, or bn 64 over at least 8 K chunks of 64 channels");
   p.tiles_n = d->cout_p / bn;
   p.ntiles = p.tiles_x * p.tiles_y * p.B * p.tiles_n;
   CUtensorMap m0, m1, mw;
diff --git a/unimatch_b200/csrc/um_norm.cu b/unimatch_b200/csrc/um_norm.cu
--- a/unimatch_b200/csrc/um_norm.cu
+++ b/unimatch_b200/csrc/um_norm.cu
@@ -70,6 +70,56 @@
   stats[((long long)n * 2 + 1) * C + c] = (float)(1.0 / sqrt(var + 1e-5));
 }
 
+constexpr int FIN_CH = 8, FIN_LANES = 128;
+
+__global__ void __launch_bounds__(FIN_CH * FIN_LANES) in_finalize_tiles_kernel(const float* __restrict__ partial, int H, int W,
+                                                                              int th, int tw, int C, float* __restrict__ stats) {
+  __shared__ double red[FIN_LANES][FIN_CH];
+  const int cl = threadIdx.x % FIN_CH, lane = threadIdx.x / FIN_CH;
+  const int c = blockIdx.x * FIN_CH + cl, n = blockIdx.y;
+  const int ntx = (W + tw - 1) / tw, nt = ntx * ((H + th - 1) / th);
+  const float* base = partial + (long long)n * nt * 3 * C + c;
+  const bool live = c < C;
+  auto count = [&](int i) {
+    const int ty = i / ntx, tx = i - ty * ntx;
+    return (double)(min(th, H - ty * th) * min(tw, W - tx * tw));
+  };
+  auto tree = [&](double v) {
+    red[lane][cl] = v;
+    __syncthreads();
+    for (int s = FIN_LANES / 2; s > 0; s >>= 1) {
+      if (lane < s) red[lane][cl] += red[lane + s][cl];
+      __syncthreads();
+    }
+    const double total = red[0][cl];
+    __syncthreads();
+    return total;
+  };
+  const double hw = (double)H * (double)W;
+  double a = 0.0;
+  if (live)
+#pragma unroll 4
+    for (int i = lane; i < nt; i += FIN_LANES) {
+      const float* e = base + (long long)i * 3 * C;
+      a += count(i) * (double)__ldg(e) + (double)__ldg(e + C);
+    }
+  const double mean = tree(a) / hw;
+  double m2 = 0.0;
+  if (live)
+#pragma unroll 4
+    for (int i = lane; i < nt; i += FIN_LANES) {
+      const float* e = base + (long long)i * 3 * C;
+      const double ni = count(i), s = (double)__ldg(e + C), dm = (double)__ldg(e) + s / ni - mean;
+      m2 += ((double)__ldg(e + 2 * C) - s * s / ni) + ni * dm * dm;
+    }
+  double var = tree(m2) / hw;
+  if (live && lane == 0) {
+    if (var < 0.0) var = 0.0;
+    stats[((long long)n * 2) * C + c] = (float)mean;
+    stats[((long long)n * 2 + 1) * C + c] = (float)(1.0 / sqrt(var + 1e-5));
+  }
+}
+
 struct ApplyParams {
   const float* a; long long ld_a; const float* st_a; int relu_a;
   const float* res; long long ld_res; const float* st_res; int relu_out;
@@ -138,6 +188,15 @@
   const int total = n * c;
   in_finalize_kernel<<<(total + 127) / 128, 128, 0, st>>>(x, ld, scratch, stats, hw, c, total);
   return um::check_launch("um_instance_norm_stats(finalize)");
+}
+
+int um_instance_norm_finalize(const float* partial, int32_t n, int32_t h, int32_t w, int32_t tile_h, int32_t tile_w,
+                              int32_t c, float* stats, void* stream) {
+  UM_REQUIRE(partial && stats && n > 0 && h > 0 && w > 0 && tile_h > 0 && tile_w > 0 && c > 0 && n <= 65535,
+             "um_instance_norm_finalize: bad arguments");
+  in_finalize_tiles_kernel<<<dim3((c + FIN_CH - 1) / FIN_CH, n), FIN_CH * FIN_LANES, 0, (cudaStream_t)stream>>>(
+      partial, h, w, tile_h, tile_w, c, stats);
+  return um::check_launch("um_instance_norm_finalize");
 }
 
 int um_instance_norm_apply(const float* a, int64_t ld_a, const float* stats_a, int32_t relu_a, const float* res,
diff --git a/unimatch_b200/csrc/um_stem.cu b/unimatch_b200/csrc/um_stem.cu
--- a/unimatch_b200/csrc/um_stem.cu
+++ b/unimatch_b200/csrc/um_stem.cu
@@ -19,11 +19,13 @@
   float scale[3], shift[3];
   float* out; long long ld_out;
   __half* split; int cp; long long plane;
+  float* partial;
   int tiles_x, tiles_y, ntiles;
 };
+static_assert(TX == UM_STEM_TILE_W && TY == UM_STEM_TILE_H, "the InstanceNorm partials' tile grid is part of the ABI");
 
 template <int CIN, int S>
-__global__ void __launch_bounds__(NT) stem7x7_kernel(StemParams p) {
+__global__ void __launch_bounds__(NT, 2) stem7x7_kernel(StemParams p) {
   extern __shared__ __align__(16) float sm[];
   constexpr int IWR = (TX - 1) * S + 7, IW = (IWR + 3) & ~3, IH = (TY - 1) * S + 7;
   constexpr int NIN = (PX - 1) * S + 7;
@@ -126,6 +128,60 @@
           }
         }
       }
+      if (p.partial) {
+        float* s_piv = s_in + CIN * IH * IW + 8;
+        float* s_red = s_piv + 64;
+        if (pg == 0) {
+#pragma unroll
+          for (int cc = 0; cc < CB; ++cc) s_piv[cg * CB + cc] = acc[0][cc];
+        }
+        __syncthreads();
+        const int half = pg >> 5;
+        bool ok[PX];
+#pragma unroll
+        for (int j = 0; j < PX; ++j) ok[j] = oy < p.HO && tx0 + lx + j < p.WO;
+#pragma unroll
+        for (int c4 = 0; c4 < CB; c4 += 4) {
+          float s[4], q[4];
+#pragma unroll
+          for (int k = 0; k < 4; ++k) {
+            const float piv = s_piv[cg * CB + c4 + k];
+            s[k] = 0.f; q[k] = 0.f;
+#pragma unroll
+            for (int j = 0; j < PX; ++j) {
+              if (ok[j]) {
+                const float d = acc[j][c4 + k] - piv;
+                s[k] += d;
+                q[k] = fmaf(d, d, q[k]);
+              }
+            }
+          }
+#pragma unroll
+          for (int m = 16; m >= 1; m >>= 1) {
+#pragma unroll
+            for (int k = 0; k < 4; ++k) {
+              s[k] += __shfl_xor_sync(0xffffffffu, s[k], m);
+              q[k] += __shfl_xor_sync(0xffffffffu, q[k], m);
+            }
+          }
+          if ((tid & 31) == 0) {
+#pragma unroll
+            for (int k = 0; k < 4; ++k) {
+              s_red[(half * 64 + cg * CB + c4 + k) * 2] = s[k];
+              s_red[(half * 64 + cg * CB + c4 + k) * 2 + 1] = q[k];
+            }
+          }
+        }
+        __syncthreads();
+        if (tid < 64) {
+          const int c0 = cbase - cg * CB;
+          float* dst = p.partial + ((long long)t * 3) * p.cout + c0 + tid;
+          dst[0] = s_piv[tid];
+          dst[p.cout] = s_red[tid * 2] + s_red[(64 + tid) * 2];
+          dst[2 * p.cout] = s_red[tid * 2 + 1] + s_red[(64 + tid) * 2 + 1];
+        }
+        __syncthreads();
+      }
     }
   }
 }
@@ -133,7 +189,7 @@
 template <int CIN, int S>
 int launch(StemParams p, cudaStream_t st) {
   constexpr int IWR = (TX - 1) * S + 7, IW = (IWR + 3) & ~3, IH = (TY - 1) * S + 7;
-  const size_t smem = (size_t)(p.cout * CIN * 49 + CIN * IH * IW + 8) * sizeof(float);
+  const size_t smem = (size_t)(p.cout * CIN * 49 + CIN * IH * IW + 8 + (p.partial ? 64 + 256 : 0)) * sizeof(float);
   static um::PerDeviceBytes configured;
   if (int rc = um::ensure_smem(configured, stem7x7_kernel<CIN, S>, smem, "stem7x7")) return rc;
   const int num_sms = um::device_sm_count();
@@ -146,10 +202,12 @@
 
 }
 
-extern "C" int um_conv7x7_small(const float* in0, const float* in1, int32_t nchw, int32_t n_half, int32_t n, int32_t h,
-                                int32_t w, int32_t cin, int32_t stride, const float* weight, const float* bias, int32_t cout,
-                                int32_t relu, const float* scale, const float* shift, float* out_f32, int64_t ld_out,
-                                void* out_split, int32_t cp, void* stream) {
+extern "C" {
+
+int um_conv7x7_small_partials(const float* in0, const float* in1, int32_t nchw, int32_t n_half, int32_t n, int32_t h,
+                              int32_t w, int32_t cin, int32_t stride, const float* weight, const float* bias, int32_t cout,
+                              int32_t relu, const float* scale, const float* shift, float* out_f32, int64_t ld_out,
+                              void* out_split, int32_t cp, float* in_partial, void* stream) {
   UM_REQUIRE(in0 && weight && n > 0 && h > 0 && w > 0 && cin >= 1 && cin <= 3 && (stride == 1 || stride == 2),
              "um_conv7x7_small: bad arguments (1 <= cin <= 3, stride 1 or 2)");
   UM_REQUIRE(cout > 0 && cout % 16 == 0 && cout <= 128 && (out_f32 || out_split),
@@ -157,6 +215,7 @@
   UM_REQUIRE(!out_f32 || ld_out % 4 == 0, "um_conv7x7_small: bad output stride");
   UM_REQUIRE(!out_split || cp % 8 == 0, "um_conv7x7_small: bad plane width");
   UM_REQUIRE(!nchw || in1 || n_half >= n, "um_conv7x7_small: second source missing");
+  UM_REQUIRE(!in_partial || cout % 64 == 0, "um_conv7x7_small: InstanceNorm partials need cout a multiple of 64");
   StemParams p{};
   p.in0 = in0; p.in1 = in1; p.nchw = nchw; p.n_half = n_half;
   p.N = n; p.H = h; p.W = w; p.cin = cin; p.stride = stride;
@@ -165,6 +224,7 @@
   for (int c = 0; c < 3; ++c) { p.scale[c] = scale ? scale[c] : 1.f; p.shift[c] = shift ? shift[c] : 0.f; }
   p.out = out_f32; p.ld_out = ld_out;
   p.split = reinterpret_cast<__half*>(out_split); p.cp = cp; p.plane = (long long)n * p.HO * p.WO * cp;
+  p.partial = in_partial;
   cudaStream_t st = (cudaStream_t)stream;
   if (stride == 1) {
     if (cin == 1) return launch<1, 1>(p, st);
@@ -175,3 +235,13 @@
   if (cin == 2) return launch<2, 2>(p, st);
   return launch<3, 2>(p, st);
 }
+
+int um_conv7x7_small(const float* in0, const float* in1, int32_t nchw, int32_t n_half, int32_t n, int32_t h, int32_t w,
+                     int32_t cin, int32_t stride, const float* weight, const float* bias, int32_t cout, int32_t relu,
+                     const float* scale, const float* shift, float* out_f32, int64_t ld_out, void* out_split, int32_t cp,
+                     void* stream) {
+  return um_conv7x7_small_partials(in0, in1, nchw, n_half, n, h, w, cin, stride, weight, bias, cout, relu, scale, shift,
+                                   out_f32, ld_out, out_split, cp, nullptr, stream);
+}
+
+}
diff --git a/unimatch_b200/ops.py b/unimatch_b200/ops.py
--- a/unimatch_b200/ops.py
+++ b/unimatch_b200/ops.py
@@ -32,6 +32,7 @@
 
 ACT_NONE, ACT_RELU, ACT_TANH, ACT_SIGMOID, ACT_GELU = 0, 1, 2, 3, 4
 CONV_LINEAR, CONV_GRU_ZR, CONV_GRU_Q, CONV_LN = 0, 1, 2, 3
+CONV_TILE, STEM_TILE = (8, 16), (8, 32)
 
 
 class AttnGeom(ctypes.Structure):
@@ -53,7 +54,7 @@
                 ("src_plane_stride", ctypes.c_int64), ("split_plane_stride", ctypes.c_int64),
                 ("win_dst", ctypes.c_void_p), ("win_c0", ctypes.c_int32), ("win_c1", ctypes.c_int32),
                 ("win_lp", ctypes.c_int32), ("win_streams", ctypes.c_int32), ("win_geom", AttnGeom),
-                ("pre", ctypes.c_void_p), ("ld_pre", ctypes.c_int64)]
+                ("pre", ctypes.c_void_p), ("ld_pre", ctypes.c_int64), ("in_partial", ctypes.c_void_p)]
 
 
 class RaggedItem(ctypes.Structure):
@@ -119,9 +120,11 @@
     "um_conv2d_tc": (_RC, [ctypes.POINTER(ConvDesc), _P]),
     "um_ffn_tc": (_RC, [ctypes.POINTER(FfnDesc), _P]),
     "um_conv7x7_small": (_RC, [_P, _P, _I, _I, _I, _I, _I, _I, _I, _P, _P, _I, _I, _FP, _FP, _P, _L, _P, _I, _P]),
+    "um_conv7x7_small_partials": (_RC, [_P, _P, _I, _I, _I, _I, _I, _I, _I, _P, _P, _I, _I, _FP, _FP, _P, _L, _P, _I, _P, _P]),
     "um_instance_norm_scratch_floats": (_L, [_I, _I]),
     "um_instance_norm_stats": (_RC, [_P, _L, _I, _I, _I, _P, _P, _P]),
     "um_instance_norm_apply": (_RC, [_P, _L, _P, _I, _P, _L, _P, _I, _P, _L, _P, _I, _I, _I, _I, _I, _P]),
+    "um_instance_norm_finalize": (_RC, [_P, _I, _I, _I, _I, _I, _I, _P, _P]),
     "um_split_planes": (_RC, [_P, _L, _I, _L, _P, _I, _I, _L, _P]),
 }
 SYMBOLS = list(_SIGNATURES)
@@ -823,7 +826,7 @@
 
 def _conv2d_tc(src0, src1, weights, bias, kh, kw, pad_h, pad_w, cout, bn, mode, act, out_f32, off_f32, out_split,
                off_split, aux0, aux1, gamma=None, beta=None, stride=1, rows=0, win_dst=None, win_geom=None, win_c0=0,
-               win_c1=0, win_streams=0, pre=None):
+               win_c1=0, win_streams=0, pre=None, in_partial=None):
     d = ConvDesc()
     if rows:
         if rows % 16 or src0.dim() != 3 or rows > src0.shape[1]:
@@ -870,6 +873,10 @@
             raise RuntimeError("conv2d_tc: win_dst must be contiguous fp16 planes [ops, 2, streams, windows, lp, 128]")
         d.win_dst = win_dst.data_ptr(); d.win_geom = g; d.win_lp = lp
         d.win_c0, d.win_c1, d.win_streams = win_c0, win_c1, win_streams
+    if in_partial is not None:
+        ho, wo = (h + 2 * pad_h - kh) // stride + 1, (w + 2 * pad_w - kw) // stride + 1
+        _partials_shape(in_partial, b, ho, wo, cout, CONV_TILE, "conv2d_tc")
+        d.in_partial = in_partial.data_ptr()
     _check(LIB.um_conv2d_tc(ctypes.byref(d), _stream()), "um_conv2d_tc")
 
 
@@ -877,7 +884,8 @@
     "conv2d_tc(Tensor src0, Tensor? src1, Tensor weights, Tensor? bias, int kh, int kw, int pad_h, int pad_w, int cout, "
     "int bn, int mode, int act, Tensor(a!)? out_f32, int off_f32, Tensor(b!)? out_split, int off_split, Tensor? aux0, "
     "Tensor? aux1, Tensor? gamma=None, Tensor? beta=None, int stride=1, int rows=0, Tensor(c!)? win_dst=None, "
-    "int[]? win_geom=None, int win_c0=0, int win_c1=0, int win_streams=0, Tensor? pre=None) -> ()", _conv2d_tc)
+    "int[]? win_geom=None, int win_c0=0, int win_c1=0, int win_streams=0, Tensor? pre=None, Tensor(d!)? in_partial=None) -> ()",
+    _conv2d_tc)
 
 
 def ffn_tc_supported(rows):
@@ -946,7 +954,31 @@
     "Tensor(a!)? out_f32, Tensor(b!)? out_split, int off) -> ()", _instance_norm_apply)
 
 
-def _conv7x7_small(in0, in1, nchw, weight, bias, stride, relu, scale, shift, out_f32, out_split):
+def norm_partials(n, h, w, c, tile, device):
+    return torch.empty((n, -(-h // tile[0]), -(-w // tile[1]), 3, c), device=device, dtype=torch.float32)
+
+
+def _partials_shape(t, n, h, w, c, tile, name):
+    want = (n, -(-h // tile[0]), -(-w // tile[1]), 3, c)
+    _f32c(t, name + ": in_partial")
+    if tuple(t.shape) != want:
+        raise RuntimeError("%s: in_partial must be [%d, %d, %d, %d, %d] (norm_partials), got %s" % ((name,) + want + (list(t.shape),)))
+
+
+def _instance_norm_finalize(partial, h, w, tile_h, tile_w):
+    n, c = partial.shape[0], partial.shape[-1]
+    _partials_shape(partial, n, h, w, c, (tile_h, tile_w), "instance_norm_finalize")
+    stats = torch.empty((n, 2, c), device=partial.device, dtype=torch.float32)
+    _check(LIB.um_instance_norm_finalize(_p(partial), n, h, w, tile_h, tile_w, c, _p(stats), _stream()),
+           "um_instance_norm_finalize")
+    return stats
+
+
+instance_norm_finalize = _define("instance_norm_finalize(Tensor partial, int h, int w, int tile_h, int tile_w) -> Tensor",
+                                 _instance_norm_finalize)
+
+
+def _conv7x7_small(in0, in1, nchw, weight, bias, stride, relu, scale, shift, out_f32, out_split, in_partial=None):
     _f32c(in0, "in0"), _f32c(weight, "weight")
     if nchw:
         n0, cin, h, w = in0.shape
@@ -957,11 +989,17 @@
     cout = weight.shape[0]
     sc = (ctypes.c_float * 3)(*scale) if scale is not None else None
     sh = (ctypes.c_float * 3)(*shift) if shift is not None else None
-    _check(LIB.um_conv7x7_small(_p(in0), _p(in1), int(nchw), n0, n, h, w, cin, stride, _p(weight), _p(bias), cout, int(relu),
-                                sc, sh, _p(out_f32), out_f32.stride(-2) if out_f32 is not None else 0, _p(out_split),
-                                out_split.shape[-1] if out_split is not None else 0, _stream()), "um_conv7x7_small")
+    if in_partial is not None:
+        _partials_shape(in_partial, n, (h - 1) // stride + 1, (w - 1) // stride + 1, cout, STEM_TILE, "conv7x7_small")
+    _check(LIB.um_conv7x7_small_partials(_p(in0), _p(in1), int(nchw), n0, n, h, w, cin, stride, _p(weight), _p(bias), cout,
+                                         int(relu), sc, sh, _p(out_f32), out_f32.stride(-2) if out_f32 is not None else 0,
+                                         _p(out_split), out_split.shape[-1] if out_split is not None else 0, _p(in_partial),
+                                         _stream()), "um_conv7x7_small")
 
 
 conv7x7_small = _define(
     "conv7x7_small(Tensor in0, Tensor? in1, bool nchw, Tensor weight, Tensor? bias, int stride, bool relu, float[]? scale, "
     "float[]? shift, Tensor(a!)? out_f32, Tensor(b!)? out_split) -> ()", _conv7x7_small)
+conv7x7_small_partials = _define(
+    "conv7x7_small_partials(Tensor in0, Tensor? in1, bool nchw, Tensor weight, Tensor? bias, int stride, bool relu, "
+    "float[]? scale, float[]? shift, Tensor(a!)? out_f32, Tensor(b!)? out_split, Tensor(c!) in_partial) -> ()", _conv7x7_small)
diff --git a/unimatch_b200/unimatch.py b/unimatch_b200/unimatch.py
--- a/unimatch_b200/unimatch.py
+++ b/unimatch_b200/unimatch.py
@@ -237,8 +237,9 @@
         T = P["tcb"]
         dev = img0.device
         nb = img0.shape[0] + (img1.shape[0] if img1 is not None else 0)
-        C, IS, IA = self._conv, _OPS.instance_norm_stats, _OPS.instance_norm_apply
+        C, IA = self._conv, _OPS.instance_norm_apply
         pad64 = lambda c: (c + 63) // 64 * 64
+        fused = dev.type == "cuda"
 
         nplanes = [0]
 
@@ -249,41 +250,54 @@
             nplanes[0] += 1
             return self._zero_padded("backbone%d" % nplanes[0], (2, nb, h, w, cp), dev)
 
-        def conv(src_s, name, h, w, stride=None):
+        def conv_in(src_s, name, h, w):
             layer = T[name]
-            out = torch.empty((nb, *layer.out_hw(h, w, layer.stride if stride is None else stride), layer.cout), device=dev)
-            C(layer, src_s, out_f32=out, stride=stride)
-            return out
+            ho, wo = layer.out_hw(h, w, layer.stride)
+            out = torch.empty((nb, ho, wo, layer.cout), device=dev)
+            if not fused:
+                C(layer, src_s, out_f32=out)
+                return out, _OPS.instance_norm_stats(out)
+            part = ops.norm_partials(nb, ho, wo, layer.cout, ops.CONV_TILE, dev)
+            C(layer, src_s, out_f32=out, in_partial=part)
+            return out, _OPS.instance_norm_finalize(part, ho, wo, *ops.CONV_TILE)
 
         hh, ww = img0.shape[2], img0.shape[3]
-        a = torch.empty((nb, (hh - 1) // 2 + 1, (ww - 1) // 2 + 1, 64), device=dev)
+        h, w = (hh - 1) // 2 + 1, (ww - 1) // 2 + 1
+        a = torch.empty((nb, h, w, 64), device=dev)
         if normalise:
             mean, std = (0.485, 0.456, 0.406), (0.229, 0.224, 0.225)
             scale = [1.0 / (255.0 * s_) for s_ in std]
             shift = [-m_ / s_ for m_, s_ in zip(mean, std)]
         else:
             scale = shift = None
-        _OPS.conv7x7_small(img0, img1, True, P["raw"]["backbone.conv1.weight"], None, 2, False, scale, shift, a, None)
-        h, w = a.shape[1], a.shape[2]
+        w_stem = P["raw"]["backbone.conv1.weight"]
+        if fused:
+            part = ops.norm_partials(nb, h, w, 64, ops.STEM_TILE, dev)
+            _OPS.conv7x7_small_partials(img0, img1, True, w_stem, None, 2, False, scale, shift, a, None, part)
+            st_a = _OPS.instance_norm_finalize(part, h, w, *ops.STEM_TILE)
+        else:
+            _OPS.conv7x7_small(img0, img1, True, w_stem, None, 2, False, scale, shift, a, None)
+            st_a = _OPS.instance_norm_stats(a)
         cur_f = torch.empty((nb, h, w, 64), device=dev)
         cur_s = planes(h, w, 64)
-        IA(a, IS(a), True, None, None, False, cur_f, cur_s, 0)
+        IA(a, st_a, True, None, None, False, cur_f, cur_s, 0)
         for li in (1, 2, 3):
             for bi in range(2):
                 pf = "backbone.layer%d.%d." % (li, bi)
-                a1 = conv(cur_s, pf + "conv1", h, w)
+                a1, st1 = conv_in(cur_s, pf + "conv1", h, w)
                 _, ho, wo, cout = a1.shape
                 t_s = planes(ho, wo, cout)
-                IA(a1, IS(a1), True, None, None, False, None, t_s, 0)
-                a2 = conv(t_s, pf + "conv2", ho, wo)
+                IA(a1, st1, True, None, None, False, None, t_s, 0)
+                a2, st2 = conv_in(t_s, pf + "conv2", ho, wo)
                 if (pf + "downsample.0") in T:
-                    res = conv(cur_s, pf + "downsample.0", h, w)
-                    st_res = IS(res)
+                    res, st_res = conv_in(cur_s, pf + "downsample.0", h, w)
                 else:
                     res, st_res = cur_f, None
-                out_f = torch.empty((nb, ho, wo, cout), device=dev)
+                nxt = "backbone.layer%d.%d." % ((li, 1) if bi == 0 else (li + 1, 0))
+                keep_f = (nxt + "conv1") in T and (nxt + "downsample.0") not in T
+                out_f = torch.empty((nb, ho, wo, cout), device=dev) if keep_f else None
                 out_s = planes(ho, wo, cout)
-                IA(a2, IS(a2), True, res, st_res, True, out_f, out_s, 0)
+                IA(a2, st2, True, res, st_res, True, out_f, out_s, 0)
                 cur_f, cur_s, h, w = out_f, out_s, ho, wo
         x6 = torch.empty((nb, h, w, 128), device=dev)
         x6_s = planes(h, w, 128) if self.num_scales > 1 else None
@@ -291,7 +305,12 @@
         if self.num_scales == 1:
             return [x6]
         strides = (1, 2, 4, 8)[:self.num_scales]
-        feats = [conv(x6_s, "backbone.trident_conv", h, w, stride=s) for s in strides]
+        feats = []
+        for s in strides:
+            layer = T["backbone.trident_conv"]
+            out = torch.empty((nb, *layer.out_hw(h, w, s), layer.cout), device=dev)
+            C(layer, x6_s, out_f32=out, stride=s)
+            feats.append(out)
         return feats[::-1]
 
     @staticmethod
```
